# vibevoice-community/VibeVoice

Hardware: AMD Instinct MI355X
Metric: audio-sec/wall-sec (higher is better)
Workload: dtype bf16

## Files before the change

include/vvhip.h:

```cpp
#ifndef VVHIP_H
#define VVHIP_H
#include <stdint.h>
#ifdef __cplusplus
extern "C" {
#endif
typedef struct vv_ctx vv_ctx;

typedef struct vv_config {
    int lm_hidden, lm_layers, lm_heads, lm_kv_heads, lm_head_dim, lm_inter, lm_vocab;
    float lm_eps;
    int head_layers, head_ffn, latent_dim;
    float head_eps;
    int n_filters, n_ratios, ratios[8];
    int n_stages, enc_depths[8];
    int sem_dim;
    int has_acoustic_encoder;
    float codec_eps;
    int n_slots;
    int max_ctx;
    int max_rows;
    int xsplit;
    int attn_splits;
    int enc_frames;
    int use_graph;
    int tts_layers;
} vv_config;

#pragma GCC visibility push(default)
int vv_create(const vv_config* cfg, vv_ctx** out);
int vv_create_shared(const vv_config* cfg, vv_ctx* parent, vv_ctx** out);
void vv_destroy(vv_ctx* ctx);
const char* vv_last_error(vv_ctx* ctx);
const char* vv_build_id(void);
int vv_check(vv_ctx* ctx, void* stream);

int vv_num_weights(vv_ctx* ctx);
int vv_weight_info(vv_ctx* ctx, int idx, char* name, int name_cap, int64_t* nelem, int* loaded);
int vv_upload(vv_ctx* ctx, const char* name, const void* src, int src_dtype, int64_t nelem);
int vv_weight_read(vv_ctx* ctx, void* stream, const char* name, float* out_dev);
int vv_weight_shape(vv_ctx* ctx, const char* name, int* N, int* K);
int vv_lora_merge(vv_ctx* ctx, void* stream, const char* name, const float* a_dev, const float* b_dev, int r, float scale,
                  int delta_bf16);
int vv_lora_reset(vv_ctx* ctx, void* stream, const char* name);
int vv_set_speech_factors(vv_ctx* ctx, float scaling, float bias);
int vv_set_valid_tokens(vv_ctx* ctx, const int* ids, int n);
int vv_set_schedule(vv_ctx* ctx, int n_steps, const float* t, const float* coef, void* stream);
int vv_set_schedule_sde(vv_ctx* ctx, int n_steps, const float* t, const float* coef6, void* stream);

typedef struct vv_row { int cache; int pos; } vv_row;

int vv_lm_forward(vv_ctx* ctx, void* stream, int n_rows, const vv_row* rows,
                  const float* x_in_dev, float* hidden_out_dev);
int vv_lm_forward_range(vv_ctx* ctx, void* stream, int n_rows, const vv_row* rows, const float* x_in_dev,
                        float* hidden_out_dev, int layer_begin, int layer_end, int final_norm);
int vv_kv_import(vv_ctx* ctx, void* stream, int cache, int layer, int n_pos, const void* k_dev, const void* v_dev,
                 int src_dtype);
int vv_kv_import_at(vv_ctx* ctx, void* stream, int cache, int layer, int pos0, int n_pos, const void* k_dev,
                    const void* v_dev, int src_dtype);
int vv_kv_move(vv_ctx* ctx, void* stream, int cache, int src_pos, int dst_pos);
int vv_kv_export(vv_ctx* ctx, void* stream, int cache, int layer, int pos0, int n_pos, void* k_out_dev, void* v_out_dev,
                 int dst_dtype);
int64_t vv_kv_snapshot_bytes(vv_ctx* ctx, int n_pos);
int vv_kv_snapshot(vv_ctx* ctx, void* stream, int cache, int n_pos, void* k_out_dev, void* v_out_dev);
int vv_kv_restore(vv_ctx* ctx, void* stream, int cache, int n_pos, const void* k_dev, const void* v_dev);
int vv_add_type_embedding(vv_ctx* ctx, void* stream, int n, const float* x_dev, int type, float* out_dev);
int vv_eos_logit(vv_ctx* ctx, void* stream, int n, const float* hidden_dev, float* out_dev);
int vv_embed(vv_ctx* ctx, void* stream, int n, const int* ids, float* out_dev);
int vv_lm_logits(vv_ctx* ctx, void* stream, int n, const float* hidden_dev, float* logits_out_dev);
int vv_lm_logits_full(vv_ctx* ctx, void* stream, int n, const float* hidden_dev, float* logits_out_dev);
int vv_lm_warp_valid(vv_ctx* ctx, void* stream, int n, const float* logits_dev, const unsigned char* seen_dev,
                     float repetition_penalty, float temperature, int do_sample, int top_k, float top_p, float min_p,
                     float* out_dev, int* survivors_dev);
typedef struct vv_noise_key { uint32_t seed_lo, seed_hi, t0, aux; } vv_noise_key;
int vv_noise_rows(vv_ctx* ctx, void* stream, int n, const vv_noise_key* keys_host, uint32_t stream0, int n_streams,
                  int n_t, int width, float* out_dev);

int vv_diffusion_sample(vv_ctx* ctx, void* stream, int n, const float* cond_dev, const float* noise_dev,
                        float cfg_scale, float* latent_out_dev);
int vv_diffusion_sample_sde(vv_ctx* ctx, void* stream, int n, const float* cond_dev, const float* noise_dev,
                            const float* step_noise_dev, float cfg_scale, float* latent_out_dev);
int vv_diffusion_sample_rows(vv_ctx*, void* stream, int n, const float* cond_dev, const float* noise_dev,
                             const float* step_noise_dev, const float* cfg_rows_dev, float* latent_out_dev);
int vv_set_schedule_general(vv_ctx* ctx, int n_steps, const float* t, const float* coef8, int stochastic, void* stream);
int vv_diffusion_sample_general(vv_ctx* ctx, void* stream, int n, const float* cond_dev, const float* noise_dev,
                                const float* step_noise_dev, float cfg_scale, const float* cfg_rows_dev, float* latent_out_dev);
int vv_head_forward(vv_ctx* ctx, void* stream, int n, const float* noisy_dev, const float* t_host,
                    const float* cond_dev, float* out_dev);

int vv_codec_decode(vv_ctx* ctx, void* stream, int slot, int frames, const float* latent_dev,
                    float* audio_out_dev, int apply_speech_factors);
int vv_semantic_encode(vv_ctx* ctx, void* stream, int slot, int frames, const float* audio_dev,
                       float* sem_out_dev);
int vv_codec_chain_batch(vv_ctx* ctx, void* stream, int n, const int* slots, const float* latent_dev,
                         float* audio_out_dev, float* sem_out_dev, int apply_speech_factors);
int vv_acoustic_encode(vv_ctx* ctx, void* stream, int frames, const float* wav_dev, float* mean_out_dev);
int vv_acoustic_encode_ragged(vv_ctx* ctx, void* stream, int frames, long long valid_samples, const float* wav_dev, float* mean_out_dev);
int vv_set_enc_pass_frames(vv_ctx* ctx, int frames_per_pass);
int vv_audio_to_pcm16(vv_ctx* ctx, void* stream, int n, int samples, const float* audio_dev, int16_t* pcm_out_dev);
int vv_resampler_set(vv_ctx* ctx, int rs, int L, int M, int T, const float* coef_host, int n_streams, void* stream);
int vv_resampler_reset(vv_ctx* ctx, void* stream, int rs, int n, const int* stream_ids_host);
typedef struct vv_resample_row { int stream; int n_in; int flush; } vv_resample_row;
int vv_resample_rows(vv_ctx* ctx, void* stream, int rs, int n, const vv_resample_row* rows_host, const float* audio_dev, int ld_in,
                     void* out_dev, int ld_out, int out_fmt, int* n_out_host);
int vv_resample_once(vv_ctx* ctx, void* stream, int L, int M, int T, const float* coef_dev, int n, int n_in, const float* audio_dev,
                     int ld_in, float* out_dev, int ld_out);
int vv_tempo_set(vv_ctx* ctx, int tp, const float* window_host, int n_streams, void* stream);
int vv_tempo_reset(vv_ctx* ctx, void* stream, int tp, int n, const int* stream_ids_host);
#define VV_TEMPO_OVER_CAPACITY 3
typedef struct vv_tempo_row { int stream; int n_in; int flush; int P; int Q; } vv_tempo_row;
int vv_tempo_rows(vv_ctx* ctx, void* stream, int tp, int n, const vv_tempo_row* rows_host, const float* audio_dev, int ld_in,
                  void* out_dev, int ld_out, int out_fmt, int* n_out_host, int* offsets_dev, int ld_off);
int vv_tempo_once(vv_ctx* ctx, void* stream, const float* window_dev, int P, int Q, int n, int n_in, const float* audio_dev, int ld_in,
                  float* out_dev, int ld_out, int* offsets_dev, int ld_off);
int vv_codec_reset(vv_ctx* ctx, void* stream, int slot);
int vv_connect(vv_ctx* ctx, void* stream, int n, const float* latent_dev, const float* sem_dev,
               float* embeds_out_dev);

int64_t vv_packed_bytes(int N, int K);
int vv_pack_matrix(void* stream, const float* src_dev, void* dst_dev, int N, int K);
int vv_unpack_matrix(void* stream, const void* packed_dev, float* dst_dev, int N, int K);
int vv_lora_merge_raw(void* stream, const void* base_packed_dev, void* dst_packed_dev, int N, int K,
                      const float* a_dev, const float* b_dev, int r, float scale, int delta_bf16);
int vv_gemm_raw(void* stream, const void* w_packed_dev, const void* w2_packed_dev, const float* x_dev,
                float* y_dev, int T, int N, int K, int ldx, int ldy, int pro, int epi,
                const float* nw_dev, float eps, const float* bias_dev, const float* nscale_dev,
                int xsplit, int ksplit, int nontemporal);
#define VV_GEMV_REFUSED 1
typedef struct vv_gemv_case_args {
    const void* W; const void* W2; const float* X; float* Y;
    int T, N, K, ldx, ldy;
    int pro, epi;
    const float* nw; float eps; const float* bias; const float* nscale;
    const float* mod_scale; const float* mod_shift; int ld_mod;
    const float* addvec; int x_row_mod, add_rows_per_vec;
    const float* gate; int ld_gate;
    float* z; float* x0p; const float* coef; float cfg; int n_cfg; const float* sde_noise;
    int kgrid; float* yparts; const float* xa; int n_xa; const float* ya; int n_ya; int part_stride;
    int sl_n, sl_T, sl_x, sl_y; int sl_id[8];
    const float* dw_hist; const float* dw_w; const float* dw_b; const float* dw_gamma; const float* dw_nw;
    float* dw_xout; float* dw_hnew;
    const float* cfg_rows;
} vv_gemv_case_args;
int vv_gemv_case(void* stream, const vv_gemv_case_args* args, int xsplit, int* form_out);
int vv_gemm3_raw(vv_ctx* ctx, void* stream, const void* w_packed_dev, const void* w2_packed_dev, const float* x_dev, int T, int N, int K,
                 int epi, const float* nw_dev, float eps, const float* bias_dev, float* y_dev, void* xp_scratch, void* yp_scratch);
int vv_profile_begin(vv_ctx* ctx);
int vv_profile_end(vv_ctx* ctx, int64_t* launches, double* total_ms, double* bytes);
int vv_profile_replay(vv_ctx* ctx, void* stream, int reps, int64_t* launches, double* total_ms, double* bytes);
int vv_profile_replay_family(vv_ctx* ctx, void* stream, int family, int reps, int64_t* launches, double* total_ms, double* bytes);
int64_t vv_stat(vv_ctx* ctx, int what);

#pragma GCC visibility pop
#ifdef __cplusplus
}
#endif
#endif
```

vibevoice_amd/_lib.py:

```python
import ctypes as C
import os

HERE = os.path.dirname(os.path.abspath(__file__))
LIB_PATH = os.environ.get("VVHIP_LIB", os.path.join(HERE, "libvvhip.so"))


class VVConfig(C.Structure):
    _fields_ = [
        ("lm_hidden", C.c_int), ("lm_layers", C.c_int), ("lm_heads", C.c_int), ("lm_kv_heads", C.c_int),
        ("lm_head_dim", C.c_int), ("lm_inter", C.c_int), ("lm_vocab", C.c_int), ("lm_eps", C.c_float),
        ("head_layers", C.c_int), ("head_ffn", C.c_int), ("latent_dim", C.c_int), ("head_eps", C.c_float),
        ("n_filters", C.c_int), ("n_ratios", C.c_int), ("ratios", C.c_int * 8),
        ("n_stages", C.c_int), ("enc_depths", C.c_int * 8), ("sem_dim", C.c_int),
        ("has_acoustic_encoder", C.c_int), ("codec_eps", C.c_float),
        ("n_slots", C.c_int), ("max_ctx", C.c_int), ("max_rows", C.c_int), ("xsplit", C.c_int),
        ("attn_splits", C.c_int), ("enc_frames", C.c_int), ("use_graph", C.c_int), ("tts_layers", C.c_int),
    ]


class VVRow(C.Structure):
    _fields_ = [("cache", C.c_int), ("pos", C.c_int)]


_P = C.c_void_p


class VVGemvCase(C.Structure):
    _fields_ = [
        ("W", _P), ("W2", _P), ("X", _P), ("Y", _P),
        ("T", C.c_int), ("N", C.c_int), ("K", C.c_int), ("ldx", C.c_int), ("ldy", C.c_int),
        ("pro", C.c_int), ("epi", C.c_int),
        ("nw", _P), ("eps", C.c_float), ("bias", _P), ("nscale", _P),
        ("mod_scale", _P), ("mod_shift", _P), ("ld_mod", C.c_int),
        ("addvec", _P), ("x_row_mod", C.c_int), ("add_rows_per_vec", C.c_int),
        ("gate", _P), ("ld_gate", C.c_int),
        ("z", _P), ("x0p", _P), ("coef", _P), ("cfg", C.c_float), ("n_cfg", C.c_int), ("sde_noise", _P),
        ("kgrid", C.c_int), ("yparts", _P), ("xa", _P), ("n_xa", C.c_int), ("ya", _P), ("n_ya", C.c_int), ("part_stride", C.c_int),
        ("sl_n", C.c_int), ("sl_T", C.c_int), ("sl_x", C.c_int), ("sl_y", C.c_int), ("sl_id", C.c_int * 8),
        ("dw_hist", _P), ("dw_w", _P), ("dw_b", _P), ("dw_gamma", _P), ("dw_nw", _P), ("dw_xout", _P), ("dw_hnew", _P),
        ("cfg_rows", _P),
    ]


class VVNoiseKey(C.Structure):
    _fields_ = [("seed_lo", C.c_uint32), ("seed_hi", C.c_uint32), ("t0", C.c_uint32), ("aux", C.c_uint32)]


class VVResampleRow(C.Structure):
    _fields_ = [("stream", C.c_int), ("n_in", C.c_int), ("flush", C.c_int)]


class VVTempoRow(C.Structure):
    _fields_ = [("stream", C.c_int), ("n_in", C.c_int), ("flush", C.c_int), ("P", C.c_int), ("Q", C.c_int)]


GEMV_REFUSED = 1
TEMPO_OVER_CAPACITY = 3
_SIGS = {
    "vv_create": (C.c_int, [C.POINTER(VVConfig), C.POINTER(_P)]),
    "vv_create_shared": (C.c_int, [C.POINTER(VVConfig), _P, C.POINTER(_P)]),
    "vv_destroy": (None, [_P]),
    "vv_last_error": (C.c_char_p, [_P]),
    "vv_num_weights": (C.c_int, [_P]),
    "vv_weight_info": (C.c_int, [_P, C.c_int, C.c_char_p, C.c_int, C.POINTER(C.c_int64), C.POINTER(C.c_int)]),
    "vv_upload": (C.c_int, [_P, C.c_char_p, _P, C.c_int, C.c_int64]),
    "vv_set_speech_factors": (C.c_int, [_P, C.c_float, C.c_float]),
    "vv_set_valid_tokens": (C.c_int, [_P, C.POINTER(C.c_int), C.c_int]),
    "vv_set_schedule": (C.c_int, [_P, C.c_int, C.POINTER(C.c_float), C.POINTER(C.c_float), _P]),
    "vv_set_schedule_sde": (C.c_int, [_P, C.c_int, C.POINTER(C.c_float), C.POINTER(C.c_float), _P]),
    "vv_set_schedule_general": (C.c_int, [_P, C.c_int, C.POINTER(C.c_float), C.POINTER(C.c_float), C.c_int, _P]),
    "vv_lm_forward": (C.c_int, [_P, _P, C.c_int, C.POINTER(VVRow), _P, _P]),
    "vv_lm_forward_range": (C.c_int, [_P, _P, C.c_int, C.POINTER(VVRow), _P, _P, C.c_int, C.c_int, C.c_int]),
    "vv_kv_import": (C.c_int, [_P, _P, C.c_int, C.c_int, C.c_int, _P, _P, C.c_int]),
    "vv_kv_import_at": (C.c_int, [_P, _P, C.c_int, C.c_int, C.c_int, C.c_int, _P, _P, C.c_int]),
    "vv_add_type_embedding": (C.c_int, [_P, _P, C.c_int, _P, C.c_int, _P]),
    "vv_eos_logit": (C.c_int, [_P, _P, C.c_int, _P, _P]),
    "vv_embed": (C.c_int, [_P, _P, C.c_int, C.POINTER(C.c_int), _P]),
    "vv_lm_logits": (C.c_int, [_P, _P, C.c_int, _P, _P]),
    "vv_lm_logits_full": (C.c_int, [_P, _P, C.c_int, _P, _P]),
    "vv_lm_warp_valid": (C.c_int, [_P, _P, C.c_int, _P, _P, C.c_float, C.c_float, C.c_int, C.c_int, C.c_float, C.c_float, _P, _P]),
    "vv_noise_rows": (C.c_int, [_P, _P, C.c_int, C.POINTER(VVNoiseKey), C.c_uint32, C.c_int, C.c_int, C.c_int, _P]),
    "vv_diffusion_sample": (C.c_int, [_P, _P, C.c_int, _P, _P, C.c_float, _P]),
    "vv_diffusion_sample_sde": (C.c_int, [_P, _P, C.c_int, _P, _P, _P, C.c_float, _P]),
    "vv_diffusion_sample_rows": (C.c_int, [_P, _P, C.c_int, _P, _P, _P, _P, _P]),
    "vv_diffusion_sample_general": (C.c_int, [_P, _P, C.c_int, _P, _P, _P, C.c_float, _P, _P]),
    "vv_head_forward": (C.c_int, [_P, _P, C.c_int, _P, C.POINTER(C.c_float), _P, _P]),
    "vv_codec_decode": (C.c_int, [_P, _P, C.c_int, C.c_int, _P, _P, C.c_int]),
    "vv_semantic_encode": (C.c_int, [_P, _P, C.c_int, C.c_int, _P, _P]),
    "vv_codec_chain_batch": (C.c_int, [_P, _P, C.c_int, _P, _P, _P, _P, C.c_int]),
    "vv_acoustic_encode": (C.c_int, [_P, _P, C.c_int, _P, _P]),
    "vv_acoustic_encode_ragged": (C.c_int, [_P, _P, C.c_int, C.c_longlong, _P, _P]),
    "vv_kv_move": (C.c_int, [_P, _P, C.c_int, C.c_int, C.c_int]),
    "vv_kv_export": (C.c_int, [_P, _P, C.c_int, C.c_int, C.c_int, C.c_int, _P, _P, C.c_int]),
    "vv_kv_snapshot_bytes": (C.c_int64, [_P, C.c_int]),
    "vv_kv_snapshot": (C.c_int, [_P, _P, C.c_int, C.c_int, _P, _P]),
    "vv_kv_restore": (C.c_int, [_P, _P, C.c_int, C.c_int, _P, _P]),
    "vv_set_enc_pass_frames": (C.c_int, [_P, C.c_int]),
    "vv_audio_to_pcm16": (C.c_int, [_P, _P, C.c_int, C.c_int, _P, _P]),
    "vv_resampler_set": (C.c_int, [_P, C.c_int, C.c_int, C.c_int, C.c_int, _P, C.c_int, _P]),
    "vv_resampler_reset": (C.c_int, [_P, _P, C.c_int, C.c_int, C.POINTER(C.c_int)]),
    "vv_resample_rows": (C.c_int, [_P, _P, C.c_int, C.c_int, C.POINTER(VVResampleRow), _P, C.c_int, _P, C.c_int, C.c_int,
                                   C.POINTER(C.c_int)]),
    "vv_resample_once": (C.c_int, [_P, _P, C.c_int, C.c_int, C.c_int, _P, C.c_int, C.c_int, _P, C.c_int, _P, C.c_int]),
    "vv_tempo_set": (C.c_int, [_P, C.c_int, _P, C.c_int, _P]),
    "vv_tempo_reset": (C.c_int, [_P, _P, C.c_int, C.c_int, C.POINTER(C.c_int)]),
    "vv_tempo_rows": (C.c_int, [_P, _P, C.c_int, C.c_int, C.POINTER(VVTempoRow), _P, C.c_int, _P, C.c_int, C.c_int, C.POINTER(C.c_int), _P,
                                C.c_int]),
    "vv_tempo_once": (C.c_int, [_P, _P, _P, C.c_int, C.c_int, C.c_int, C.c_int, _P, C.c_int, _P, C.c_int, _P, C.c_int]),
    "vv_codec_reset": (C.c_int, [_P, _P, C.c_int]),
    "vv_connect": (C.c_int, [_P, _P, C.c_int, _P, _P, _P]),
    "vv_packed_bytes": (C.c_int64, [C.c_int, C.c_int]),
    "vv_pack_matrix": (C.c_int, [_P, _P, _P, C.c_int, C.c_int]),
    "vv_unpack_matrix": (C.c_int, [_P, _P, _P, C.c_int, C.c_int]),
    "vv_lora_merge_raw": (C.c_int, [_P, _P, _P, C.c_int, C.c_int, _P, _P, C.c_int, C.c_float, C.c_int]),
    "vv_weight_read": (C.c_int, [_P, _P, C.c_char_p, _P]),
    "vv_weight_shape": (C.c_int, [_P, C.c_char_p, C.POINTER(C.c_int), C.POINTER(C.c_int)]),
    "vv_lora_merge": (C.c_int, [_P, _P, C.c_char_p, _P, _P, C.c_int, C.c_float, C.c_int]),
    "vv_lora_reset": (C.c_int, [_P, _P, C.c_char_p]),
    "vv_gemm_raw": (C.c_int, [_P, _P, _P, _P, _P, C.c_int, C.c_int, C.c_int, C.c_int, C.c_int, C.c_int, C.c_int,
                              _P, C.c_float, _P, _P, C.c_int, C.c_int, C.c_int]),
    "vv_gemv_case": (C.c_int, [_P, C.POINTER(VVGemvCase), C.c_int, C.POINTER(C.c_int)]),
    "vv_gemm3_raw": (C.c_int, [_P, _P, _P, _P, _P, C.c_int, C.c_int, C.c_int, C.c_int, _P, C.c_float, _P, _P, _P, _P]),
    "vv_profile_begin": (C.c_int, [_P]),
    "vv_profile_end": (C.c_int, [_P, C.POINTER(C.c_int64), C.POINTER(C.c_double), C.POINTER(C.c_double)]),
    "vv_profile_replay": (C.c_int, [_P, _P, C.c_int, C.POINTER(C.c_int64), C.POINTER(C.c_double), C.POINTER(C.c_double)]),
    "vv_profile_replay_family": (C.c_int, [_P, _P, C.c_int, C.c_int, C.POINTER(C.c_int64), C.POINTER(C.c_double), C.POINTER(C.c_double)]),
    "vv_stat": (C.c_int64, [_P, C.c_int]),
    "vv_build_id": (C.c_char_p, []),
    "vv_check": (C.c_int, [_P, _P]),
}

EXPORTS = tuple(_SIGS)
_lib = None


def load():
    global _lib
    if _lib is not None:
        return _lib
    if not os.path.exists(LIB_PATH):
        raise RuntimeError(
            f"{LIB_PATH} is missing: the HIP engine has not been built "
            "(run `python -m vibevoice_amd.build`); there is no CPU/PyTorch fallback")
    from . import build as _build
    if _build.have_sources() and _build.binary_id(LIB_PATH) != _build.source_id():
        import sys
        print(f"[vibevoice_amd] {LIB_PATH} was built from other sources (binary id {_build.binary_id(LIB_PATH)}, sources "
              f"{_build.source_id()}): rebuilding with hipcc (about two minutes)", file=sys.stderr, flush=True)
        try:
            _build.build_locked()
        except Exception as ex:
            raise RuntimeError(
                f"{LIB_PATH} was built from different sources (binary id {_build.binary_id(LIB_PATH)}, sources "
                f"{_build.source_id()}) and could not be rebuilt ({ex}); run `python -m vibevoice_amd.build`") from ex
    lib = C.CDLL(LIB_PATH)
    for name, (res, args) in _SIGS.items():
        fn = getattr(lib, name)
        fn.restype = res
        fn.argtypes = args
    _lib = lib
    return lib
```

vibevoice_amd/build.py:

```python
import os
import shutil
import subprocess
import sys

HERE = os.path.dirname(os.path.abspath(__file__))
CSRC = os.path.join(HERE, "csrc")
LIB = os.path.join(HERE, "libvvhip.so")
SOURCES = ["gemm.hip", "gemv.hip", "gemv16p.hip", "headtail.hip", "solver.hip", "tile.hip", "prefill.hip", "attn.hip", "misc.hip", "warp.hip", "noise.hip", "kvspan.hip", "block1d.hip", "lora.hip", "resample.hip", "tempo.hip", "engine.hip",
           "engine_lm.hip", "engine_head.hip", "engine_codec.hip", "engine_prof.hip", "engine_lora.hip"]
HEADERS = [os.path.join(CSRC, "vv_common.h"), os.path.join(CSRC, "vv_device.h"), os.path.join(CSRC, "vv_launch.h"), os.path.join(CSRC, "gemv_plan.h"),
           os.path.join(CSRC, "prefill_plan.h"), os.path.join(CSRC, "pass_plan.h"), os.path.join(CSRC, "engine_ctx.h"),
           os.path.join(os.path.dirname(HERE), "include", "vvhip.h")]


def _hipcc():
    for c in ("/opt/rocm/bin/hipcc", shutil.which("hipcc") or ""):
        if c and os.path.exists(c):
            return c
    raise RuntimeError("hipcc not found: libvvhip.so cannot be built")


FLAGS = ["--offload-arch=gfx950", "-O3", "-std=c++17", "-fPIC", "-shared", "-fvisibility=hidden", "-fvisibility-inlines-hidden",
         "-Wno-unused-value", "-Wno-unused-result", "-mllvm", "-amdgpu-kernarg-preload-count=16"]


def _extra_flags():
    return os.environ.get("VVHIP_CFLAGS", "").split()


def source_id():
    import hashlib
    h = hashlib.sha256()
    for d in [os.path.join(CSRC, s) for s in SOURCES] + HEADERS:
        h.update(os.path.basename(d).encode() + b"\0")
        with open(d, "rb") as f:
            h.update(f.read())
    h.update(" ".join(FLAGS + _extra_flags()).encode())
    return h.hexdigest()[:16]


def binary_id(path=LIB):
    try:
        with open(path, "rb") as f:
            blob = f.read()
    except OSError:
        return None
    k = blob.find(b"VVHIP_BUILD_ID=")
    if k < 0:
        return None
    return blob[k + 15:k + 31].decode("ascii", "replace")


def have_sources():
    return all(os.path.exists(d) for d in [os.path.join(CSRC, s) for s in SOURCES] + HEADERS)


def stale():
    if not os.path.exists(LIB):
        return True
    return have_sources() and binary_id() != source_id()


def _object_key(src, flags, build_id):
    import hashlib
    h = hashlib.sha256()
    for d in [src] + HEADERS:
        with open(d, "rb") as f:
            h.update(f.read())
    h.update(" ".join(flags).encode())
    if os.path.basename(src) == "engine.hip":
        h.update(build_id.encode())
    return h.hexdigest()[:16]


def build(force=False, verbose=True, _locked=False):
    if not force and not stale():
        return LIB
    if not _locked:
        import fcntl
        with open(LIB + ".lock", "w") as lk:
            fcntl.flock(lk, fcntl.LOCK_EX)
            try:
                if not force and not stale():
                    return LIB
                return build(force=force, verbose=verbose, _locked=True)
            finally:
                fcntl.flock(lk, fcntl.LOCK_UN)
    from concurrent.futures import ThreadPoolExecutor
    hipcc = _hipcc()
    bid = source_id()
    cflags = [f for f in FLAGS if f != "-shared"] + _extra_flags()
    objdir = os.path.join(CSRC, ".obj")
    os.makedirs(objdir, exist_ok=True)
    jobs, objs = [], []
    for sname in SOURCES:
        src = os.path.join(CSRC, sname)
        obj = os.path.join(objdir, f"{os.path.splitext(sname)[0]}.{_object_key(src, cflags, bid)}.o")
        objs.append(obj)
        if not os.path.exists(obj):
            jobs.append((src, obj))

    def compile_one(job):
        src, obj = job
        tmp = f"{obj}.tmp{os.getpid()}"
        cmd = [hipcc] + cflags + [f'-DVV_BUILD_ID="{bid}"', "-c", src, "-o", tmp]
        if verbose:
            print("[vibevoice_amd] compiling", os.path.basename(src), file=sys.stderr)
        subprocess.run(cmd, check=True)
        os.replace(tmp, obj)
    with ThreadPoolExecutor(max_workers=min(8, max(1, len(jobs)))) as ex:
        list(ex.map(compile_one, jobs))
    keep = set(objs)
    for fn in os.listdir(objdir):
        full = os.path.join(objdir, fn)
        if fn.endswith(".o") and full not in keep:
            try:
                os.remove(full)
            except OSError:
                pass
    tmp = f"{LIB}.tmp{os.getpid()}"
    cmd = [hipcc, "--offload-arch=gfx950", "-shared", "-fPIC"] + _extra_flags() + objs + ["-o", tmp]
    if verbose:
        print("[vibevoice_amd] linking libvvhip.so", file=sys.stderr)
    subprocess.run(cmd, check=True)
    os.replace(tmp, LIB)
    return LIB


def build_locked():
    import fcntl
    with open(LIB + ".lock", "w") as lk:
        fcntl.flock(lk, fcntl.LOCK_EX)
        try:
            if stale():
                build(force=True, verbose=False, _locked=True)
        finally:
            fcntl.flock(lk, fcntl.LOCK_UN)
    return LIB


if __name__ == "__main__":
    build(force="--force" in sys.argv)
    print(LIB)
```

vibevoice_amd/csrc/block1d.hip:

```cpp
#include "vv_common.h"
#include "vv_device.h"
#include "vv_launch.h"

namespace {

struct VVBlock {
    const float* xin;
    float* xout;
    float* nst;
    const float *norm_w, *ffn_norm_w, *gamma, *ffn_gamma, *dw_w , *dw_b, *b1, *b2;
    const u32x4 *w1, *w2;
    int T;
    float eps;
    VVSlotIds sl;
    int64_t sx, snst;
};

template <int XS>
__device__ __forceinline__ void split_store(unsigned char* base, size_t part_stride, int byte_off, float v) {
    __bf16 h = (__bf16)v;
    *reinterpret_cast<__bf16*>(base + byte_off) = h;
    if constexpr (XS > 1) {
        float r = v - (float)h;
        __bf16 m = (__bf16)r;
        *reinterpret_cast<__bf16*>(base + part_stride + byte_off) = m;
        if constexpr (XS > 2) *reinterpret_cast<__bf16*>(base + 2 * part_stride + byte_off) = (__bf16)(r - (float)m);
    }
}

template <int C, int XS>
__global__ __launch_bounds__(256) void vv_block1d_kernel(const VVBlock a) {
    constexpr int TT = 16, HALO = 6, F = 4 * C;
    constexpr int KT1 = C / 32, NT1 = F / 16;
    constexpr int KT2 = F / 32, NT2 = C / 16;
    extern __shared__ __attribute__((aligned(16))) unsigned char smem[];
    float* nrm = reinterpret_cast<float*>(smem);
    float* xs = nrm + (TT + HALO) * C;
    float* rs2 = xs + TT * C;
    unsigned char* f1 = reinterpret_cast<unsigned char*>(rs2 + TT);
    unsigned char* f2 = f1 + (size_t)XS * KT1 * 1024;
    const int tid = threadIdx.x, lane = tid & 63;
    const int wave = __builtin_amdgcn_readfirstlane(tid >> 6);
    const int t0 = blockIdx.x * TT;
    const float* xin = a.xin; float* xout = a.xout; float* nst = a.nst;
    if (a.sl.n > 0) {
        const int64_t id = vv_slot_id(a.sl.id, blockIdx.y);
        xin += id * a.sx; xout += id * a.sx; nst += id * a.snst;
    }
    constexpr int M1 = (NT1 + 3) / 4, M2 = (NT2 + 3) / 4;
    u32x4 w1r[M1][KT1], w2r[M2][KT2];
#pragma unroll
    for (int i = 0; i < M1; ++i) {
        const int nt = wave + 4 * i;
#pragma unroll
        for (int kt = 0; kt < KT1; ++kt)
            w1r[i][kt] = (nt < NT1) ? a.w1[((int64_t)nt * KT1 + kt) * 64 + lane] : u32x4{0u, 0u, 0u, 0u};
    }
#pragma unroll
    for (int i = 0; i < M2; ++i) {
        const int nt = wave + 4 * i;
#pragma unroll
        for (int kt = 0; kt < KT2; ++kt)
            w2r[i][kt] = (nt < NT2) ? a.w2[((int64_t)nt * KT2 + kt) * 64 + lane] : u32x4{0u, 0u, 0u, 0u};
    }

    constexpr int CL = (C + 63) / 64;
    float nw_r[CL], fnw_r[CL];
#pragma unroll
    for (int i = 0; i < CL; ++i) {
        const int c = lane + i * 64;
        nw_r[i] = (c < C) ? a.norm_w[c] : 0.f;
        fnw_r[i] = (c < C) ? a.ffn_norm_w[c] : 0.f;
    }
    const int cc = tid % C;
    float dw_r[7];
#pragma unroll
    for (int j = 0; j < 7; ++j) dw_r[j] = a.dw_w[j * C + cc];
    const float dwb_r = a.dw_b[cc], gam_r = a.gamma[cc];
    const int frow = lane & 15, fq = lane >> 4;
    float4 b1_r[M1], b2_r[M2], fg_r[M2];
#pragma unroll
    for (int i = 0; i < M1; ++i) {
        const int nt = wave + 4 * i;
        b1_r[i] = (nt < NT1) ? *reinterpret_cast<const float4*>(a.b1 + nt * 16 + fq * 4) : float4{0.f, 0.f, 0.f, 0.f};
    }
#pragma unroll
    for (int i = 0; i < M2; ++i) {
        const int nt = wave + 4 * i;
        b2_r[i] = (nt < NT2) ? *reinterpret_cast<const float4*>(a.b2 + nt * 16 + fq * 4) : float4{0.f, 0.f, 0.f, 0.f};
        fg_r[i] = (nt < NT2) ? *reinterpret_cast<const float4*>(a.ffn_gamma + nt * 16 + fq * 4) : float4{0.f, 0.f, 0.f, 0.f};
    }

    constexpr int RW = (TT + HALO + 3) / 4;
    float xv[RW][CL];
#pragma unroll
    for (int i = 0; i < RW; ++i) {
        const int rr = wave + 4 * i;
        const int t = t0 - HALO + rr;
#pragma unroll
        for (int q = 0; q < CL; ++q) {
            const int c = lane + q * 64;
            float v = 0.f;
            if (rr < TT + HALO && c < C) {
                if (t < 0) v = nst[(HALO + t) * C + c];
                else if (t < a.T) v = xin[(int64_t)t * C + c];
            }
            xv[i][q] = v;
        }
    }
#pragma unroll
    for (int i = 0; i < RW; ++i) {
        const int rr = wave + 4 * i;
        if (rr >= TT + HALO) break;
        const int t = t0 - HALO + rr;
        if (t < 0) {
#pragma unroll
            for (int q = 0; q < CL; ++q) { const int c = lane + q * 64; if (c < C) nrm[rr * C + c] = xv[i][q]; }
        } else if (t < a.T) {
            float s = 0.f;
#pragma unroll
            for (int q = 0; q < CL; ++q) s += xv[i][q] * xv[i][q];
            const float r = rsqrtf(vv_wave_sum(s) / (float)C + a.eps);
#pragma unroll
            for (int q = 0; q < CL; ++q) {
                const int c = lane + q * 64;
                if (c < C) {
                    const float n = xv[i][q] * r * nw_r[q];
                    nrm[rr * C + c] = n;
                    if (rr >= HALO) xs[(rr - HALO) * C + c] = xv[i][q];
                    if (t >= a.T - HALO) nst[(HALO + t - (a.T - HALO)) * C + c] = n;
                }
            }
        } else {
#pragma unroll
            for (int q = 0; q < CL; ++q) {
                const int c = lane + q * 64;
                if (c < C) { nrm[rr * C + c] = 0.f; if (rr >= HALO) xs[(rr - HALO) * C + c] = 0.f; }
            }
        }
    }
    __syncthreads();
    for (int e = tid; e < TT * C; e += 256) {
        const int r = e / C;
        float acc = dwb_r;
#pragma unroll
        for (int j = 0; j < 7; ++j) acc += dw_r[j] * nrm[(r + j) * C + cc];
        xs[e] += gam_r * acc;
    }
    __syncthreads();
    for (int r = wave; r < TT; r += 4) {
        float s = 0.f;
        float xr[CL];
#pragma unroll
        for (int q = 0; q < CL; ++q) { const int c = lane + q * 64; xr[q] = (c < C) ? xs[r * C + c] : 0.f; s += xr[q] * xr[q]; }
        const float rr = rsqrtf(vv_wave_sum(s) / (float)C + a.eps);
#pragma unroll
        for (int q = 0; q < CL; ++q) {
            const int c = lane + q * 64;
            if (c < C) {
                const float n = xr[q] * rr * fnw_r[q];
                const int off = vv_packed_index(c >> 5, r, c) * 2;
                split_store<XS>(f1, (size_t)KT1 * 1024, off, n);
            }
        }
    }
    __syncthreads();
#pragma unroll
    for (int i1 = 0; i1 < M1; ++i1) {
        const int nt = wave + 4 * i1;
        if (nt >= NT1) break;
        f32x4 acc = {0.f, 0.f, 0.f, 0.f};
#pragma unroll
        for (int kt = 0; kt < KT1; ++kt) {
            const bf16x8 wf = __builtin_bit_cast(bf16x8, w1r[i1][kt]);
#pragma unroll
            for (int p = 0; p < XS; ++p) {
                const bf16x8 xb = __builtin_bit_cast(bf16x8, *reinterpret_cast<const u32x4*>(f1 + ((size_t)(p * KT1 + kt) * 64 + lane) * 16));
                acc = __builtin_amdgcn_mfma_f32_16x16x32_bf16(wf, xb, acc, 0, 0, 0);
            }
        }
        const int n0 = nt * 16 + fq * 4;
        float u[4];
        const float bb[4] = {b1_r[i1].x, b1_r[i1].y, b1_r[i1].z, b1_r[i1].w};
#pragma unroll
        for (int r = 0; r < 4; ++r) u[r] = vv_gelu_erf(acc[r] + bb[r]);
        const int off = vv_packed_index(n0 >> 5, frow, n0) * 2;
#pragma unroll
        for (int r = 0; r < 4; ++r) split_store<XS>(f2, (size_t)KT2 * 1024, off + r * 2, u[r]);
    }
    __syncthreads();
#pragma unroll
    for (int i2 = 0; i2 < M2; ++i2) {
        const int nt = wave + 4 * i2;
        if (nt >= NT2) break;
        f32x4 acc = {0.f, 0.f, 0.f, 0.f};
#pragma unroll
        for (int kt = 0; kt < KT2; ++kt) {
            const bf16x8 wf = __builtin_bit_cast(bf16x8, w2r[i2][kt]);
#pragma unroll
            for (int p = 0; p < XS; ++p) {
                const bf16x8 ub = __builtin_bit_cast(bf16x8, *reinterpret_cast<const u32x4*>(f2 + ((size_t)(p * KT2 + kt) * 64 + lane) * 16));
                acc = __builtin_amdgcn_mfma_f32_16x16x32_bf16(wf, ub, acc, 0, 0, 0);
            }
        }
        const int c0 = nt * 16 + fq * 4;
        const int t = t0 + frow;
        if (t < a.T) {
            float4 o;
            o.x = xs[frow * C + c0 + 0] + fg_r[i2].x * (acc[0] + b2_r[i2].x);
            o.y = xs[frow * C + c0 + 1] + fg_r[i2].y * (acc[1] + b2_r[i2].y);
            o.z = xs[frow * C + c0 + 2] + fg_r[i2].z * (acc[2] + b2_r[i2].z);
            o.w = xs[frow * C + c0 + 3] + fg_r[i2].w * (acc[3] + b2_r[i2].w);
            *reinterpret_cast<float4*>(xout + (int64_t)t * C + c0) = o;
        }
    }
}

template <int C, int XS>
static void go(const VVBlock& a, hipStream_t s) {
    constexpr int TT = 16, HALO = 6, F = 4 * C;
    const size_t smem = (size_t)((TT + HALO) * C + TT * C + TT) * 4 + (size_t)XS * (C / 32) * 1024 + (size_t)XS * (F / 32) * 1024;
    static const hipError_t lds = vv_raise_lds_limit(160 * 1024, &vv_block1d_kernel<C, XS>);
    (void)lds;
    hipLaunchKernelGGL((vv_block1d_kernel<C, XS>), dim3((a.T + TT - 1) / TT, a.sl.n > 0 ? a.sl.n : 1), dim3(256), smem, s, a);
}

}

extern "C" int vv_block1d_supported(int C) { return C == 32 || C == 64 || C == 128; }
extern "C" int vv_block1d_slots_launch(int C, int xs, const float* xin, float* xout, float* nst, const float* norm_w,
                                       const float* ffn_norm_w, const float* gamma, const float* ffn_gamma,
                                       const float* dw_w, const float* dw_b, const float* b1, const float* b2,
                                       const void* w1, const void* w2, int T, float eps, const int* ids, int n, int64_t sx,
                                       int64_t snst, hipStream_t s) {
    if (n < 0 || n > 8) return -1;
    VVBlock a{xin, xout, nst, norm_w, ffn_norm_w, gamma, ffn_gamma, dw_w, dw_b, b1, b2,
              (const u32x4*)w1, (const u32x4*)w2, T, eps};
    a.sl = vv_slot_ids(ids, n);
    a.sx = sx; a.snst = snst;
#define VV_B(C_)                                                     \
    do {                                                             \
        if (xs == 1) go<C_, 1>(a, s);                                \
        else if (xs == 2) go<C_, 2>(a, s);                           \
        else go<C_, 3>(a, s);                                        \
    } while (0)
    if (C == 32) VV_B(32);
    else if (C == 64) VV_B(64);
    else if (C == 128) VV_B(128);
    else return -1;
#undef VV_B
    return vv_launch_rc(0);
}
```

vibevoice_amd/csrc/engine_codec.hip:

```cpp
#include "engine_ctx.h"

static bool is_stem(const ConvG& g) { return g.K == 7 && g.ldx == 1; }
static bool is_conv1_head(const ConvG& g) { return g.N == 1 && g.K == 7 * g.ldx && (g.ldx & 3) == 0 && g.ldx <= 1024; }

int build_codec(vv_ctx* ctx, CodecNet& net, const std::string& pfx, bool decoder, int vae_dim, int Fmax, int n_slots) {
    const vv_config& c = ctx->c;
    const int ns = c.n_stages;
    const int nf = c.n_filters;
    net.decoder = decoder; net.Fmax = Fmax;
    std::vector<int> depths(ns), ratios(c.n_ratios);
    if (decoder) { for (int i = 0; i < ns; ++i) depths[i] = c.enc_depths[ns - 1 - i]; for (int i = 0; i < c.n_ratios; ++i) ratios[i] = c.ratios[i]; }
    else { for (int i = 0; i < ns; ++i) depths[i] = c.enc_depths[i]; for (int i = 0; i < c.n_ratios; ++i) ratios[i] = c.ratios[c.n_ratios - 1 - i]; }
    int hop = 1; for (int i = 0; i < c.n_ratios; ++i) hop *= c.ratios[i];
    ctx->hop = hop;
    std::vector<int> C(ns), Tpf(ns);
    for (int i = 0; i < ns; ++i) {
        if (decoder) { C[i] = nf << (ns - 1 - i); Tpf[i] = (i == 0) ? 1 : Tpf[i - 1] * ratios[i - 1]; }
        else { C[i] = nf << i; Tpf[i] = (i == 0) ? hop : Tpf[i - 1] / ratios[i - 1]; }
    }
    net.in_dim = decoder ? vae_dim : 1;
    net.out_dim = decoder ? 1 : vae_dim;
    net.in_Tpf = decoder ? 1 : hop;
    net.in_hist = 6;
    net.maxC = 1;
    size_t umax = 0;
    struct StageW { ConvG in; std::vector<Block> blocks; };
    std::vector<StageW> sw(ns);
    for (int i = 0; i < ns; ++i) {
        ConvG& g = sw[i].in;
        char nm[256];
        if (i == 0) {
            const int Cin = net.in_dim;
            g.K = 7 * Cin; g.N = C[0]; g.ldx = Cin; g.rows_per_frame = Tpf[0];
            g.w = alloc_packed(ctx, g.N, g.K);
            snprintf(nm, 256, "%s%s.0.0.conv.conv.", pfx.c_str(), decoder ? "upsample_layers" : "downsample_layers");
            add_mat(ctx, std::string(nm) + "weight", g.N, g.K, g.w, 0, 1, Cin, g.N, 7, 1);
            g.bias = add_vec(ctx, std::string(nm) + "bias", g.N);
        } else if (decoder) {
            const int s = ratios[i - 1], Cin = C[i - 1], Cout = C[i];
            g.K = 2 * Cin; g.N = s * Cout; g.ldx = Cin; g.rows_per_frame = Tpf[i - 1];
            g.w = alloc_packed(ctx, g.N, g.K);
            snprintf(nm, 256, "%supsample_layers.%d.0.convtr.convtr.", pfx.c_str(), i);
            add_mat(ctx, std::string(nm) + "weight", g.N, g.K, g.w, 0, 2, Cin, Cout, 2 * s, s, (int64_t)Cin * Cout * 2 * s);
            g.bias = add_vec(ctx, std::string(nm) + "bias", Cout, nullptr, W_BIAS_REP, s);
        } else {
            const int s = ratios[i - 1], Cin = C[i - 1], Cout = C[i];
            g.K = 2 * s * Cin; g.N = Cout; g.ldx = s * Cin; g.rows_per_frame = Tpf[i];
            g.w = alloc_packed(ctx, g.N, g.K);
            snprintf(nm, 256, "%sdownsample_layers.%d.0.conv.conv.", pfx.c_str(), i);
            add_mat(ctx, std::string(nm) + "weight", g.N, g.K, g.w, 0, 1, Cin, Cout, 2 * s, s);
            g.bias = add_vec(ctx, std::string(nm) + "bias", Cout);
        }
        if (C[i] > net.maxC) net.maxC = C[i];
        for (int j = 0; j < depths[i]; ++j) {
            Block b; b.C = C[i]; b.nb = nullptr;
            snprintf(nm, 256, "%sstages.%d.%d.", pfx.c_str(), i, j);
            std::string p(nm);
            b.gamma = add_vec(ctx, p + "gamma", C[i]);
            b.ffn_gamma = add_vec(ctx, p + "ffn_gamma", C[i]);
            b.norm_w = add_vec(ctx, p + "norm.weight", C[i]);
            b.ffn_norm_w = add_vec(ctx, p + "ffn_norm.weight", C[i]);
            b.dw_w = add_vec(ctx, p + "mixer.conv.conv.conv.weight", (int64_t)C[i] * 7, nullptr, W_DW);
            b.dw_b = add_vec(ctx, p + "mixer.conv.conv.conv.bias", C[i]);
            b.w1 = alloc_packed(ctx, 4 * C[i], C[i]);
            add_mat(ctx, p + "ffn.linear1.weight", 4 * C[i], C[i], b.w1, 0);
            b.b1 = add_vec(ctx, p + "ffn.linear1.bias", 4 * C[i]);
            b.w2 = alloc_packed(ctx, C[i], 4 * C[i]);
            add_mat(ctx, p + "ffn.linear2.weight", C[i], 4 * C[i], b.w2, 0);
            b.b2 = add_vec(ctx, p + "ffn.linear2.bias", C[i]);
            sw[i].blocks.push_back(b);
            size_t ub = (size_t)Tpf[i] * Fmax * 4 * C[i] * 4;
            if (ub > umax) umax = ub;
        }
    }
    {
        ConvG& g = net.head;
        const int Cin = C[ns - 1];
        g.K = 7 * Cin; g.N = net.out_dim; g.ldx = Cin; g.rows_per_frame = Tpf[ns - 1];
        g.w = alloc_packed(ctx, g.N, g.K);
        add_mat(ctx, pfx + "head.conv.conv.weight", g.N, g.K, g.w, 0, 1, Cin, g.N, 7, 1);
        g.bias = add_vec(ctx, pfx + "head.conv.conv.bias", g.N);
    }
    auto pad64 = [](size_t n) { return (n + 63) / 64 * 64; };
    net.u.resize(n_slots);
    net.u_stride = (int64_t)pad64(umax / 4 + 1);
    float* u_all = (float*)dalloc(ctx, (size_t)n_slots * net.u_stride * 4, false);
    net.in_buf.resize(n_slots); net.st.resize(n_slots);
    net.in_stride = (int64_t)pad64((size_t)(6 + net.in_Tpf * Fmax) * net.in_dim);
    float* in_all = (float*)dalloc(ctx, (size_t)n_slots * net.in_stride * 4);
    if (!u_all || !in_all) return -1;
    for (int sl = 0; sl < n_slots; ++sl) {
        net.u[sl] = u_all + (size_t)sl * net.u_stride;
        net.in_buf[sl] = in_all + (size_t)sl * net.in_stride;
        net.st[sl].resize(ns);
    }
    for (int i = 0; i < ns; ++i) {
        const int hist = (i == ns - 1) ? 6 : (decoder ? 1 : ratios[i]);
        const bool fused = vv_block1d_supported(C[i]) && Tpf[i] >= 8 && !sw[i].blocks.empty();
        const bool pp = !fused && !sw[i].blocks.empty() && (vv_normdw_sliced_ok(Tpf[i], C[i]) || vv_normdw_rows_ok(Tpf[i], C[i]));
        const int64_t xstride = (int64_t)pad64((size_t)(hist + (size_t)Tpf[i] * Fmax) * C[i]);
        float* xs_all = (float*)dalloc(ctx, (size_t)n_slots * xstride * 4);
        float* xs2_all = (fused || pp) ? (float*)dalloc(ctx, (size_t)n_slots * xstride * 4) : nullptr;
        if (!xs_all || ((fused || pp) && !xs2_all)) return -1;
        const int64_t nbstride = (int64_t)pad64(fused ? (size_t)12 * C[i] : (size_t)(6 + (size_t)Tpf[i] * Fmax) * C[i]);
        std::vector<float*> nb_all(sw[i].blocks.size());
        for (auto& p : nb_all) { p = (float*)dalloc(ctx, (size_t)n_slots * nbstride * 4); if (!p) return -1; }
        for (int sl = 0; sl < n_slots; ++sl) {
            Stage& s = net.st[sl][i];
            s.C = C[i]; s.Tpf = Tpf[i]; s.in = sw[i].in; s.hist = hist; s.fused = fused; s.pp = pp; s.sl_stride = xstride;
            s.xs = xs_all + (size_t)sl * xstride;
            s.xs2 = xs2_all ? xs2_all + (size_t)sl * xstride : nullptr;
            s.blocks = sw[i].blocks;
            s.xfinal = ((s.fused || s.pp) && (s.blocks.size() & 1)) ? s.xs2 : s.xs;
            for (size_t j = 0; j < s.blocks.size(); ++j) {
                Block& b = s.blocks[j];
                b.nb = nullptr; b.nst = nullptr; b.nb_stride = nbstride;
                if (s.fused) b.nst = nb_all[j] + (size_t)sl * nbstride;
                else b.nb = nb_all[j] + (size_t)sl * nbstride;
            }
        }
    }
    {
        const char* mode = getenv("VVHIP_BATCH_CODEC");
        const bool off = (mode && !strcmp(mode, "0")) || ctx->c.xsplit > 2 || n_slots < 2 || Fmax != 1;
        const bool heavy_only = mode && !strcmp(mode, "heavy");
        auto gemm_ok = [&](const ConvG& cg, int64_t sx, int64_t sy) {
            VVGemm g = mk_gemm(cg.w, net.in_buf[0], net.u[0], 2 * cg.rows_per_frame, cg.N, cg.K, cg.ldx, cg.N);
            g.epi = VV_EPI_BIAS; g.bias = cg.bias;
            g.sl_n = 2; g.sl_T = cg.rows_per_frame; g.sl_x = (int)sx; g.sl_y = (int)sy; g.sl_id[0] = 0; g.sl_id[1] = n_slots - 1;
            return vv_gemv_ok(&g) != 0;
        };
        auto ok = [&](int i) {
            const Stage& s = net.st[0][i];
            if (off || s.blocks.empty() || (s.C & 31)) return false;
            if (!is_stem(s.in) && !gemm_ok(s.in, i == 0 ? net.in_stride : net.st[0][i - 1].sl_stride, s.sl_stride)) return false;
            if (s.pp && vv_normdw_sliced_ok(s.Tpf, s.C)) return true;
            if (heavy_only) return false;
            return s.fused || (s.pp && vv_normdw_rows_ok(s.Tpf, s.C));
        };
        net.kd = 0; net.ke = ns;
        if (decoder) { while (net.kd < ns && ok(net.kd)) net.kd++; }
        else { while (net.ke > 0 && ok(net.ke - 1)) net.ke--; }
        const ConvG& h = net.head;
        const bool conv1 = is_conv1_head(h);
        net.head_batch = !off && !heavy_only && (conv1 || gemm_ok(h, net.st[0][ns - 1].sl_stride, 0));
        if (!decoder && net.ke < ns && !(conv1 || gemm_ok(h, net.st[0][ns - 1].sl_stride, 0))) net.ke = ns;
    }
    return 0;
}

struct SlotSet { const int* ids; int n; int sl; };
static SlotSet one_slot(int sl) { return {nullptr, 0, sl}; }

static void codec_table_entries(CodecNet& net, int sl, int F, std::vector<VVShiftH>& t) {
    t.push_back({net.in_buf[sl], net.in_Tpf * F, 6, net.in_dim});
    for (auto& s : net.st[sl]) {
        t.push_back({s.xfinal, s.Tpf * F, s.hist, s.C});
        for (auto& b : s.blocks) {
            if (s.fused) t.push_back({b.nst, 6, 6, s.C});
            else t.push_back({b.nb, s.Tpf * F, 6, s.C});
        }
    }
}
static int codec_tables(vv_ctx* ctx, CodecNet& net, SlotSet ss, int F, void** tab_out, int* n_out) {
    const int* ids = ss.n ? ss.ids : &ss.sl;
    const int n = ss.n ? ss.n : 1;
    uint64_t mask = 0;
    for (int j = 0; j < n; ++j) {
        if (ids[j] >= 64) return fail(ctx, "tokenizer slot %d: the history tables are keyed by a 64-bit slot mask", ids[j]);
        mask |= 1ull << ids[j];
    }
    auto it = net.shift_tab.find({mask, F});
    if (it == net.shift_tab.end()) {
        std::vector<VVShiftH> t;
        for (int j = 0; j < n; ++j) codec_table_entries(net, ids[j], F, t);
        void* d = dalloc(ctx, t.size() * sizeof(VVShiftH), false);
        if (!d) return -1;
        HIPCHK(ctx, hipMemcpy(d, t.data(), t.size() * sizeof(VVShiftH), hipMemcpyHostToDevice));
        it = net.shift_tab.emplace(std::make_pair(mask, F), std::make_pair(d, (int)t.size())).first;
    }
    *tab_out = it->second.first; *n_out = it->second.second;
    return 0;
}

static int run_codec(vv_ctx* ctx, CodecNet& net, SlotSet ss, int F, float* out, hipStream_t st, int i0 = 0, int i1 = -1,
                     bool head = true, bool shift = true, int tail_valid = -1) {
    const float eps = ctx->c.codec_eps;
    const bool batched = ss.n > 0;
    const bool stream_w = (F == 1);
    const int base = batched ? 0 : ss.sl;
    auto& stages = net.st[base];
    float* u = net.u[base];
    const int ns = (int)stages.size();
    if (i1 < 0) i1 = ns;
    auto stride = [&](int64_t s) { return batched ? s : (int64_t)0; };
    auto slots = [&](VVGemm& g, int rows, int64_t sx, int64_t sy) {
        if (!batched) return;
        g.sl_n = ss.n; g.sl_T = rows; g.sl_x = (int)sx; g.sl_y = (int)sy; g.T = ss.n * rows;
        for (int j = 0; j < 8; ++j) g.sl_id[j] = j < ss.n ? ss.ids[j] : 0;
    };
    auto nt = [&](int rows) { return batched ? 1 : (int)(stream_w && rows <= 16); };
    auto ffn1 = [&](const Stage& s, const Block& b, float* xo, int T, const float* dw_in) {
        VVGemm g1 = mk_gemm(b.w1, dw_in ? dw_in : xo, u, T, 4 * s.C, s.C, s.C, 4 * s.C);
        g1.pro = VV_PRO_RMS; g1.nw = b.ffn_norm_w; g1.eps = eps; g1.epi = VV_EPI_BIAS_GELU; g1.bias = b.b1; g1.nt = nt(T);
        if (dw_in) {
            g1.pro = VV_PRO_NORMDW;
            g1.dw_hist = b.nb; g1.dw_w = b.dw_w; g1.dw_b = b.dw_b; g1.dw_gamma = b.gamma; g1.dw_nw = b.norm_w;
            g1.dw_xout = xo; g1.dw_hnew = b.nb + 6 * (size_t)s.C;
        }
        slots(g1, T, s.sl_stride, 0);
        return g1;
    };
    auto ffn = [&](const Stage& s, const Block& b, const VVGemm& g1, float* xo, int T) -> int {
        GEMM(g1);
        VVGemm g2 = mk_gemm(b.w2, u, xo, T, s.C, 4 * s.C, 4 * s.C, s.C);
        g2.epi = VV_EPI_RESID; g2.bias = b.b2; g2.nscale = b.ffn_gamma; g2.nt = nt(T);
        slots(g2, T, 0, s.sl_stride);
        GEMM(g2);
        return 0;
    };
    for (int i = i0; i < i1; ++i) {
        Stage& s = stages[i];
        const int T = s.Tpf * F;
        float* x = s.xs + (size_t)s.hist * s.C;
        if (tail_valid >= 0 && i > 0) {
            Stage& pv = stages[i - 1];
            const int Tp = pv.Tpf * F;
            if (tail_valid < Tp)
                VVCHK(vv_zero_launch(pv.xfinal + ((size_t)pv.hist + tail_valid) * pv.C, (size_t)(Tp - tail_valid) * pv.C * 4, st));
            const int r = pv.Tpf / s.Tpf;
            tail_valid = (tail_valid + r - 1) / r;
        }
        {
            const ConvG& cg = s.in;
            const float* X = (i == 0) ? net.in_buf[base] : stages[i - 1].xfinal;
            const int64_t sx = (i == 0) ? net.in_stride : stages[i - 1].sl_stride;
            const int Trows = cg.rows_per_frame * F;
            if (is_stem(cg)) {
                ctx->launches++;
                VVCHK(vv_stem_conv_slots_launch(X, cg.w, cg.bias, x, Trows, cg.N, ss.ids, ss.n, stride(sx), stride(s.sl_stride), st));
            } else {
                VVGemm g = mk_gemm(cg.w, X, x, Trows, cg.N, cg.K, cg.ldx, cg.N);
                g.epi = VV_EPI_BIAS; g.bias = cg.bias; g.nt = nt(Trows);
                slots(g, Trows, sx, s.sl_stride);
                GEMM(g);
            }
        }
        float* xo = (s.fused || s.pp) ? s.xs2 + (size_t)s.hist * s.C : x;
        if (s.fused) {
            for (auto& b : s.blocks) {
                ctx->launches++;
                VVCHK(vv_block1d_slots_launch(s.C, ctx->c.xsplit, x, xo, b.nst, b.norm_w, b.ffn_norm_w, b.gamma, b.ffn_gamma, b.dw_w, b.dw_b,
                                              b.b1, b.b2, b.w1, b.w2, T, eps, ss.ids, ss.n, stride(s.sl_stride), stride(b.nb_stride), st));
                std::swap(x, xo);
            }
            continue;
        }
        for (auto& b : s.blocks) {
            const bool sliced = s.pp && vv_normdw_sliced_ok(T, s.C);
            if (sliced && T == 1 && !batched) {
                const VVGemm g1 = ffn1(s, b, xo, T, x);
                if (vv_gemv_ok(&g1)) {
                    VVTRY(ffn(s, b, g1, xo, T));
                    std::swap(x, xo);
                    continue;
                }
            }
            if (sliced) {
                ctx->launches += 1;
                VVCHK(vv_normdw_sliced_slots_launch(x, xo, b.nb, b.norm_w, b.dw_w, b.dw_b, b.gamma, T, s.C, eps, ss.ids, ss.n, stride(s.sl_stride),
                                                    stride(b.nb_stride), st));
            } else if (s.pp && vv_normdw_rows_ok(T, s.C)) {
                ctx->launches += 1;
                VVCHK(vv_normdw_rows_slots_launch(x, xo, b.nb, b.norm_w, b.dw_w, b.dw_b, b.gamma, T, s.C, eps, ss.ids, ss.n, stride(s.sl_stride),
                                                  stride(b.nb_stride), st));
            } else if (!s.pp && (size_t)T * s.C <= 8192 && (s.C & 3) == 0) {
                ctx->launches += 1;
                VVCHK(vv_normdw_launch(x, b.nb, b.norm_w, b.dw_w, b.dw_b, b.gamma, T, s.C, eps, st));
            } else {
                ctx->launches += 2;
                VVCHK(vv_rmsnorm_rows_launch(x, s.C, b.nb + 6 * (size_t)s.C, s.C, b.norm_w, T, s.C, eps, st));
                VVCHK(vv_dwconv_res_launch(b.nb, x, xo, b.dw_w, b.dw_b, b.gamma, T, s.C, st));
            }
            VVTRY(ffn(s, b, ffn1(s, b, xo, T, nullptr), xo, T));
            if (s.pp) std::swap(x, xo);
        }
    }
    if (head) {
        const ConvG& cg = net.head;
        Stage& s = stages[ns - 1];
        const int Trows = cg.rows_per_frame * F;
        if (is_conv1_head(cg)) {
            ctx->launches++;
            VVCHK(vv_head_conv1_slots_launch(s.xfinal, cg.w, cg.bias, out, Trows, cg.ldx, ss.ids, ss.n, stride(s.sl_stride), stride(Trows), st));
        } else {
            VVGemm g = mk_gemm(cg.w, s.xfinal, out, Trows, cg.N, cg.K, cg.ldx, cg.N);
            g.epi = VV_EPI_BIAS; g.bias = cg.bias;
            slots(g, Trows, s.sl_stride, 0);
            GEMM(g);
        }
    }
    if (!shift) return 0;
    void* tab; int n_tab;
    if (codec_tables(ctx, net, ss, F, &tab, &n_tab)) return -1;
    ctx->launches++;
    VVCHK(vv_shift_rows_launch(tab, n_tab, net.maxC, st));
    return 0;
}

static int zero_codec(vv_ctx* ctx, CodecNet& net, int sl, hipStream_t st) {
    void* tab; int nt;
    if (codec_tables(ctx, net, one_slot(sl), 1, &tab, &nt)) return -1;
    ctx->launches++;
    VVCHK(vv_zero_hist_launch(tab, nt, st));
    return 0;
}
extern "C" int vv_codec_decode(vv_ctx* ctx, void* stream, int slot, int frames, const float* latent_dev, float* audio_out_dev, int apply) {
    hipStream_t st = (hipStream_t)stream;
    if (slot < 0 || slot >= ctx->c.n_slots) return fail(ctx, "slot %d out of range", slot);
    if (frames != 1) return fail(ctx, "vv_codec_decode: streaming decode takes one frame per call");
    CodecNet& net = ctx->dec;
    ctx->launches = 0;
    char key[128]; snprintf(key, 128, "dec:%d:%d:%d:%p:%p", apply ? 1 : 0, slot, frames, (const void*)latent_dev, (void*)audio_out_dev);
    return graphed(ctx, key, st, [&]() {
        const int L = ctx->c.latent_dim;
        const float mul = apply ? 1.0f / ctx->scaling : 1.0f, add = apply ? -ctx->bias : 0.0f;
        ctx->launches++;
        VVCHK(vv_affine_launch(latent_dev, net.in_buf[slot] + 6 * L, mul, add, frames * L, st));
        return run_codec(ctx, net, one_slot(slot), frames, audio_out_dev, st);
    });
}

extern "C" int vv_semantic_encode(vv_ctx* ctx, void* stream, int slot, int frames, const float* audio_dev, float* sem_out_dev) {
    hipStream_t st = (hipStream_t)stream;
    if (ctx->c.sem_dim <= 0) return fail(ctx, "no semantic tokenizer configured");
    if (slot < 0 || slot >= ctx->c.n_slots) return fail(ctx, "slot %d out of range", slot);
    if (frames != 1) return fail(ctx, "vv_semantic_encode: streaming encode takes one frame per call");
    CodecNet& net = ctx->senc;
    ctx->launches = 0;
    char key[128]; snprintf(key, 128, "senc:%d:%d:%p:%p", slot, frames, (const void*)audio_dev, (void*)sem_out_dev);
    return graphed(ctx, key, st, [&]() {
        VVCHK(vv_copy_launch(net.in_buf[slot] + 6, audio_dev, (size_t)frames * ctx->hop * 4, st));
        return run_codec(ctx, net, one_slot(slot), frames, sem_out_dev, st);
    });
}

extern "C" int vv_codec_chain_batch(vv_ctx* ctx, void* stream, int n, const int* slots, const float* latent_dev,
                                    float* audio_out_dev, float* sem_out_dev, int apply) {
    hipStream_t st = (hipStream_t)stream;
    if (n < 1 || n > 8) return fail(ctx, "vv_codec_chain_batch: n = %d, must be 1..8", n);
    uint64_t mask = 0;
    for (int j = 0; j < n; ++j) {
        if (slots[j] < 0 || slots[j] >= ctx->c.n_slots || slots[j] >= 64) return fail(ctx, "slot %d out of range", slots[j]);
        if (mask & (1ull << slots[j])) return fail(ctx, "vv_codec_chain_batch: slot %d listed twice", slots[j]);
        mask |= 1ull << slots[j];
    }
    const bool sem = sem_out_dev != nullptr;
    if (sem && ctx->c.sem_dim <= 0) return fail(ctx, "no semantic tokenizer configured");
    if (!ctx->side_ready) {
        for (int j = 0; j < 8; ++j) {
            HIPCHK(ctx, hipStreamCreateWithFlags(&ctx->side[j], hipStreamNonBlocking));
            HIPCHK(ctx, hipEventCreateWithFlags(&ctx->ev_join[j], hipEventDisableTiming));
        }
        HIPCHK(ctx, hipEventCreateWithFlags(&ctx->ev_fork, hipEventDisableTiming));
        ctx->side_ready = true;
    }
    ctx->launches = 0;
    std::string key = apply ? "chain:1:" : "chain:0:";
    for (int j = 0; j < n; ++j) key += std::to_string(slots[j]) + ",";
    char kp[128]; snprintf(kp, 128, ":%p:%p:%p", (const void*)latent_dev, (void*)audio_out_dev, (void*)sem_out_dev);
    key += kp;
    std::vector<int> ids(slots, slots + n);
    return graphed(ctx, key, st, [&]() {
        CodecNet& dec = ctx->dec; CodecNet& senc = ctx->senc;
        const int L = ctx->c.latent_dim, S = ctx->c.sem_dim, hop = ctx->hop;
        const float mul = apply ? 1.0f / ctx->scaling : 1.0f, add = apply ? -ctx->bias : 0.0f;
        const int ns_d = (int)dec.st[0].size(), ns_e = sem ? (int)senc.st[0].size() : 0;
        const bool bd = n > 1 && dec.kd > 0, be = sem && n > 1 && senc.ke < ns_e;
        const bool dec_full = bd && dec.kd == ns_d && dec.head_batch;
        const bool enc_full = be && senc.ke == 0;
        const bool fork = n > 1 && !(dec_full && (!sem || enc_full));
        const SlotSet set = {ids.data(), n, 0};
        if (bd) {
            ctx->launches++;
            VVCHK(vv_affine_slots_launch(latent_dev, dec.in_buf[0] + 6 * L, mul, add, L, ids.data(), n, dec.in_stride, st));
            if (run_codec(ctx, dec, set, 1, audio_out_dev, st, 0, dec.kd, dec_full, dec_full)) return -1;
        }
        if (fork || n == 1) {
            if (fork) HIPCHK(ctx, hipEventRecord(ctx->ev_fork, st));
            for (int j = 0; j < n; ++j) {
                hipStream_t ss = fork ? ctx->side[j] : st;
                const int sl = ids[j];
                if (fork) HIPCHK(ctx, hipStreamWaitEvent(ss, ctx->ev_fork, 0));
                float* audio = audio_out_dev + (size_t)j * hop;
                if (!dec_full) {
                    if (!bd) {
                        ctx->launches++;
                        VVCHK(vv_affine_launch(latent_dev + (size_t)j * L, dec.in_buf[sl] + 6 * L, mul, add, L, ss));
                    }
                    if (run_codec(ctx, dec, one_slot(sl), 1, audio, ss, bd ? dec.kd : 0, ns_d, true, true)) return -1;
                }
                if (sem) {
                    VVCHK(vv_copy_launch(senc.in_buf[sl] + 6, audio, (size_t)hop * 4, ss));
                    if (run_codec(ctx, senc, one_slot(sl), 1, sem_out_dev + (size_t)j * S, ss, 0, be ? senc.ke : ns_e, !be, !be)) return -1;
                }
                if (fork) HIPCHK(ctx, hipEventRecord(ctx->ev_join[j], ss));
            }
            if (fork) for (int j = 0; j < n; ++j) HIPCHK(ctx, hipStreamWaitEvent(st, ctx->ev_join[j], 0));
        } else if (sem) {
            ctx->launches++;
            VVCHK(vv_affine_slots_launch(audio_out_dev, senc.in_buf[0] + 6, 1.0f, 0.0f, hop, ids.data(), n, senc.in_stride, st));
        }
        if (be && run_codec(ctx, senc, set, 1, sem_out_dev, st, senc.ke, ns_e, true, true)) return -1;
        return 0;
    });
}

extern "C" int vv_acoustic_encode_ragged(vv_ctx* ctx, void* stream, int frames, long long valid_samples, const float* wav_dev, float* mean_out_dev) {
    VV_SHARED;
    hipStream_t st = (hipStream_t)stream;
    if (!ctx->c.has_acoustic_encoder) return fail(ctx, "no acoustic encoder configured");
    if (valid_samples <= (int64_t)(frames - 1) * ctx->hop || valid_samples > (int64_t)frames * ctx->hop)
        return fail(ctx, "vv_acoustic_encode_ragged: %lld valid samples do not end in frame %d of %d", (long long)valid_samples, frames - 1, frames);
    CodecNet& net = ctx->aenc;
    if (zero_codec(ctx, net, 0, st)) return -1;
    const int L = ctx->c.latent_dim;
    const int pass = ctx->enc_pass > 0 ? std::min(ctx->enc_pass, net.Fmax) : net.Fmax;
    for (int f0 = 0; f0 < frames; f0 += pass) {
        const int F = std::min(pass, frames - f0);
        VVCHK(vv_copy_launch(net.in_buf[0] + 6, wav_dev + (size_t)f0 * ctx->hop, (size_t)F * ctx->hop * 4, st));
        const int64_t v = valid_samples - (int64_t)f0 * ctx->hop;
        const int tail = (f0 + F == frames && v < (int64_t)F * ctx->hop) ? (int)v : -1;
        if (run_codec(ctx, net, one_slot(0), F, mean_out_dev + (size_t)f0 * L, st, 0, -1, true, true, tail)) return -1;
    }
    return 0;
}

extern "C" int vv_acoustic_encode(vv_ctx* ctx, void* stream, int frames, const float* wav_dev, float* mean_out_dev) {
    return vv_acoustic_encode_ragged(ctx, stream, frames, (long long)frames * ctx->hop, wav_dev, mean_out_dev);
}

extern "C" int vv_set_enc_pass_frames(vv_ctx* ctx, int frames_per_pass) {
    if (!ctx->c.has_acoustic_encoder) return fail(ctx, "no acoustic encoder configured");
    if (frames_per_pass < 1 || frames_per_pass > ctx->aenc.Fmax) return fail(ctx, "frames_per_pass %d out of range [1,%d]", frames_per_pass, ctx->aenc.Fmax);
    ctx->enc_pass = frames_per_pass;
    return 0;
}

extern "C" int vv_codec_reset(vv_ctx* ctx, void* stream, int slot) {
    VV_SHARED;
    hipStream_t st = (hipStream_t)stream;
    if (slot < 0 || slot >= ctx->c.n_slots) return fail(ctx, "slot %d out of range", slot);
    if (zero_codec(ctx, ctx->dec, slot, st)) return -1;
    if (ctx->c.sem_dim > 0 && zero_codec(ctx, ctx->senc, slot, st)) return -1;
    return 0;
}

static int64_t rs_emitted(int64_t total, int L, int M, int T) {
    const int64_t a = total * L - (L * T - 2) / 2 - 1;
    return a < 0 ? 0 : a / M + 1;
}

extern "C" int vv_resampler_set(vv_ctx* ctx, int rs, int L, int M, int T, const float* coef_host, int n_streams, void* stream) {
    VV_SHARED;
    if (rs < 0 || rs >= vv_ctx::N_RESAMPLERS) return fail(ctx, "vv_resampler_set: configuration %d out of range [0,%d)", rs, vv_ctx::N_RESAMPLERS);
    if (L < 1 || L > 4096 || M < 1 || M > 4096) return fail(ctx, "vv_resampler_set: L = %d, M = %d must be in [1,4096]", L, M);
    if (T < 2 || (T & 1) || T > 4096) return fail(ctx, "vv_resampler_set: T = %d must be even and in [2,4096]", T);
    if (n_streams < 1 || n_streams > 65536) return fail(ctx, "vv_resampler_set: n_streams = %d must be in [1,65536]", n_streams);
    if (!coef_host) return fail(ctx, "vv_resampler_set: null coefficient table");
    if (vv_resample_lds_bytes(L, T, T) > 65536 - 64)
        return fail(ctx, "vv_resampler_set: the %d x %d coefficient table (%d bytes) does not fit the resampling kernel's 64 KiB of LDS; "
                         "this rate pair is not served", L, T, L * T * 4);
    vv_ctx::Resampler& r = ctx->rs[rs];
    HIPCHK(ctx, hipStreamSynchronize((hipStream_t)stream));
    dfree(ctx, r.coef); dfree(ctx, r.hist);
    r = vv_ctx::Resampler();
    float* coef = (float*)dalloc(ctx, (size_t)L * T * 4, false);
    float* hist = (float*)dalloc(ctx, (size_t)n_streams * T * 4, true);
    if (!coef || !hist) { dfree(ctx, coef); dfree(ctx, hist); return -1; }
    if (hipMemcpy(coef, coef_host, (size_t)L * T * 4, hipMemcpyHostToDevice) != hipSuccess) {
        dfree(ctx, coef); dfree(ctx, hist);
        return fail(ctx, "vv_resampler_set: the coefficient upload failed");
    }
    r.L = L; r.M = M; r.T = T; r.n_streams = n_streams; r.coef = coef; r.hist = hist;
    r.total.assign(n_streams, 0); r.flushed.assign(n_streams, 0);
    return 0;
}

extern "C" int vv_resampler_reset(vv_ctx* ctx, void* stream, int rs, int n, const int* stream_ids_host) {
    VV_SHARED;
    hipStream_t st = (hipStream_t)stream;
    if (rs < 0 || rs >= vv_ctx::N_RESAMPLERS || !ctx->rs[rs].coef) return fail(ctx, "vv_resampler_reset: configuration %d is not set", rs);
    vv_ctx::Resampler& r = ctx->rs[rs];
    std::vector<int> ids;
    if (!stream_ids_host) { for (int i = 0; i < r.n_streams; ++i) ids.push_back(i); }
    else {
        if (n < 1) return fail(ctx, "vv_resampler_reset: n = %d must be >= 1", n);
        ids.assign(stream_ids_host, stream_ids_host + n);
    }
    for (int id : ids)
        if (id < 0 || id >= r.n_streams) return fail(ctx, "vv_resampler_reset: stream id %d out of range [0,%d)", id, r.n_streams);
    for (size_t i0 = 0; i0 < ids.size(); i0 += 16)
        VVCHK(vv_resample_reset_launch(r.hist, r.T, r.n_streams, ids.data() + i0, (int)std::min<size_t>(16, ids.size() - i0), st));
    for (int id : ids) { r.total[id] = 0; r.flushed[id] = 0; }
    return 0;
}

extern "C" int vv_resample_rows(vv_ctx* ctx, void* stream, int rs, int n, const vv_resample_row* rows_host, const float* audio_dev, int ld_in,
                                void* out_dev, int ld_out, int out_fmt, int* n_out_host) {
    VV_SHARED;
    if (rs < 0 || rs >= vv_ctx::N_RESAMPLERS || !ctx->rs[rs].coef) return fail(ctx, "vv_resample_rows: configuration %d is not set", rs);
    vv_ctx::Resampler& r = ctx->rs[rs];
    if (n < 1 || n > 16) return fail(ctx, "vv_resample_rows: n = %d must be in [1,16]", n);
    if (!rows_host || !out_dev || !n_out_host) return fail(ctx, "vv_resample_rows: null rows / out / n_out pointer");
    if (out_fmt != 0 && out_fmt != 1) return fail(ctx, "vv_resample_rows: out_fmt = %d must be 0 (fp32) or 1 (int16)", out_fmt);
    VVRsRows kr;
    memset(&kr, 0, sizeof(kr));
    int max_in = 0;
    for (int i = 0; i < n; ++i) {
        const vv_resample_row& q = rows_host[i];
        if (q.stream < 0 || q.stream >= r.n_streams) return fail(ctx, "vv_resample_rows: row %d: stream id %d out of range [0,%d)", i, q.stream, r.n_streams);
        for (int j = 0; j < i; ++j)
            if (rows_host[j].stream == q.stream) return fail(ctx, "vv_resample_rows: stream %d is named twice (rows %d and %d)", q.stream, j, i);
        if (q.n_in < 0) return fail(ctx, "vv_resample_rows: row %d: n_in = %d must be >= 0", i, q.n_in);
        if (q.n_in > ld_in || (q.n_in > 0 && !audio_dev)) return fail(ctx, "vv_resample_rows: row %d: n_in = %d exceeds the input rows (ld_in = %d)", i, q.n_in, ld_in);
        if (r.flushed[q.stream]) return fail(ctx, "vv_resample_rows: stream %d has been flushed; reset it before its next push", q.stream);
        const int64_t before = r.total[q.stream], after = before + q.n_in;
        const int64_t m0 = rs_emitted(before, r.L, r.M, r.T);
        const int64_t m1 = q.flush ? (after * r.L + r.M - 1) / r.M : rs_emitted(after, r.L, r.M, r.T);
        const int64_t n_out = m1 - m0;
        if (n_out > ld_out) return fail(ctx, "vv_resample_rows: row %d emits %lld samples, the output rows hold %d", i, (long long)n_out, ld_out);
        if (n_out > VV_RS_MAX_OUT) return fail(ctx, "vv_resample_rows: row %d emits %lld samples, one push emits at most %d per row", i, (long long)n_out, VV_RS_MAX_OUT);
        const int64_t k0 = m0 * r.M + (r.L * r.T - 2) / 2;
        kr.r[i].stream = q.stream; kr.r[i].n_in = q.n_in; kr.r[i].n_out = (int)n_out;
        kr.r[i].p0 = (int)(k0 % r.L); kr.r[i].b0 = (int)(k0 / r.L - before + r.T);
        max_in = std::max(max_in, q.n_in);
    }
    if (vv_resample_lds_bytes(r.L, r.T, max_in) > 65536 - 64)
        return fail(ctx, "vv_resample_rows: a chunk of %d samples does not fit the kernel's LDS beside the %d x %d table; push at most %d at a time",
                    max_in, r.L, r.T, (65536 - 64) / 4 - r.L * (r.T + 1) - r.T - r.T / 2);
    for (int i = n; i < 16; ++i) kr.r[i] = kr.r[0];
    VVCHK(vv_resample_rows_launch(&kr, n, r.L, r.M, r.T, r.coef, r.hist, r.n_streams, audio_dev, ld_in, out_dev, ld_out, out_fmt, (hipStream_t)stream));
    for (int i = 0; i < n; ++i) {
        r.total[rows_host[i].stream] += rows_host[i].n_in;
        if (rows_host[i].flush) r.flushed[rows_host[i].stream] = 1;
        n_out_host[i] = kr.r[i].n_out;
    }
    return 0;
}

extern "C" int vv_resample_once(vv_ctx* ctx, void* stream, int L, int M, int T, const float* coef_dev, int n, int n_in, const float* audio_dev,
                                int ld_in, float* out_dev, int ld_out) {
    VV_SHARED;
    if (L < 1 || L > 4096 || M < 1 || M > 4096 || T < 2 || (T & 1) || T > 4096) return fail(ctx, "vv_resample_once: L = %d, M = %d in [1,4096], T = %d even in [2,4096]", L, M, T);
    if (n < 1 || n > 65535 || n_in < 1 || n_in > ld_in) return fail(ctx, "vv_resample_once: n = %d in [1,65535], n_in = %d in [1, ld_in = %d]", n, n_in, ld_in);
    const int64_t n_out = ((int64_t)n_in * L + M - 1) / M;
    if (n_out > ld_out || n_out >= ((int64_t)1 << 31) - 256) return fail(ctx, "vv_resample_once: %lld output samples per row, the output rows hold %d", (long long)n_out, ld_out);
    if (!coef_dev || !audio_dev || !out_dev) return fail(ctx, "vv_resample_once: null coef / audio / out pointer");
    VVCHK(vv_resample_once_launch(L, M, T, coef_dev, n, n_in, audio_dev, ld_in, out_dev, ld_out, (hipStream_t)stream));
    return 0;
}

static int64_t tp_a(int64_t k, int P, int Q) { return k < 0 ? -(int64_t)VV_TP_HS : (k * VV_TP_HS * P) / Q; }

static int64_t tp_emitted(int64_t total, int P, int Q) {
    const int64_t room = total - VV_TP_DELTA - VV_TP_N;
    if (room < 0) return 0;
    int64_t k = ((room + 1) * Q) / ((int64_t)VV_TP_HS * P) + 1;
    while (k > 0 && std::max(tp_a(k - 1, P, Q), tp_a(k - 2, P, Q) + VV_TP_HS) > room) --k;
    return k;
}

static bool tp_speed_ok(int P, int Q) { return P >= 1 && Q >= 1 && Q <= 100 && P <= 2 * Q && Q <= 2 * P; }

extern "C" int vv_tempo_set(vv_ctx* ctx, int tp, const float* window_host, int n_streams, void* stream) {
    VV_SHARED;
    if (tp < 0 || tp >= vv_ctx::N_TEMPOS) return fail(ctx, "vv_tempo_set: configuration %d out of range [0,%d)", tp, vv_ctx::N_TEMPOS);
    if (n_streams < 1 || n_streams > 65536) return fail(ctx, "vv_tempo_set: n_streams = %d must be in [1,65536]", n_streams);
    if (!window_host) return fail(ctx, "vv_tempo_set: null window table");
// ... 100 lines not shown
```

vibevoice_amd/csrc/engine_prof.hip:

```cpp
#include "engine_ctx.h"

static __global__ void vv_nan_probe_kernel(const float* __restrict__ p, int n, unsigned* __restrict__ rec) {
    unsigned cnt = 0, first = 0xffffffffu, mx = 0;
    for (int i = blockIdx.x * blockDim.x + threadIdx.x; i < n; i += gridDim.x * blockDim.x) {
        const float v = p[i];
        if (!(fabsf(v) <= 3.0e38f)) { cnt++; first = min(first, (unsigned)i); }
        else mx = max(mx, __float_as_uint(fabsf(v)));
    }
    if (cnt) { atomicAdd(rec, cnt); atomicMax(rec + 1, 0xffffffffu - first); }
    atomicMax(rec + 2, mx);
}
void nan_probe(vv_ctx* ctx, hipStream_t st, const char* name, const void* p, size_t n) {
    if (!ctx->probe_on || !p || n == 0) return;
    const int id = (int)ctx->probe_names.size();
    if (id >= PROBE_MAX) return;
    ctx->probe_names.push_back(name);
    if (id == 0) (void)vv_zero_launch(ctx->probe_rec, PROBE_MAX * 16, st);
    hipLaunchKernelGGL(vv_nan_probe_kernel, dim3(64), dim3(256), 0, st, (const float*)p, (int)n, ctx->probe_rec + 4 * id);
}
void nan_probe_report(vv_ctx* ctx, hipStream_t st, const char* what) {
    if (!ctx->probe_on) return;
    std::vector<unsigned> h(PROBE_MAX * 4);
    const hipError_t e1 = hipStreamSynchronize(st);
    const hipError_t e2 = hipMemcpy(h.data(), ctx->probe_rec, PROBE_MAX * 16, hipMemcpyDeviceToHost);
    const int call = ctx->probe_calls++;
    if (e1 != hipSuccess || e2 != hipSuccess) { fprintf(stderr, "[nan_probe] %s call %d: sync %d copy %d\n", what, call, (int)e1, (int)e2); (void)hipGetLastError(); return; }
    { const size_t ns = ctx->probe_names.size(); bool tail_dirty = false;
      for (size_t i = 4 * ns; i < (size_t)PROBE_MAX * 4; ++i) if (h[i]) { tail_dirty = true; break; }
      if (tail_dirty) fprintf(stderr, "[nan_probe] %s call %d (prof %d): record buffer %p holds words nobody wrote: %08x %08x %08x %08x | %08x %08x %08x %08x (last 4 words)\n",
                              what, call, (int)ctx->prof_on, (void*)ctx->probe_rec, h[0], h[1], h[2], h[3], h[4092], h[4093], h[4094], h[4095]); }
    int bad = 0;
    for (size_t i = 0; i < ctx->probe_names.size(); ++i) if (h[4 * i]) bad++;
    if (!bad) { if (call < 6) fprintf(stderr, "[nan_probe] %s call %d: %zu stages clean\n", what, call, ctx->probe_names.size()); return; }
    fprintf(stderr, "[nan_probe] %s call %d: %d of %zu stages hold non-finite values\n", what, call, bad, ctx->probe_names.size());
    int shown = 0;
    for (size_t i = 0; i < ctx->probe_names.size() && shown < 12; ++i) {
        float mx; memcpy(&mx, &h[4 * i + 2], 4);
        if (h[4 * i] || (i + 1 < ctx->probe_names.size() && h[4 * (i + 1)] && !shown)) {
            fprintf(stderr, "[nan_probe]   stage %3zu %-28s non-finite %u (first at %u), finite absmax %.4e\n", i, ctx->probe_names[i].c_str(), h[4 * i],
                    h[4 * i] ? 0xffffffffu - h[4 * i + 1] : 0u, mx);
            if (h[4 * i]) shown++;
        }
    }
}
static double gemm_bytes(const VVGemm& g) {
    double w = (double)vv_packed_elems(g.N, g.K) * 2.0 * (g.W2 ? 2.0 : 1.0);
    double x = (double)g.T * g.K * 4.0;
    double y = (double)g.T * g.N * 4.0 * ((g.epi == VV_EPI_RESID || g.epi == VV_EPI_GATED_RESID) ? 2.0 : 1.0);
    return w + x + y;
}
int gemm_prof(vv_ctx* ctx, const VVGemm& g, hipStream_t st) {
    if ((size_t)(2 * ctx->prof_n + 2) > ctx->prof_ev.size()) {
        size_t old = ctx->prof_ev.size();
        ctx->prof_ev.resize(old + 2048);
        for (size_t i = old; i < ctx->prof_ev.size(); ++i) hipEventCreate(&ctx->prof_ev[i]);
    }
    ctx->prof_stream = st;
    hipEventRecord(ctx->prof_ev[2 * ctx->prof_n], st);
    int r = vv_gemm_launch(g, ctx->c.xsplit, st);
    hipEventRecord(ctx->prof_ev[2 * ctx->prof_n + 1], st);
    ctx->prof_n++;
    ctx->prof_bytes += gemm_bytes(g);
    const bool is_gemv = vv_gemm_route(&g, ctx->c.xsplit) == VV_ROUTE_GEMV;
    ctx->prof_rec.push_back({g.T, g.N, g.K, g.pro, g.epi, g.W2 ? 1 : 0, gemm_bytes(g), is_gemv});
    if (is_gemv) { ctx->prof_gemv.push_back(g); ctx->prof_gemv_bytes += gemm_bytes(g); }
    return r;
}
#ifdef VV_GEMM_TIMING
constexpr int TL_MAX = 4096, TL_STRIDE = 16 + 2 * 3200;
int gemm_tl(vv_ctx* ctx, VVGemm g, hipStream_t st) {
    if (!ctx->tl_base && getenv("VVHIP_TIMELINE")) {
        if (hipMalloc(&ctx->tl_base, (size_t)TL_MAX * TL_STRIDE * 8) != hipSuccess) return -9;
        hipMemset(ctx->tl_base, 0, (size_t)TL_MAX * TL_STRIDE * 8);
    }
    const bool gv = vv_gemm_route(&g, ctx->c.xsplit) == VV_ROUTE_GEMV;
    const bool want = gv ? ((g.T <= 4 || g.T != 16 || g.N > 16384) && (g.N + 15) / 16 <= 3200) : (g.T > 16);
    if (ctx->tl_base && ctx->tl_idx < TL_MAX && want) {
        g.dbg = ctx->tl_base + (size_t)ctx->tl_idx * TL_STRIDE;
        ctx->tl_rec.push_back({g.T, g.N, g.K, g.pro, gv ? g.epi : g.epi + 100});
        ctx->tl_idx++;
    }
    return vv_gemm_launch(g, ctx->c.xsplit, st);
}
extern "C" int vv_timeline_dump(vv_ctx* ctx, unsigned long long* out_host, int* meta_host, int max_launches) {
    VV_SHARED;
    hipDeviceSynchronize();
    const int n = std::min(max_launches, ctx->tl_idx);
    if (n > 0) hipMemcpy(out_host, ctx->tl_base, (size_t)n * TL_STRIDE * 8, hipMemcpyDeviceToHost);
    for (int i = 0; i < n; ++i) { const auto& r = ctx->tl_rec[i]; int* m = meta_host + 5 * i; m[0] = r.T; m[1] = r.N; m[2] = r.K; m[3] = r.pro; m[4] = r.epi; }
    return n;
}
#endif

extern "C" int vv_gemm_raw(void* stream, const void* w, const void* w2, const float* x, float* y, int T, int N, int K,
                           int ldx, int ldy, int pro, int epi, const float* nw, float eps, const float* bias,
                           const float* nscale, int xsplit, int ksplit, int nontemporal) {
    VVGemm g = mk_gemm(w, x, y, T, N, K, ldx, ldy);
    g.W2 = (const u32x4*)w2; g.pro = pro; g.epi = epi; g.nw = nw; g.eps = eps; g.bias = bias; g.nscale = nscale;
    g.ksplit = ksplit & 0xff; g.nt = 1;
    g.dbg = (unsigned long long*)(uintptr_t)0;
    if (nontemporal > 1) g.dbg = reinterpret_cast<unsigned long long*>(const_cast<float*>(nscale));
    if (g.dbg) g.nscale = nullptr;
    return vv_gemm_launch(g, xsplit, (hipStream_t)stream);
}
extern "C" int vv_gemv_case(void* stream, const vv_gemv_case_args* c, int xsplit, int* form_out) {
    if (!c || xsplit < 1 || xsplit > 3) return -1;
    VVGemm g = mk_gemm(c->W, c->X, c->Y, c->T, c->N, c->K, c->ldx, c->ldy);
    g.W2 = (const u32x4*)c->W2; g.pro = c->pro; g.epi = c->epi; g.nw = c->nw; g.eps = c->eps; g.bias = c->bias; g.nscale = c->nscale;
    g.mod_scale = c->mod_scale; g.mod_shift = c->mod_shift; g.ld_mod = c->ld_mod;
    g.addvec = c->addvec; g.x_row_mod = c->x_row_mod; g.add_rows_per_vec = c->add_rows_per_vec;
    g.gate = c->gate; g.ld_gate = c->ld_gate;
    g.z = c->z; g.x0p = c->x0p; g.coef = c->coef; g.cfg = c->cfg; g.n_cfg = c->n_cfg; g.sde_noise = c->sde_noise;
    g.cfg_rows = c->cfg_rows;
    g.kgrid = c->kgrid; g.yparts = c->yparts; g.xa = c->xa; g.n_xa = c->n_xa; g.ya = c->ya; g.n_ya = c->n_ya; g.part_stride = c->part_stride;
    g.sl_n = c->sl_n; g.sl_T = c->sl_T; g.sl_x = c->sl_x; g.sl_y = c->sl_y;
    for (int j = 0; j < 8; ++j) g.sl_id[j] = c->sl_id[j];
    g.dw_hist = c->dw_hist; g.dw_w = c->dw_w; g.dw_b = c->dw_b; g.dw_gamma = c->dw_gamma; g.dw_nw = c->dw_nw;
    g.dw_xout = c->dw_xout; g.dw_hnew = c->dw_hnew;
    g.nt = 1;
    if (!vv_gemv_ok(&g)) return VV_GEMV_REFUSED;
    int form[5] = {0, 0, 0, 0, 0};
    const int r = vv_gemv_launch(g, xsplit, (hipStream_t)stream, form);
    if (r == VV_RC_NO_FORM) return VV_GEMV_REFUSED;
    if (r == 0 && form_out) for (int j = 0; j < 5; ++j) form_out[j] = form[j];
    return r;
}
extern "C" int vv_gemm3_raw(vv_ctx* ctx, void* stream, const void* w, const void* w2, const float* x_dev, int T, int N, int K, int epi,
                            const float* nw_dev, float eps, const float* bias_dev, float* y_dev, void* xp_scratch, void* yp_scratch) {
    hipStream_t st = (hipStream_t)stream;
    if (ctx && ksplit_check(ctx, st)) return -1;
    int r = vv_pack_rows_launch(x_dev, K, nw_dev, eps, xp_scratch, T, K, st);
    if (r) return r;
    r = vv_gemm3_launch(w, w2, xp_scratch, y_dev, yp_scratch, bias_dev, T, N, K, N, epi, ctx ? &ctx->gws : nullptr, st);
    if (r) return r;
    if (epi == VV_EPI_SWIGLU) r = vv_unpack_rows_launch(yp_scratch, y_dev, T, N, st);
    return r;
}
extern "C" int vv_profile_begin(vv_ctx* ctx) {
    { VV_SHARED; HIPCHK(ctx, hipDeviceSynchronize()); }
    ctx->prof_on = true; ctx->prof_n = 0; ctx->prof_bytes = 0.0; ctx->prof_rec.clear();
    ctx->prof_gemv.clear(); ctx->prof_gemv_bytes = 0.0; ctx->prof_other.clear();
    return 0;
}
extern "C" int vv_profile_end(vv_ctx* ctx, int64_t* launches, double* total_ms, double* bytes) {
    { VV_SHARED; HIPCHK(ctx, hipDeviceSynchronize()); }
    double ms = 0.0, raw_ms = 0.0;
    int64_t n_other = 0; double ms_other = 0.0, by_other = 0.0;
    double ev_over = 0.0;
    {
        const int reps = 64;
        std::vector<hipEvent_t> ev(2 * reps);
        for (auto& e : ev) hipEventCreate(&e);
        hipStream_t ps = ctx->prof_stream;
        if (ctx->tmp1) vv_silu_launch(ctx->tmp1, 64, ps);
        for (int i = 0; i < reps; ++i) { hipEventRecord(ev[2 * i], ps); hipEventRecord(ev[2 * i + 1], ps); }
        hipStreamSynchronize(ps);
        std::vector<float> d(reps);
        for (int i = 0; i < reps; ++i) { d[i] = 0.f; hipEventElapsedTime(&d[i], ev[2 * i], ev[2 * i + 1]); }
        std::sort(d.begin(), d.end());
        ev_over = d[reps / 2];
        for (auto& e : ev) hipEventDestroy(e);
    }
    const char* csv = getenv("VVHIP_PROF_CSV");
    FILE* f = csv ? fopen(csv, "w") : nullptr;
    if (f) fprintf(f, "idx,T,N,K,pro,epi,dual,bytes,us\n");
    for (int i = 0; i < ctx->prof_n; ++i) {
        float e = 0.f;
        HIPCHK(ctx, hipEventElapsedTime(&e, ctx->prof_ev[2 * i], ctx->prof_ev[2 * i + 1]));
        if (ctx->prof_rec[i].gemv) raw_ms += e;
        e = (float)std::max(0.0, (double)e - ev_over);
        if (ctx->prof_rec[i].gemv) ms += e;
        else { n_other++; ms_other += e; by_other += ctx->prof_rec[i].bytes; }
        if (f) { const auto& r = ctx->prof_rec[i]; fprintf(f, "%d,%d,%d,%d,%d,%d,%d,%.0f,%.3f\n", i, r.T, r.N, r.K, r.pro, r.epi, r.dual, r.bytes, e * 1e3); }
    }
    if (f) fclose(f);
    if (launches) { launches[0] = ctx->prof_n - n_other; launches[1] = n_other; }
    if (total_ms) { total_ms[0] = ms; total_ms[1] = ms_other; }
    if (bytes) { bytes[0] = ctx->prof_bytes - by_other; bytes[1] = by_other; }
    ctx->prof_raw_ns = (int64_t)(raw_ms * 1e6); ctx->prof_ev_over_ns = (int64_t)(ev_over * 1e6);
    ctx->prof_on = false;
    return 0;
}
extern "C" int vv_profile_replay_family(vv_ctx* ctx, void* stream, int family, int reps, int64_t* launches, double* total_ms, double* bytes) {
    hipStream_t st = (hipStream_t)stream;
    if (ctx->prof_on) return fail(ctx, "vv_profile_replay: call vv_profile_end first");
    int64_t n = 0; double by = 0.0;
    if (family == 0) { n = (int64_t)ctx->prof_gemv.size(); by = ctx->prof_gemv_bytes; }
    else for (const auto& l : ctx->prof_other) if (l.family == family) { ++n; by += l.bytes; }
    if (launches) *launches = 0;
    if (total_ms) *total_ms = 0.0;
    if (bytes) *bytes = 0.0;
    if (n == 0) return family == 0 ? fail(ctx, "vv_profile_replay: the last profile window recorded no GEMV launches") : 0;
    if (reps < 1) reps = 1;
    HIPCHK(ctx, hipStreamSynchronize(st));
    hipGraph_t graph; hipGraphExec_t exec;
    HIPCHK(ctx, hipStreamBeginCapture(st, hipStreamCaptureModeRelaxed));
    int rr = 0;
    if (family == 0) { for (const VVGemm& g : ctx->prof_gemv) { rr = vv_gemm_launch(g, ctx->c.xsplit, st); if (rr) break; } }
    else for (const auto& l : ctx->prof_other) if (l.family == family) { rr = l.fn(st); if (rr) break; }
    hipError_t e = hipStreamEndCapture(st, &graph);
    if (rr) return fail(ctx, "vv_profile_replay: launch failed (%d)", rr);
    HIPCHK(ctx, e);
    HIPCHK(ctx, hipGraphInstantiate(&exec, graph, nullptr, nullptr, 0));
    hipGraphDestroy(graph);
    hipEvent_t e0, e1;
    hipEventCreate(&e0); hipEventCreate(&e1);
    HIPCHK(ctx, hipGraphLaunch(exec, st));
    HIPCHK(ctx, hipEventRecord(e0, st));
    for (int i = 0; i < reps; ++i) HIPCHK(ctx, hipGraphLaunch(exec, st));
    HIPCHK(ctx, hipEventRecord(e1, st));
    HIPCHK(ctx, hipStreamSynchronize(st));
    float ms = 0.f;
    HIPCHK(ctx, hipEventElapsedTime(&ms, e0, e1));
    hipEventDestroy(e0); hipEventDestroy(e1);
    hipGraphExecDestroy(exec);
    if (launches) *launches = n * reps;
    if (total_ms) *total_ms = ms;
    if (bytes) *bytes = by * reps;
    return 0;
}
extern "C" int vv_profile_replay(vv_ctx* ctx, void* stream, int reps, int64_t* launches, double* total_ms, double* bytes) {
    return vv_profile_replay_family(ctx, stream, 0, reps, launches, total_ms, bytes);
}
```

vibevoice_amd/csrc/misc.hip:

```cpp
#include "vv_common.h"
#include "vv_device.h"
#include "vv_launch.h"

namespace {

__global__ void vv_embed_kernel(const __bf16* __restrict__ table, const int* __restrict__ ids,
                                float* __restrict__ out, int H) {
    const int i = blockIdx.x;
    const __bf16* src = table + (int64_t)ids[i] * H;
    for (int k = threadIdx.x; k < H; k += blockDim.x) out[(int64_t)i * H + k] = (float)src[k];
}

template <int RPB>
__global__ __launch_bounds__(256) void vv_rmsnorm_rows_kernel(const float* __restrict__ x, int ldx, float* __restrict__ y, int ldy,
                                                              const float* __restrict__ w, int T, int C, float eps) {
    constexpr int NTH = 256 / RPB;
    constexpr int MAXV = (RPB == 1) ? 4 : 8;
    __shared__ float part[4];
    const int sub = threadIdx.x / NTH, tl = threadIdx.x % NTH;
    const int t = blockIdx.x * RPB + sub;
    const bool live = t < T;
    const float* xr = x + (int64_t)(live ? t : 0) * ldx;
    const bool vec = ((C & 3) == 0) && ((ldx & 3) == 0) && ((ldy & 3) == 0) && C <= NTH * 4 * MAXV;
    float4 v[MAXV];
// ... 170 lines not shown
    float4 wj[7];
#pragma unroll
    for (int j = 0; j < 7; ++j) wj[j] = *reinterpret_cast<const float4*>(w + (size_t)j * C + c4);
    const float4 bb = *reinterpret_cast<const float4*>(b + c4), gg = *reinterpret_cast<const float4*>(gamma + c4);
#pragma unroll
    for (int i = 0; i < RPW; ++i) {
        const int rr = wave * RPW + i, t = t0 - 6 + rr;
        if (rr >= RB + 6) break;
        float rs = 1.0f;
        const bool cur = (t >= 0 && t < T);
        if (cur) {
            float s = 0.f;
#pragma unroll
            for (int q = 0; q < NCH; ++q) s += v[i][q].x * v[i][q].x + v[i][q].y * v[i][q].y + v[i][q].z * v[i][q].z + v[i][q].w * v[i][q].w;
            rs = rsqrtf(vv_wave_sum(s) / (float)C + eps);
        }
        const bool keep = cur && (rr >= 6) && (t >= T - 6);
#pragma unroll
        for (int q = 0; q < NCH; ++q) {
            const int c = (q * 64 + lane) * 4;
            float4 o = v[i][q];
            if (cur) o = float4{o.x * rs * nwv[q].x, o.y * rs * nwv[q].y, o.z * rs * nwv[q].z, o.w * rs * nwv[q].w};
            *reinterpret_cast<float4*>(nrm_sh + (size_t)rr * C + c) = o;
            if (rr >= 6) *reinterpret_cast<float4*>(raw_sh + (size_t)(rr - 6) * C + c) = v[i][q];
            if (keep) *reinterpret_cast<float4*>(nb + (int64_t)(6 + t) * C + c) = o;
        }
    }
    __syncthreads();
    for (int e = tid; e < RB * C4; e += 256) {
        const int r = e / C4;
        const int t = t0 + r;
        if (t >= T) break;
        float4 acc = bb;
#pragma unroll
        for (int j = 0; j < 7; ++j) {
            const float4 nj = *reinterpret_cast<const float4*>(nrm_sh + (size_t)(r + j) * C + c4);
            acc.x += wj[j].x * nj.x; acc.y += wj[j].y * nj.y; acc.z += wj[j].z * nj.z; acc.w += wj[j].w * nj.w;
        }
        const float4 xv = *reinterpret_cast<const float4*>(raw_sh + (size_t)r * C + c4);
        *reinterpret_cast<float4*>(xout + (int64_t)t * C + c4) = float4{xv.x + gg.x * acc.x, xv.y + gg.y * acc.y, xv.z + gg.z * acc.z, xv.w + gg.w * acc.w};
    }
}

__device__ __forceinline__ float packed_w(const __bf16* __restrict__ wp, int KT, int n, int k) {
    return (float)wp[vv_packed_index((int64_t)(n >> 4) * KT + (k >> 5), n & 15, k)];
}

__global__ void vv_stem_conv_kernel(const float* __restrict__ in, const __bf16* __restrict__ wp, const float* __restrict__ bias,
                                    float* __restrict__ out, int T, int N, const VVSlotIds sl, int64_t s_in, int64_t s_out) {
    const int e = blockIdx.x * blockDim.x + threadIdx.x;
    if (e >= T * N) return;
    if (sl.n > 0) { const int64_t id = vv_slot_id(sl.id, blockIdx.y); in += id * s_in; out += id * s_out; }
    const int t = e / N, n = e - t * N;
    float acc = bias[n];
#pragma unroll
    for (int j = 0; j < 7; ++j) acc += packed_w(wp, 1, n, j) * in[t + j];
    out[e] = acc;
}

__global__ __launch_bounds__(256) void vv_head_conv1_kernel(const float* __restrict__ x, const __bf16* __restrict__ wp,
                                                            const float* __restrict__ bias, float* __restrict__ out, int T, int Cin,
                                                            const VVSlotIds sl, int64_t s_in, int64_t s_out) {
    extern __shared__ float wsh[];
    if (sl.n > 0) { x += (int64_t)vv_slot_id(sl.id, blockIdx.y) * s_in; out += (int64_t)blockIdx.y * s_out; }
    const int K = 7 * Cin, KT = (K + 31) >> 5;
    for (int k = threadIdx.x; k < K; k += 256) wsh[k] = packed_w(wp, KT, 0, k);
    __syncthreads();
    const int g = blockIdx.x * 64 + (threadIdx.x >> 2), part = threadIdx.x & 3;
    float acc = 0.f;
    if (g < T) {
        const float* xr = x + (int64_t)g * Cin;
        for (int k = part * 4; k < K; k += 16) {
            const float4 v = *reinterpret_cast<const float4*>(xr + k);
            acc += v.x * wsh[k] + v.y * wsh[k + 1] + v.z * wsh[k + 2] + v.w * wsh[k + 3];
        }
    }
    acc += __shfl_xor(acc, 1);
    acc += __shfl_xor(acc, 2);
    if (g < T && part == 0) out[g] = acc + bias[0];
}

struct VVShift { float* buf; int T, hist, C; };
__global__ void vv_shift_rows_kernel(const VVShift* __restrict__ tab) {
    const VVShift e = tab[blockIdx.x];
    for (int c = blockIdx.y * blockDim.x + threadIdx.x; c < e.C; c += gridDim.y * blockDim.x)
        for (int r = 0; r < e.hist; ++r) e.buf[(int64_t)r * e.C + c] = e.buf[(int64_t)(r + e.T) * e.C + c];
}

__global__ void vv_zero_hist_kernel(const VVShift* __restrict__ tab) {
    const VVShift e = tab[blockIdx.x];
    const int64_t n = (int64_t)e.hist * e.C;
    for (int64_t i = blockIdx.y * blockDim.x + threadIdx.x; i < n; i += (int64_t)gridDim.y * blockDim.x) e.buf[i] = 0.f;
}

__global__ void vv_affine_kernel(const float* __restrict__ x, float* __restrict__ y, float mul, float add, int n) {
    const int i = blockIdx.x * blockDim.x + threadIdx.x;
    if (i < n) y[i] = x[i] * mul + add;
}

__global__ void vv_copy_words_kernel(const unsigned* __restrict__ src, unsigned* __restrict__ dst, size_t n) {
    for (size_t i = (size_t)blockIdx.x * blockDim.x + threadIdx.x; i < n; i += (size_t)gridDim.x * blockDim.x) dst[i] = src[i];
}
__global__ void vv_copy_quads_kernel(const uint4* __restrict__ src, uint4* __restrict__ dst, size_t n) {
    for (size_t i = (size_t)blockIdx.x * blockDim.x + threadIdx.x; i < n; i += (size_t)gridDim.x * blockDim.x) dst[i] = src[i];
}
__global__ void vv_zero_words_kernel(unsigned* __restrict__ dst, size_t n) {
    for (size_t i = (size_t)blockIdx.x * blockDim.x + threadIdx.x; i < n; i += (size_t)gridDim.x * blockDim.x) dst[i] = 0u;
}
__global__ void vv_sampler_init_kernel(const float* __restrict__ noise, float* __restrict__ z, float* __restrict__ x0p, int nL) {
    const int i = blockIdx.x * blockDim.x + threadIdx.x;
    if (i < nL) { const float v = noise[i]; z[i] = v; z[nL + i] = v; x0p[i] = 0.f; }
}

__global__ void vv_tfreq_kernel(const float* __restrict__ t, float* __restrict__ out, int n) {
    const int i = blockIdx.x, k = threadIdx.x;
    const float f = expf(-logf(10000.f) * (float)k / 128.f);
    const float arg = t[i] * f;
    out[i * 256 + k] = cosf(arg);
    out[i * 256 + 128 + k] = sinf(arg);
}

__global__ void vv_add_rows_kernel(const float* __restrict__ x, const float* __restrict__ v, float* __restrict__ y, int n, int C) {
    const int i = blockIdx.x * blockDim.x + threadIdx.x;
    if (i < n * C) y[i] = x[i] + v[i % C];
}
__global__ void vv_relu_kernel(float* __restrict__ x, int n) {
    const int i = blockIdx.x * blockDim.x + threadIdx.x;
    if (i < n) x[i] = fmaxf(x[i], 0.f);
}
template <typename ST>
__global__ void vv_kv_import_kernel(const ST* __restrict__ k, const ST* __restrict__ v, __bf16* __restrict__ kc,
                                    __bf16* __restrict__ vc, int L, int D, int64_t head_stride, int pos0) {
    const int h = blockIdx.y, d = threadIdx.x;
    const int64_t si = ((int64_t)h * L + blockIdx.x) * D + d;
    const int pos = pos0 + (int)blockIdx.x;
    __bf16* kb = kc + (int64_t)h * head_stride;
    __bf16* vb = vc + (int64_t)h * head_stride;
    {
        const int64_t tile = (int64_t)(pos >> 4) * (D / 32) + (d >> 5);
        const int ln = (pos & 15) + 16 * ((d & 31) >> 3);
        kb[(tile * 64 + ln) * 8 + (d & 7)] = (__bf16)(float)k[si];
    }
    {
        const int p = pos & 31, half = p >> 4, pp = p & 15, q4 = pp >> 2, rr = pp & 3;
        const int64_t tile = (int64_t)(pos >> 5) * (D / 16) + (d >> 4);
        const int ln = (d & 15) + 16 * q4;
        vb[(tile * 64 + ln) * 8 + half * 4 + rr] = (__bf16)(float)v[si];
    }
}

__global__ void vv_kv_move_kernel(__bf16* __restrict__ kc, __bf16* __restrict__ vc, int D, int64_t layer_stride, int64_t head_stride,
                                  int src, int dst) {
    const int d = threadIdx.x;
    __bf16* kb = kc + (int64_t)blockIdx.x * layer_stride + (int64_t)blockIdx.y * head_stride;
    __bf16* vb = vc + (int64_t)blockIdx.x * layer_stride + (int64_t)blockIdx.y * head_stride;
    auto kidx = [&](int pos) {
        const int64_t tile = (int64_t)(pos >> 4) * (D / 32) + (d >> 5);
        return vv_packed_index(tile, pos & 15, d);
    };
    auto vidx = [&](int pos) {
        const int p = pos & 31, half = p >> 4, pp = p & 15, q4 = pp >> 2, rr = pp & 3;
        const int64_t tile = (int64_t)(pos >> 5) * (D / 16) + (d >> 4);
        return (tile * 64 + (d & 15) + 16 * q4) * 8 + half * 4 + rr;
    };
    kb[kidx(dst)] = kb[kidx(src)];
    vb[vidx(dst)] = vb[vidx(src)];
}

__global__ void vv_kv_zero_v_tail_kernel(__bf16* __restrict__ vc, const VVRow* __restrict__ rows, int R, int D, int64_t cache_stride,
                                         int64_t layer_stride, int64_t head_stride, int max_ctx) {
    const int d = threadIdx.x;
    const VVRow last = rows[R - 1];
    const int p0 = last.pos + 1;
    const int p1 = min(max_ctx, (p0 + 63) & ~63);
    __bf16* vb = vc + (int64_t)last.cache * cache_stride + (int64_t)blockIdx.x * layer_stride + (int64_t)blockIdx.y * head_stride;
    for (int pos = p0; pos < p1; ++pos) {
        const int p = pos & 31, half = p >> 4, pp = p & 15, q4 = pp >> 2, rr = pp & 3;
        const int64_t tile = (int64_t)(pos >> 5) * (D / 16) + (d >> 4);
        vb[(tile * 64 + (d & 15) + 16 * q4) * 8 + half * 4 + rr] = (__bf16)0.0f;
    }
}

__global__ __launch_bounds__(256) void vv_pcm16_kernel(const float* __restrict__ x, short* __restrict__ out, int samples) {
    const float* xr = x + (size_t)blockIdx.x * samples;
    short* orow = out + (size_t)blockIdx.x * samples;
    float mx = 0.f;
    for (int i = threadIdx.x; i < samples; i += 256) mx = fmaxf(mx, fabsf(xr[i]));
#pragma unroll
    for (int o = 32; o >= 1; o >>= 1) mx = fmaxf(mx, __shfl_xor(mx, o));
    __shared__ float wmx[4];
    if ((threadIdx.x & 63) == 0) wmx[threadIdx.x >> 6] = mx;
    __syncthreads();
    const float peak = fmaxf(fmaxf(wmx[0], wmx[1]), fmaxf(wmx[2], wmx[3]));
    for (int i = threadIdx.x; i < samples; i += 256) {
        float v = xr[i];
        if (peak > 1.0f) v = __fdiv_rn(v, peak);
        orow[i] = (short)(int)__fmul_rn(v, 32767.0f);
    }
}

__global__ void vv_ada_in_kernel(const float* __restrict__ cproj, const float* __restrict__ temb, float* __restrict__ out,
                                 int rows, int n_steps, int H) {
    const int q = blockIdx.x * blockDim.x + threadIdx.x;
    const int H4 = H >> 2;
    if (q >= rows * n_steps * H4) return;
    const int t = q / H4, k4 = q - t * H4;
    const int i = t / rows, r = t - i * rows;
    const float4 c = reinterpret_cast<const float4*>(cproj)[r * H4 + k4];
    const float4 e = reinterpret_cast<const float4*>(temb)[i * H4 + k4];
    float4 o;
    float u;
    u = c.x + e.x; o.x = vv_silu(u);
    u = c.y + e.y; o.y = vv_silu(u);
    u = c.z + e.z; o.z = vv_silu(u);
    u = c.w + e.w; o.w = vv_silu(u);
    reinterpret_cast<float4*>(out)[q] = o;
}

__global__ void vv_silu_kernel(float* __restrict__ x, int n) {
    const int i = blockIdx.x * blockDim.x + threadIdx.x;
    if (i < n) x[i] = vv_silu(x[i]);
}

__global__ void vv_cvt_bf16_to_f32_kernel(const __bf16* __restrict__ s, float* __restrict__ d, int64_t n) {
    for (int64_t i = (int64_t)blockIdx.x * blockDim.x + threadIdx.x; i < n; i += (int64_t)gridDim.x * blockDim.x) d[i] = (float)s[i];
}
__global__ void vv_cvt_f32_to_bf16_kernel(const float* __restrict__ s, __bf16* __restrict__ d, int64_t n) {
    for (int64_t i = (int64_t)blockIdx.x * blockDim.x + threadIdx.x; i < n; i += (int64_t)gridDim.x * blockDim.x) d[i] = (__bf16)s[i];
}
__global__ void vv_dw_transpose_kernel(const float* __restrict__ s, float* __restrict__ d, int C) {
    const int i = blockIdx.x * blockDim.x + threadIdx.x;
    if (i < C * 7) { const int c = i / 7, j = i - c * 7; d[j * C + c] = s[i]; }
}

__global__ __launch_bounds__(256) void vv_logits_full_kernel(const __bf16* __restrict__ table, const float* __restrict__ hidden,
                                                             float* __restrict__ out, int n, int V, int H) {
    const int lane = threadIdx.x & 63;
    const int v = blockIdx.x * 4 + (threadIdx.x >> 6);
    if (v >= V) return;
    const __bf16* wrow = table + (int64_t)v * H;
    float acc[16];
#pragma unroll
    for (int r = 0; r < 16; ++r) acc[r] = 0.f;
    for (int k = lane * 8; k < H; k += 512) {
        const u32x4 wv = *reinterpret_cast<const u32x4*>(wrow + k);
        const bf16x8 w8 = __builtin_bit_cast(bf16x8, wv);
        float wf[8];
#pragma unroll
        for (int j = 0; j < 8; ++j) wf[j] = (float)w8[j];
#pragma unroll
        for (int r = 0; r < 16; ++r) {
            if (r < n) {
                const float4 a = *reinterpret_cast<const float4*>(hidden + (int64_t)r * H + k);
                const float4 b = *reinterpret_cast<const float4*>(hidden + (int64_t)r * H + k + 4);
                acc[r] += a.x * wf[0] + a.y * wf[1] + a.z * wf[2] + a.w * wf[3] + b.x * wf[4] + b.y * wf[5] + b.z * wf[6] + b.w * wf[7];
            }
        }
    }
#pragma unroll
    for (int r = 0; r < 16; ++r) {
        if (r < n) {
            float t = acc[r];
#pragma unroll
            for (int o = 32; o > 0; o >>= 1) t += __shfl_xor(t, o);
            if (lane == 0) out[(int64_t)r * V + v] = t;
        }
    }
}

}

static inline int okk() { return vv_launch_rc(0); }

extern "C" {

int vv_logits_full_launch(const void* table, const float* hidden, float* out, int n, int V, int H, hipStream_t s) {
    if (n < 1 || n > 16 || V < 1 || (H & 7)) return -1;
    hipLaunchKernelGGL(vv_logits_full_kernel, dim3((V + 3) / 4), dim3(256), 0, s, (const __bf16*)table, hidden, out, n, V, H);
    return okk();
}
int vv_embed_launch(const void* table, const int* ids, float* out, int n, int H, hipStream_t s) {
    hipLaunchKernelGGL(vv_embed_kernel, dim3(n), dim3(256), 0, s, (const __bf16*)table, ids, out, H);
    return okk();
}
int vv_rmsnorm_rows_launch(const float* x, int ldx, float* y, int ldy, const float* w, int T, int C, float eps, hipStream_t s) {
    if (C > 1024 || T < 64)
        hipLaunchKernelGGL((vv_rmsnorm_rows_kernel<1>), dim3(T), dim3(256), 0, s, x, ldx, y, ldy, w, T, C, eps);
    else
        hipLaunchKernelGGL((vv_rmsnorm_rows_kernel<4>), dim3((T + 3) / 4), dim3(256), 0, s, x, ldx, y, ldy, w, T, C, eps);
    return okk();
}
int vv_dwconv_res_launch(const float* nb, const float* x, float* xo, const float* w, const float* b, const float* gamma, int T, int C, hipStream_t s) {
    int64_t total = (int64_t)T * C;
    int blocks = (int)((total + 255) / 256);
    if (blocks > 4096) blocks = 4096;
    hipLaunchKernelGGL(vv_dwconv_res_kernel, dim3(blocks), dim3(256), 0, s, nb, x, xo, w, b, gamma, T, C);
    return okk();
}
int vv_normdw_launch(float* x, float* nb, const float* nw, const float* w, const float* b, const float* gamma,
                     int T, int C, float eps, hipStream_t s) {
    hipLaunchKernelGGL(vv_normdw_kernel, dim3(1), dim3(1024), 0, s, x, nb, nw, w, b, gamma, T, C, eps);
    return okk();
}
int vv_normdw_sliced_ok(int T, int C) { return T >= 1 && T <= 8 && (C == 1024 || C == 2048); }
int vv_normdw_sliced_slots_launch(const float* xin, float* xout, float* nb, const float* nw, const float* w, const float* b,
                                  const float* gamma, int T, int C, float eps, const int* ids, int n, int64_t sx, int64_t snb,
                                  hipStream_t s) {
    if (!vv_normdw_sliced_ok(T, C) || xin == xout || n < 0 || n > 8) return -1;
    const VVSlotIds sl = vv_slot_ids(ids, n);
    const dim3 grid(C / 256, sl.n > 0 ? sl.n : 1);
    if (C == 1024) hipLaunchKernelGGL((vv_normdw_sliced_kernel<1>), grid, dim3(256), 0, s, xin, xout, nb, nw, w, b, gamma, T, C, eps, sl, sx, snb);
    else hipLaunchKernelGGL((vv_normdw_sliced_kernel<2>), grid, dim3(256), 0, s, xin, xout, nb, nw, w, b, gamma, T, C, eps, sl, sx, snb);
    return okk();
}
static __global__ void vv_affine_slots_kernel(const float* __restrict__ x, float* __restrict__ y, float mul, float add, int L,
                                       const VVSlotIds sl, int64_t stride) {
    const int j = blockIdx.y, c = blockIdx.x * blockDim.x + threadIdx.x;
    if (c < L) y[(int64_t)vv_slot_id(sl.id, j) * stride + c] = x[(int64_t)j * L + c] * mul + add;
}
int vv_affine_slots_launch(const float* x, float* y, float mul, float add, int L, const int* ids, int n, int64_t stride, hipStream_t s) {
    if (n < 1 || n > 8) return -1;
    const VVSlotIds sl = vv_slot_ids(ids, n);
    hipLaunchKernelGGL(vv_affine_slots_kernel, dim3((L + 255) / 256, n), dim3(256), 0, s, x, y, mul, add, L, sl, stride);
    return okk();
}
int vv_normdw_rows_ok(int T, int C) { return T >= 1 && (C == 256 || C == 512 || C == 1024); }
int vv_normdw_rows_slots_launch(const float* xin, float* xout, float* nb, const float* nw, const float* w, const float* b,
                                const float* gamma, int T, int C, float eps, const int* ids, int n, int64_t sx, int64_t snb,
                                hipStream_t s) {
    if (!vv_normdw_rows_ok(T, C) || xin == xout || n < 0 || n > 8) return -1;
    constexpr int RB = 8;
    const size_t smem = (size_t)(2 * RB + 6) * C * 4;
    const VVSlotIds sl = vv_slot_ids(ids, n);
    const dim3 grid((T + RB - 1) / RB, sl.n > 0 ? sl.n : 1);
    static const hipError_t lds = vv_raise_lds_limit(160 * 1024, &vv_normdw_rows_kernel<RB, 4>);
    (void)lds;
    if (C == 256) hipLaunchKernelGGL((vv_normdw_rows_kernel<RB, 1>), grid, dim3(256), smem, s, xin, xout, nb, nw, w, b, gamma, T, C, eps, sl, sx, snb);
    else if (C == 512) hipLaunchKernelGGL((vv_normdw_rows_kernel<RB, 2>), grid, dim3(256), smem, s, xin, xout, nb, nw, w, b, gamma, T, C, eps, sl, sx, snb);
    else hipLaunchKernelGGL((vv_normdw_rows_kernel<RB, 4>), grid, dim3(256), smem, s, xin, xout, nb, nw, w, b, gamma, T, C, eps, sl, sx, snb);
    return okk();
}
int vv_stem_conv_slots_launch(const float* in, const void* wp, const float* bias, float* out, int T, int N, const int* ids, int n,
                              int64_t s_in, int64_t s_out, hipStream_t s) {
    if (n < 0 || n > 8) return -1;
    const VVSlotIds sl = vv_slot_ids(ids, n);
    hipLaunchKernelGGL(vv_stem_conv_kernel, dim3((T * N + 255) / 256, sl.n > 0 ? sl.n : 1), dim3(256), 0, s, in, (const __bf16*)wp, bias, out, T, N, sl, s_in, s_out);
    return okk();
}
int vv_head_conv1_slots_launch(const float* x, const void* wp, const float* bias, float* out, int T, int Cin, const int* ids, int n,
                               int64_t s_in, int64_t s_out, hipStream_t s) {
    if ((Cin & 3) || (((uintptr_t)x) & 15) || 7 * Cin * 4 > 48 * 1024 || n < 0 || n > 8 || (s_in & 3)) return -1;
    const VVSlotIds sl = vv_slot_ids(ids, n);
    hipLaunchKernelGGL(vv_head_conv1_kernel, dim3((T + 63) / 64, sl.n > 0 ? sl.n : 1), dim3(256), (size_t)7 * Cin * 4, s, x, (const __bf16*)wp, bias, out, T, Cin, sl, s_in, s_out);
    return okk();
}
int vv_shift_rows_launch(const void* tab, int n_entries, int maxC, hipStream_t s) {
    int cy = (maxC + 255) / 256; if (cy < 1) cy = 1; if (cy > 16) cy = 16;
    hipLaunchKernelGGL(vv_shift_rows_kernel, dim3(n_entries, cy), dim3(256), 0, s, (const VVShift*)tab);
    return okk();
}
int vv_zero_hist_launch(const void* tab, int n_entries, hipStream_t s) {
    hipLaunchKernelGGL(vv_zero_hist_kernel, dim3(n_entries, 8), dim3(256), 0, s, (const VVShift*)tab);
    return okk();
}
int vv_affine_launch(const float* x, float* y, float mul, float add, int n, hipStream_t s) {
    hipLaunchKernelGGL(vv_affine_kernel, dim3((n + 255) / 256), dim3(256), 0, s, x, y, mul, add, n);
    return okk();
}
int vv_copy_launch(void* dst, const void* src, size_t bytes, hipStream_t s) {
    if (bytes == 0) return 0;
    if ((bytes & 3) || ((uintptr_t)dst & 3) || ((uintptr_t)src & 3)) { g_vv_launch_err = (int)hipErrorInvalidValue; return -1; }
    if (!(bytes & 15) && !((uintptr_t)dst & 15) && !((uintptr_t)src & 15)) {
        const size_t n = bytes >> 4;
        hipLaunchKernelGGL(vv_copy_quads_kernel, dim3((unsigned)std::min<size_t>((n + 255) / 256, 4096)), dim3(256), 0, s, (const uint4*)src, (uint4*)dst, n);
    } else {
        const size_t n = bytes >> 2;
        hipLaunchKernelGGL(vv_copy_words_kernel, dim3((unsigned)std::min<size_t>((n + 255) / 256, 4096)), dim3(256), 0, s, (const unsigned*)src, (unsigned*)dst, n);
    }
    return okk();
}
int vv_zero_launch(void* dst, size_t bytes, hipStream_t s) {
    if (bytes == 0) return 0;
    if ((bytes & 3) || ((uintptr_t)dst & 3)) { g_vv_launch_err = (int)hipErrorInvalidValue; return -1; }
    const size_t n = bytes >> 2;
    hipLaunchKernelGGL(vv_zero_words_kernel, dim3((unsigned)std::min<size_t>((n + 255) / 256, 4096)), dim3(256), 0, s, (unsigned*)dst, n);
    return okk();
}
int vv_sampler_init_launch(const float* noise, float* z, float* x0p, int nL, hipStream_t s) {
    hipLaunchKernelGGL(vv_sampler_init_kernel, dim3((nL + 255) / 256), dim3(256), 0, s, noise, z, x0p, nL);
    return okk();
}
int vv_tfreq_launch(const float* t, float* out, int n, hipStream_t s) {
    hipLaunchKernelGGL(vv_tfreq_kernel, dim3(n), dim3(128), 0, s, t, out, n);
    return okk();
}
int vv_add_rows_launch(const float* x, const float* v, float* y, int n, int C, hipStream_t s) {
    hipLaunchKernelGGL(vv_add_rows_kernel, dim3((n * C + 255) / 256), dim3(256), 0, s, x, v, y, n, C);
    return okk();
}
int vv_relu_launch(float* x, int n, hipStream_t s) {
    hipLaunchKernelGGL(vv_relu_kernel, dim3((n + 255) / 256), dim3(256), 0, s, x, n);
    return okk();
}
int vv_kv_import_launch(const void* k, const void* v, int src_bf16, void* kc, void* vc, int L, int Hkv, int D,
                        int64_t head_stride, int pos0, hipStream_t s) {
    if (src_bf16) hipLaunchKernelGGL((vv_kv_import_kernel<__bf16>), dim3(L, Hkv), dim3(D), 0, s, (const __bf16*)k, (const __bf16*)v, (__bf16*)kc, (__bf16*)vc, L, D, head_stride, pos0);
    else hipLaunchKernelGGL((vv_kv_import_kernel<float>), dim3(L, Hkv), dim3(D), 0, s, (const float*)k, (const float*)v, (__bf16*)kc, (__bf16*)vc, L, D, head_stride, pos0);
    return okk();
}
int vv_kv_move_launch(void* kc, void* vc, int layers, int Hkv, int D, int64_t layer_stride, int64_t head_stride, int src, int dst, hipStream_t s) {
    hipLaunchKernelGGL(vv_kv_move_kernel, dim3(layers, Hkv), dim3(D), 0, s, (__bf16*)kc, (__bf16*)vc, D, layer_stride, head_stride, src, dst);
    return okk();
}
int vv_kv_zero_v_tail_launch(void* vc, const VVRow* rows, int R, int layers, int Hkv, int D, int64_t cache_stride, int64_t layer_stride,
                             int64_t head_stride, int max_ctx, hipStream_t s) {
    hipLaunchKernelGGL(vv_kv_zero_v_tail_kernel, dim3(layers, Hkv), dim3(D), 0, s, (__bf16*)vc, rows, R, D, cache_stride, layer_stride, head_stride, max_ctx);
    return okk();
}
int vv_pcm16_launch(const float* x, short* out, int n, int samples, hipStream_t s) {
    hipLaunchKernelGGL(vv_pcm16_kernel, dim3(n), dim3(256), 0, s, x, out, samples);
    return okk();
}
int vv_ada_in_launch(const float* cproj, const float* temb, float* out, int rows, int n_steps, int H, hipStream_t s) {
    if (H & 3) return -1;
    const int n4 = rows * n_steps * (H >> 2);
    hipLaunchKernelGGL(vv_ada_in_kernel, dim3((n4 + 255) / 256), dim3(256), 0, s, cproj, temb, out, rows, n_steps, H);
    return vv_launch_rc(0);
}
int vv_silu_launch(float* x, int n, hipStream_t s) {
    hipLaunchKernelGGL(vv_silu_kernel, dim3((n + 255) / 256), dim3(256), 0, s, x, n);
    return okk();
}
int vv_cvt_launch(const void* src, void* dst, int64_t n, int to_bf16, hipStream_t s) {
    int blocks = (int)((n + 255) / 256); if (blocks > 8192) blocks = 8192; if (blocks < 1) blocks = 1;
    if (to_bf16) hipLaunchKernelGGL(vv_cvt_f32_to_bf16_kernel, dim3(blocks), dim3(256), 0, s, (const float*)src, (__bf16*)dst, n);
    else hipLaunchKernelGGL(vv_cvt_bf16_to_f32_kernel, dim3(blocks), dim3(256), 0, s, (const __bf16*)src, (float*)dst, n);
    return okk();
}
int vv_dw_transpose_launch(const float* src, float* dst, int C, hipStream_t s) {
    hipLaunchKernelGGL(vv_dw_transpose_kernel, dim3((C * 7 + 255) / 256), dim3(256), 0, s, src, dst, C);
    return okk();
}

}
```

vibevoice_amd/csrc/vv_launch.h:

```cpp
#pragma once
#include "vv_common.h"
#include "gemv_plan.h"

struct VVSolverStep {
    const float* eps;
    const float* z_in; const float* m1_in; const float* m2_in;
    float* z_out; float* m1_out; float* m2_out;
    const float* coef;
    float cfg; const float* cfg_rows;
    const float* noise;
    int n, L;
    const u32x4* Win;
    float* Xout;
    int H, xs;
};
extern "C" {
int vv_gemm_launch(VVGemm a, int xs, hipStream_t s);
int vv_pack_launch(const void* src, int src_is_bf16, void* dst, int N, int K, int kind, int Cin, int Cout, int ksz, int stride, hipStream_t s);
int vv_rope_append_launch(int D, const float* qkv, const VVRow* rows, const float* inv_freq, float* q_out, void* kc, void* vc, int R, int Hq, int Hkv,
                          int64_t cache_stride, int64_t head_stride, hipStream_t s);
int vv_rope_table_launch(const float* inv_freq, void* tab, int n_pos, int half, hipStream_t s);
int vv_attn_fused_launch(int D, int xs, const float* qkv, const VVRow* rows, const void* rope_tab, void* kc, void* vc, int R, int Hq, int Hkv,
                         int64_t cache_stride, int64_t head_stride, int S, float* pm, float* pl, float* po, float* out, void* out_packed,
                         hipStream_t s);
int vv_attn_launch(int D, int xs, const float* q, const VVRow* rows, const void* kc, const void* vc, int R, int Hq, int Hkv, int64_t cache_stride,
                   int64_t head_stride, int S, float* pm, float* pl, float* po, float* out, hipStream_t s);
int vv_embed_launch(const void* table, const int* ids, float* out, int n, int H, hipStream_t s);
int vv_logits_full_launch(const void* table, const float* hidden, float* out, int n, int V, int H, hipStream_t s);
int vv_warp_valid_launch(const float* logits, const unsigned char* seen, float* out, int* survivors, int n, int V, const int* ids, int n_valid,
                         float pen, float temp, int do_sample, int top_k, float top_p, float min_p, hipStream_t s);
int vv_noise_rows_launch(float* out, int n, const uint32_t* keys, uint32_t stream0, int n_streams, int n_t, int width, hipStream_t s);
int vv_rmsnorm_rows_launch(const float* x, int ldx, float* y, int ldy, const float* w, int T, int C, float eps, hipStream_t s);
int vv_dwconv_res_launch(const float* nb, const float* x, float* xo, const float* w, const float* b, const float* gamma, int T, int C, hipStream_t s);
int vv_normdw_sliced_ok(int T, int C);
int vv_normdw_sliced_slots_launch(const float* xin, float* xout, float* nb, const float* nw, const float* w, const float* b, const float* gamma,
                                  int T, int C, float eps, const int* ids, int n, int64_t sx, int64_t snb, hipStream_t s);
int vv_normdw_rows_slots_launch(const float* xin, float* xout, float* nb, const float* nw, const float* w, const float* b, const float* gamma, int T,
                                int C, float eps, const int* ids, int n, int64_t sx, int64_t snb, hipStream_t s);
int vv_stem_conv_slots_launch(const float* in, const void* wp, const float* bias, float* out, int T, int N, const int* ids, int n, int64_t s_in,
                              int64_t s_out, hipStream_t s);
int vv_head_conv1_slots_launch(const float* x, const void* wp, const float* bias, float* out, int T, int Cin, const int* ids, int n, int64_t s_in,
                               int64_t s_out, hipStream_t s);
int vv_block1d_slots_launch(int C, int xs, const float* xin, float* xout, float* nst, const float* norm_w, const float* ffn_norm_w,
                            const float* gamma, const float* ffn_gamma, const float* dw_w, const float* dw_b, const float* b1, const float* b2,
                            const void* w1, const void* w2, int T, float eps, const int* ids, int n, int64_t sx, int64_t snst, hipStream_t s);
int vv_affine_slots_launch(const float* x, float* y, float mul, float add, int L, const int* ids, int n, int64_t stride, hipStream_t s);
int vv_normdw_launch(float* x, float* nb, const float* nw, const float* w, const float* b, const float* gamma, int T, int C, float eps,
                     hipStream_t s);
int vv_normdw_rows_ok(int T, int C);
int vv_shift_rows_launch(const void* tab, int n_entries, int maxC, hipStream_t s);
int vv_zero_hist_launch(const void* tab, int n_entries, hipStream_t s);
int vv_affine_launch(const float* x, float* y, float mul, float add, int n, hipStream_t s);
int vv_copy_launch(void* dst, const void* src, size_t bytes, hipStream_t s);
int vv_zero_launch(void* dst, size_t bytes, hipStream_t s);
int vv_sampler_init_launch(const float* noise, float* z, float* x0p, int nL, hipStream_t s);
int vv_tfreq_launch(const float* t, float* out, int n, hipStream_t s);
int vv_silu_launch(float* x, int n, hipStream_t s);
int vv_ada_in_launch(const float* cproj, const float* temb, float* out, int rows, int n_steps, int H, hipStream_t s);
int vv_add_rows_launch(const float* x, const float* v, float* y, int n, int C, hipStream_t s);
int vv_relu_launch(float* x, int n, hipStream_t s);
int vv_kv_import_launch(const void* k, const void* v, int src_bf16, void* kc, void* vc, int L, int Hkv, int D, int64_t head_stride, int pos0,
                        hipStream_t s);
int vv_kv_move_launch(void* kc, void* vc, int layers, int Hkv, int D, int64_t layer_stride, int64_t head_stride, int src, int dst, hipStream_t s);
int vv_kv_zero_v_tail_launch(void* vc, const VVRow* rows, int R, int layers, int Hkv, int D, int64_t cache_stride, int64_t layer_stride,
                             int64_t head_stride, int max_ctx, hipStream_t s);
int vv_kv_span_copy_launch(void* kc, void* vc, void* ks, void* vs, int to_cache, int layers, int Hkv, int D, int64_t layer_stride,
                           int64_t head_stride, int n_pos, hipStream_t s);
int vv_kv_export_launch(const void* kc, const void* vc, void* k, void* v, int dst_bf16, int L, int Hkv, int D, int64_t head_stride, int pos0,
                        hipStream_t s);
int vv_pcm16_launch(const float* x, short* out, int n, int samples, hipStream_t s);
int vv_cvt_launch(const void* src, void* dst, int64_t n, int to_bf16, hipStream_t s);
int vv_dw_transpose_launch(const float* src, float* dst, int C, hipStream_t s);
int vv_pack_rows_launch(const float* x, int ldx, const float* nw, float eps, void* xp, int T, int K, hipStream_t s);
int vv_unpack_rows_launch(const void* xp, float* x, int T, int K, hipStream_t s);
int vv_pack16_launch(const float* x, int ldx, int mode, const float* nw, float eps, const float* sc, const float* sh, int ld_mod, void* xp, int T,
                     int K, hipStream_t s);
int vv_gemv16p_launch(const void* W, const void* W2, const void* Xp, float* Y, void* Yp, const float* bias, const float* gate, int T, int N, int K,
                      int ldy, int ld_gate, int epi, hipStream_t s);
int vv_gemv16p_launch2(const VVGemv16p* a, int epi, int flags, hipStream_t s);
int vv_head_tail_ok(const VVTail* a);
int vv_head_tail_init();
int vv_head_tail_launch(const VVTail* a, hipStream_t s);
int vv_solver_step_ok(const VVSolverStep* a);
int vv_solver_step_fused_ok(const VVSolverStep* a);
int vv_solver_step_launch(const VVSolverStep* a, hipStream_t s);
int vv_pack16_tiles_launch(const float* x, int ldx, int64_t stride_outer, int n_inner, int64_t stride_inner, void* xp, int64_t tile_bytes, int T,
                           int K, int n_tiles, hipStream_t s);
int vv_ada_pack_launch(const float* cproj, const float* temb, void* xp, int rows, int n_steps, int H, hipStream_t s);
int vv_gemm3_launch(const void* W, const void* W2, const void* Xp, float* Y, void* Yp, const float* bias, int T, int N, int K, int ldy, int epi,
                    const VVGemmWs* ws, hipStream_t s);
int vv_gemm_qkv_rope_launch(const void* W, const void* Xp, const float* bias, int T, int K, int D, int Hq, int Hkv, const VVRow* rows_dev,
                            const void* rope_tab, float* q_out, void* kc, void* vc, int64_t cache_stride, int64_t head_stride, const VVGemmWs* ws,
                            hipStream_t s);
int vv_attn_prefill4_launch(int D, const float* q, const VVRow* rows, const void* kc, const void* vc, int R, int Hq, int Hkv, int64_t cache_stride,
                            int64_t head_stride, float* out, void* out_packed, hipStream_t s);
int vv_block1d_supported(int C);
int vv_gemv_ok(const VVGemm* a);
int vv_gemv_launch(VVGemm a, int xs, hipStream_t s, int* form);
int vv_tile_ok(const VVGemm* a, int xs);
int vv_tile_launch(VVGemm a, int xs, hipStream_t s);
int vv_lora_merge_launch(const void* base, void* dst, int N, int K, const float* a, const float* b, int r, float scale, int delta_bf16,
                         hipStream_t s);
int vv_unpack_launch(const void* packed, float* dst, int N, int K, hipStream_t s);
int vv_resample_lds_bytes(int L, int T, int n_in);
int vv_resample_rows_launch(const VVRsRows* rows, int n, int L, int M, int T, const float* coef, float* hist, int n_streams, const float* x,
                            int ld_in, void* out, int ld_out, int pcm16, hipStream_t s);
int vv_resample_once_launch(int L, int M, int T, const float* coef, int n, int n_in, const float* x, int ld_in, float* out, int ld_out, hipStream_t s);
int vv_resample_reset_launch(float* hist, int T, int n_streams, const int* ids, int n, hipStream_t s);
int vv_tempo_rows_launch(const VVTpRows* rows, int n, const float* window, float* hist, int* dstate, int n_streams, const float* x, int ld_in,
                         void* out, int ld_out, int pcm16, int* offsets, int ld_off, hipStream_t s);
int vv_tempo_once_launch(const float* window, int P, int Q, int n, int n_in, const float* x, int ld_in, float* out, int ld_out, int* offsets,
                         int ld_off, hipStream_t s);
int vv_tempo_reset_launch(float* hist, int* dstate, int n_streams, const int* ids, int n, hipStream_t s);
}
```

vibevoice_amd/engine.py:

```python
import ctypes as C
from dataclasses import dataclass, field
from typing import Dict, List, Optional, Sequence

import numpy as np
import torch

from . import _lib
from . import schedule as _schedule


@dataclass
class EngineConfig:
    lm_hidden: int
    lm_layers: int
    lm_heads: int
    lm_kv_heads: int
    lm_inter: int
    lm_vocab: int
    lm_head_dim: Optional[int] = None
    lm_eps: float = 1e-6
    rope_theta: float = 1e6
    head_layers: int = 4
    head_ffn_ratio: float = 3.0
    latent_dim: int = 64
# ... 483 lines not shown
        from . import tempo as _tp
        w = self.__dict__.get("_tp_window")
        if w is None:
            w = self.__dict__["_tp_window"] = torch.from_numpy(np.array(_tp.window())).to(self.device)
        return w

    def time_stretch(self, audio: torch.Tensor, speed: float, stream=None, return_offsets: bool = False):
        from . import tempo as _tp
        P, Q = _tp.ratio(speed)
        x = audio.detach().to(device=self.device, dtype=torch.float32)
        if x.dim() not in (1, 2):
            raise ValueError(f"Engine.time_stretch: audio is [samples] or [n, samples], got {tuple(audio.shape)}")
        x2 = x.reshape(-1, x.shape[-1]).contiguous()
        n, n_in = x2.shape
        n_out = _tp.total_out(n_in, P, Q)
        nblk = -(-n_out // _tp.HS)
        out = torch.empty((n, n_out), dtype=torch.float32, device=self.device)
        offs = torch.zeros((n, max(nblk, 1)), dtype=torch.int32, device=self.device) if return_offsets else None
        if n and n_in:
            w = self._tempo_window()
            st = stream if stream is not None else torch.cuda.current_stream(self.device)
            for i0 in range(0, n, 65535):
                nn = min(65535, n - i0)
                self._chk(self.lib.vv_tempo_once(self._ctx, self._sp(st), self._p(w), P, Q, nn, n_in, self._p(x2[i0:]), n_in, self._p(out[i0:]),
                                                 n_out, self._p(offs[i0:]) if offs is not None else None, max(nblk, 1)), "vv_tempo_once")
        out = out.reshape(x.shape[:-1] + (n_out,))
        return (out, offs[:, :nblk].reshape(x.shape[:-1] + (nblk,))) if return_offsets else out

    def codec_reset(self, slot: int):
        self._chk(self.lib.vv_codec_reset(self._ctx, self._s, slot), "vv_codec_reset")

    def connect(self, n: int, latent: torch.Tensor, sem: Optional[torch.Tensor], out: torch.Tensor):
        self._chk(self.lib.vv_connect(self._ctx, self._s, n, self._p(latent), self._p(sem), self._p(out)), "vv_connect")

    def profile_begin(self):
        self._chk(self.lib.vv_profile_begin(self._ctx), "vv_profile_begin")

    def profile_end(self):
        n, ms, by = (C.c_int64 * 2)(), (C.c_double * 2)(), (C.c_double * 2)()
        self._chk(self.lib.vv_profile_end(self._ctx, n, ms, by), "vv_profile_end")
        return (n[0], ms[0], by[0]), (n[1], ms[1], by[1])

    def profile_replay(self, reps=3, family=0):
        n, ms, by = C.c_int64(), C.c_double(), C.c_double()
        self._chk(self.lib.vv_profile_replay_family(self._ctx, self._s, int(family), int(reps), C.byref(n), C.byref(ms), C.byref(by)),
                  "vv_profile_replay_family")
        return n.value, ms.value, by.value

    def stat(self, what=0):
        return int(self.lib.vv_stat(self._ctx, what))

    def pack_matrix(self, w: torch.Tensor) -> torch.Tensor:
        N, K = w.shape
        out = torch.empty(int(self.lib.vv_packed_bytes(N, K)), dtype=torch.uint8, device=self.device)
        w = w.to(self.device, torch.float32).contiguous()
        with torch.cuda.stream(self.stream):
            rc = self.lib.vv_pack_matrix(self._s, self._p(w), self._p(out), N, K)
        if rc != 0:
            raise EngineError("vv_pack_matrix failed")
        self.sync()
        return out

    MERGE_DTYPES = ("float32", "bfloat16")

    def _dev_tensor(self, what, name, t, numel, dtype=torch.float32, unaligned_ok=False):
        if not isinstance(t, torch.Tensor) or t.device != self.device:
            raise ValueError(f"{what}: {name} is not a tensor on {self.device}")
        if t.dtype != dtype:
            raise ValueError(f"{what}: {name} is {t.dtype}, expected {dtype}")
        if not t.is_contiguous():
            raise ValueError(f"{what}: {name} is not contiguous")
        if t.data_ptr() % 16 and not unaligned_ok:
            raise ValueError(f"{what}: {name} is not 16-byte aligned")
        if t.numel() < numel:
            raise ValueError(f"{what}: {name} holds {t.numel()} elements, the launch addresses {numel}")

    @staticmethod
    def _shape_ints(what, **ints):
        for k, v in ints.items():
            if not isinstance(v, (int, np.integer)) or isinstance(v, bool) or v < 1 or v >= (1 << 30):
                raise ValueError(f"{what}: {k} = {v!r} is not an int in [1, 2^30)")

    def _delta_flag(self, what, merge_dtype):
        if merge_dtype not in self.MERGE_DTYPES:
            raise ValueError(f"{what}: merge_dtype must be one of {self.MERGE_DTYPES}, got {merge_dtype!r}")
        return 1 if merge_dtype == "bfloat16" else 0

    def _raw_err(self):
        s = self.lib.vv_last_error(None)
        return s.decode() if s else "?"

    def _mat_shape(self, name):
        tab = self.__dict__.setdefault("_mat_shapes", {})
        if name not in tab:
            n, k = C.c_int(), C.c_int()
            tab[name] = (n.value, k.value) if self.lib.vv_weight_shape(self._ctx, name.encode(), C.byref(n), C.byref(k)) == 0 else None
        return tab[name]

    def _after_producer(self):
        self.stream.wait_stream(torch.cuda.current_stream(self.device))

    def unpack_matrix(self, packed: torch.Tensor, N: int, K: int, out: Optional[torch.Tensor] = None) -> torch.Tensor:
        self._shape_ints("unpack_matrix", N=N, K=K)
        self._dev_tensor("unpack_matrix", "packed", packed, int(self.lib.vv_packed_bytes(N, K)), torch.uint8)
        if out is None:
            with torch.cuda.stream(self.stream):
                out = torch.empty(N, K, dtype=torch.float32, device=self.device)
        self._dev_tensor("unpack_matrix", "out", out, N * K)
        self._after_producer()
        if self.lib.vv_unpack_matrix(self._s, self._p(packed), self._p(out), int(N), int(K)) != 0:
            raise EngineError("vv_unpack_matrix failed: " + self._raw_err())
        return out

    def lora_merge_raw(self, base_packed: torch.Tensor, dst_packed: torch.Tensor, N: int, K: int, a: torch.Tensor, b: torch.Tensor,
                       scale: float, merge_dtype: str = "float32", unaligned_ok=()):
        what = "lora_merge_raw"
        self._shape_ints(what, N=N, K=K)
        flag = self._delta_flag(what, merge_dtype)
        if not isinstance(a, torch.Tensor) or not isinstance(b, torch.Tensor) or a.dim() != 2 or b.dim() != 2:
            raise ValueError(f"{what}: a and b are 2-D tensors")
        r = int(a.shape[0])
        if tuple(a.shape) != (r, K) or tuple(b.shape) != (N, r):
            raise ValueError(f"{what}: a {tuple(a.shape)} / b {tuple(b.shape)} do not factor an [{N}, {K}] matrix")
        nb = int(self.lib.vv_packed_bytes(N, K))
        self._dev_tensor(what, "base_packed", base_packed, nb, torch.uint8, "base_packed" in unaligned_ok)
        self._dev_tensor(what, "dst_packed", dst_packed, nb, torch.uint8, "dst_packed" in unaligned_ok)
        self._dev_tensor(what, "a", a, r * K, unaligned_ok="a" in unaligned_ok)
        self._dev_tensor(what, "b", b, N * r, unaligned_ok="b" in unaligned_ok)
        self._after_producer()
        if self.lib.vv_lora_merge_raw(self._s, self._p(base_packed), self._p(dst_packed), int(N), int(K), self._p(a), self._p(b), r,
                                      float(scale), flag) != 0:
            raise EngineError("vv_lora_merge_raw failed: " + self._raw_err())

    def weight_read(self, name: str, shape: Sequence[int]) -> torch.Tensor:
        nk = self._mat_shape(name)
        if nk is not None and tuple(int(v) for v in shape) != nk:
            raise ValueError(f"weight_read({name}): shape {tuple(shape)}, the parameter is {nk}")
        with torch.cuda.stream(self.stream):
            out = torch.empty(*[int(v) for v in shape], dtype=torch.float32, device=self.device)
        self._chk(self.lib.vv_weight_read(self._ctx, self._s, name.encode(), self._p(out)), f"vv_weight_read({name})")
        return out

    def lora_merge(self, name: str, a: torch.Tensor, b: torch.Tensor, scale: float, merge_dtype: str = "float32", unaligned_ok=()):
        what = f"lora_merge({name})"
        flag = self._delta_flag(what, merge_dtype)
        if not isinstance(a, torch.Tensor) or not isinstance(b, torch.Tensor) or a.dim() != 2 or b.dim() != 2 or a.shape[0] != b.shape[1]:
            raise ValueError(f"{what}: a [r, K] and b [N, r] are 2-D tensors with one r")
        r, K, N = int(a.shape[0]), int(a.shape[1]), int(b.shape[0])
        nk = self._mat_shape(name)
        if nk is not None and (N, K) != nk:
            raise ValueError(f"{what}: b @ a is [{N}, {K}], the parameter is {list(nk)}")
        self._dev_tensor(what, "a", a, r * K, unaligned_ok="a" in unaligned_ok)
        self._dev_tensor(what, "b", b, N * r, unaligned_ok="b" in unaligned_ok)
        self._after_producer()
        self._chk(self.lib.vv_lora_merge(self._ctx, self._s, name.encode(), self._p(a), self._p(b), r, float(scale), flag),
                  f"vv_lora_merge({name})")
        if name.startswith("head."):
            self._n_steps = None

    def lora_reset(self, name: Optional[str] = None):
        self._chk(self.lib.vv_lora_reset(self._ctx, self._s, name.encode() if name is not None else None), f"vv_lora_reset({name})")
        if name is None or name.startswith("head."):
            self._n_steps = None

    def gemm3_raw(self, wp, x, y, N, K, epi=0, w2p=None, nw=None, eps=1e-6, bias=None, ksplit=True):
        T = x.shape[0]
        xp = torch.zeros(int(self.lib.vv_packed_bytes(T, K)), dtype=torch.uint8, device=self.device)
        yp = torch.zeros(int(self.lib.vv_packed_bytes(T, N)), dtype=torch.uint8, device=self.device)
        torch.cuda.synchronize(self.device)
        rc = self.lib.vv_gemm3_raw(self._ctx if ksplit else None, self._s, self._p(wp), self._p(w2p), self._p(x), T, N, K, epi, self._p(nw), float(eps),
                                   self._p(bias), self._p(y), self._p(xp), self._p(yp))
        if rc != 0:
            raise EngineError(f"vv_gemm3_raw failed ({rc})")
        self.sync()

    def gemm_raw(self, wp, x, y, N, K, T=None, ldx=None, ldy=None, pro=0, epi=0, w2p=None, nw=None, eps=1e-6,
                 bias=None, nscale=None, xsplit=None, ksplit=0, nontemporal=0):
        T = x.shape[0] if T is None else T
        rc = self.lib.vv_gemm_raw(self._s, self._p(wp), self._p(w2p), self._p(x), self._p(y), T, N, K,
                                  ldx or K, ldy or N, pro, epi, self._p(nw), float(eps), self._p(bias),
                                  self._p(nscale), xsplit or self.cfg.xsplit, ksplit, nontemporal)
        if rc != 0:
            raise EngineError(f"vv_gemm_raw failed ({rc})")

    PRO_NONE, PRO_RMS, PRO_RMS_MOD, PRO_ADD_SILU, PRO_NORMDW = 0, 1, 2, 3, 4
    EPI_STORE, EPI_BIAS, EPI_BIAS_GELU, EPI_SWIGLU, EPI_RESID, EPI_GATED_RESID, EPI_CFG_DPM = 0, 1, 2, 3, 4, 5, 6

    def gemv_case(self, wp, x, y, T, N, K, *, ldx=None, ldy=None, pro=0, epi=0, w2p=None, nw=None, eps=1e-6, bias=None, nscale=None,
                  mod_scale=None, mod_shift=None, ld_mod=0, addvec=None, x_row_mod=0, add_rows_per_vec=0, gate=None, ld_gate=0,
                  z=None, x0p=None, coef=None, cfg=0.0, n_cfg=0, sde_noise=None, cfg_rows=None,
                  kgrid=0, yparts=None, xa=None, n_xa=0, ya=None, n_ya=0, part_stride=0,
                  sl_n=0, sl_T=0, sl_x=0, sl_y=0, sl_id=(),
                  dw_hist=None, dw_w=None, dw_b=None, dw_gamma=None, dw_nw=None, dw_xout=None, dw_hnew=None,
                  xsplit=None, unaligned_ok=()):
        ldx = K if ldx is None else ldx
        ldy = N if ldy is None else ldy
        xs = self.cfg.xsplit if xsplit is None else xsplit
        ints = dict(T=T, N=N, K=K, ldx=ldx, ldy=ldy, pro=pro, epi=epi, ld_mod=ld_mod, x_row_mod=x_row_mod, add_rows_per_vec=add_rows_per_vec,
                    ld_gate=ld_gate, n_cfg=n_cfg, kgrid=kgrid, n_xa=n_xa, n_ya=n_ya, part_stride=part_stride, sl_n=sl_n, sl_T=sl_T,
                    sl_x=sl_x, sl_y=sl_y, xsplit=xs)
        for k, v in ints.items():
            if not isinstance(v, (int, np.integer)) or isinstance(v, bool) or v < 0 or v >= (1 << 30):
                raise ValueError(f"gemv_case: {k} = {v!r} is not an int in [0, 2^30)")
        if T < 1 or N < 1 or K < 1:
            raise ValueError(f"gemv_case: T, N, K = {T}, {N}, {K} must be positive")
        if xs not in (1, 2, 3):
            raise ValueError(f"gemv_case: xsplit = {xs}")
        if not 0 <= pro <= 4 or not 0 <= epi <= 6:
            raise ValueError(f"gemv_case: pro = {pro}, epi = {epi}")
        if ldx < K or ldy < N:
            raise ValueError(f"gemv_case: ldx = {ldx} < K = {K} or ldy = {ldy} < N = {N}")
        sl_id = [int(v) for v in sl_id]
        if sl_n > 8 or len(sl_id) < sl_n or len(sl_id) > 8 or any(v < 0 or v >= (1 << 20) for v in sl_id):
            raise ValueError(f"gemv_case: sl_n = {sl_n}, sl_id = {sl_id}")
        if sl_n > 0 and (sl_T < 1 or T != sl_n * sl_T):
            raise ValueError(f"gemv_case: T = {T} is not sl_n * sl_T = {sl_n} * {sl_T}")
        if sl_n == 0 and (sl_T or sl_x or sl_y or sl_id):
            raise ValueError("gemv_case: slot fields without sl_n")

        def need(name, t, numel, dtype=torch.float32, required=True):
            if t is None:
                if required:
                    raise ValueError(f"gemv_case: {name} is required here")
                return
            if not isinstance(t, torch.Tensor) or t.device != self.device:
                raise ValueError(f"gemv_case: {name} is not a tensor on {self.device}")
            if t.dtype != dtype:
                raise ValueError(f"gemv_case: {name} is {t.dtype}, expected {dtype}")
            if not t.is_contiguous():
                raise ValueError(f"gemv_case: {name} is not contiguous")
            if t.data_ptr() % 16 and name not in unaligned_ok:
                raise ValueError(f"gemv_case: {name} is not 16-byte aligned")
            if t.numel() < numel:
                raise ValueError(f"gemv_case: {name} holds {t.numel()} elements, the launch addresses {numel}")

        def extent(rows, ld, width, slot_stride):
            if sl_n > 0 and slot_stride > 0:
                return max(sl_id[:sl_n]) * slot_stride + (sl_T - 1) * ld + width
            return (rows - 1) * ld + width
        x_rows = x_row_mod if x_row_mod > 0 else T
        x_need = extent(x_rows, ldx, K, sl_x)
        y_need = extent(T, ldy, N, sl_y)
        wbytes = int(self.lib.vv_packed_bytes(N, K))
        need("wp", wp, wbytes, torch.uint8)
        need("w2p", w2p, wbytes, torch.uint8, required=epi == self.EPI_SWIGLU)
        need("x", x, x_need)
        need("y", y, y_need, required=epi != self.EPI_CFG_DPM)
        need("nw", nw, K, required=False)
        need("bias", bias, N, required=False)
        need("nscale", nscale, N, required=False)
        is_mod = pro == self.PRO_RMS_MOD
        if is_mod and ld_mod < K:
            raise ValueError(f"gemv_case: ld_mod = {ld_mod} < K = {K}")
        need("mod_scale", mod_scale, (T - 1) * ld_mod + K, required=is_mod)
        need("mod_shift", mod_shift, (T - 1) * ld_mod + K, required=is_mod)
        n_vec = (T - 1) // add_rows_per_vec + 1 if add_rows_per_vec > 0 else 1
        need("addvec", addvec, n_vec * K, required=pro == self.PRO_ADD_SILU)
        is_gated = epi == self.EPI_GATED_RESID
        if is_gated and ld_gate < N:
            raise ValueError(f"gemv_case: ld_gate = {ld_gate} < N = {N}")
        need("gate", gate, (T - 1) * ld_gate + N, required=is_gated)
        is_cfg = epi == self.EPI_CFG_DPM
        if is_cfg and n_cfg < 1:
            raise ValueError("gemv_case: the CFG epilogue needs n_cfg >= 1")
        need("z", z, 2 * n_cfg * N, required=is_cfg)
        need("x0p", x0p, n_cfg * N, required=is_cfg)
        need("coef", coef, 6, required=is_cfg)
        need("sde_noise", sde_noise, n_cfg * N, required=False)
        need("cfg_rows", cfg_rows, n_cfg, required=False)
        if (kgrid > 1 or n_xa or n_ya) and part_stride < max(x_need if n_xa else 0, y_need if (kgrid > 1 or n_ya) else 0):
            raise ValueError(f"gemv_case: part_stride = {part_stride} is smaller than one part tensor")
        need("yparts", yparts, (kgrid - 2) * part_stride + y_need if kgrid > 1 else 0, required=kgrid > 1)
        need("xa", xa, (max(n_xa, 2) - 1) * part_stride + x_need, required=n_xa > 0)
        need("ya", ya, (max(n_ya, 2) - 1) * part_stride + y_need, required=n_ya > 0)
        is_dw = pro == self.PRO_NORMDW
        for name, t, rows in (("dw_hist", dw_hist, 6), ("dw_w", dw_w, 7), ("dw_b", dw_b, 1), ("dw_gamma", dw_gamma, 1), ("dw_nw", dw_nw, 1),
                              ("dw_xout", dw_xout, 1), ("dw_hnew", dw_hnew, 1)):
            need(name, t, rows * K, required=is_dw)

        a = _lib.VVGemvCase()
        p = lambda t: t.data_ptr() if t is not None else None
        a.W, a.W2, a.X, a.Y = p(wp), p(w2p), p(x), p(y)
        a.T, a.N, a.K, a.ldx, a.ldy, a.pro, a.epi = T, N, K, ldx, ldy, pro, epi
        a.nw, a.eps, a.bias, a.nscale = p(nw), float(eps), p(bias), p(nscale)
        a.mod_scale, a.mod_shift, a.ld_mod = p(mod_scale), p(mod_shift), ld_mod
        a.addvec, a.x_row_mod, a.add_rows_per_vec = p(addvec), x_row_mod, add_rows_per_vec
        a.gate, a.ld_gate = p(gate), ld_gate
        a.z, a.x0p, a.coef, a.cfg, a.n_cfg, a.sde_noise = p(z), p(x0p), p(coef), float(cfg), n_cfg, p(sde_noise)
        a.kgrid, a.yparts, a.xa, a.n_xa, a.ya, a.n_ya, a.part_stride = kgrid, p(yparts), p(xa), n_xa, p(ya), n_ya, part_stride
        a.sl_n, a.sl_T, a.sl_x, a.sl_y = sl_n, sl_T, sl_x, sl_y
        for j, v in enumerate(sl_id):
            a.sl_id[j] = v
        a.dw_hist, a.dw_w, a.dw_b, a.dw_gamma, a.dw_nw = p(dw_hist), p(dw_w), p(dw_b), p(dw_gamma), p(dw_nw)
        a.dw_xout, a.dw_hnew = p(dw_xout), p(dw_hnew)
        a.cfg_rows = p(cfg_rows)
        form = (C.c_int * 5)()
        rc = self.lib.vv_gemv_case(self._s, C.byref(a), xs, form)
        if rc == _lib.GEMV_REFUSED:
            return None
        if rc != 0:
            raise EngineError(f"vv_gemv_case failed ({rc})")
        return tuple(form)


class TempoCapacityError(EngineError):
    """A Tempo.push row that brings more input, or emits more output, than one launch takes per row; nothing ran, no state changed:
    push it in pieces."""


class Tempo:

    def __init__(self, engine: Engine, slot: int, n_streams: int):
        from . import tempo as _tp
        self.engine, self.slot, self.n_streams = engine, slot, int(n_streams)
        self.delay_samples, self.max_in = _tp.delay_samples(), 7680
        self.total = [0] * self.n_streams
        self.ratio = [None] * self.n_streams
        w = np.ascontiguousarray(_tp.window())
        engine._chk(engine.lib.vv_tempo_set(engine._ctx, slot, C.c_void_p(w.ctypes.data), self.n_streams, engine._s), "vv_tempo_set")

    def counts(self, stream_id: int, n_in: int, speed=None, flush: bool = False) -> int:
        from . import tempo as _tp
        P, Q = self.ratio[stream_id] or _tp.ratio(speed)
        return _tp.counts(P, Q, self.total[stream_id], n_in, flush)[1]

    def max_out(self, n_in: int) -> int:
        return 2 * (int(n_in) + 880) + 1

    def push(self, audio: Optional[torch.Tensor], stream_ids: Sequence[int], speeds, flush=False, out: Optional[torch.Tensor] = None,
             n_in=None, stream=None, pcm16: bool = False, return_offsets: bool = False):
        from . import tempo as _tp
        e = self.engine
        ids = [int(i) for i in stream_ids]
        n = len(ids)
        samples = 0 if audio is None else int(audio.shape[-1])
        if audio is not None:
            if audio.dim() != 2 or audio.dtype != torch.float32 or not audio.is_contiguous() or audio.device != e.device or audio.shape[0] < n:
                raise ValueError(f"Tempo.push: audio is a contiguous fp32 [n >= {n}, samples] tensor on {e.device}")
        nin = [samples] * n if n_in is None else [int(v) for v in n_in]
        fl = [bool(flush)] * n if isinstance(flush, (bool, int)) else [bool(v) for v in flush]
        sp = [speeds] * n if not hasattr(speeds, "__len__") else list(speeds)
        if len(nin) != n or len(fl) != n or len(sp) != n:
            raise ValueError("Tempo.push: n_in, flush and speeds name one value per row")
        pq = [_tp.ratio(v) for v in sp]
        dt = torch.int16 if pcm16 else torch.float32
        if out is None:
            out = torch.empty((max(n, 1), self.max_out(max(nin, default=0))), dtype=dt, device=e.device)
        elif out.dim() != 2 or out.dtype != dt or not out.is_contiguous() or out.device != e.device or out.shape[0] < n:
            raise ValueError(f"Tempo.push: out is a contiguous {dt} [n >= {n}, capacity] tensor on {e.device}")
        cap = int(out.shape[1])
        ld_off = -(-cap // _tp.HS)
        offs = torch.zeros((max(n, 1), ld_off), dtype=torch.int32, device=e.device) if return_offsets else None
        st = stream if stream is not None else torch.cuda.current_stream(e.device)
        cnts = (C.c_int * max(n, 1))()
        rows = (_lib.VVTempoRow * max(n, 1))()
        for i in range(n):
            rows[i].stream, rows[i].n_in, rows[i].flush, rows[i].P, rows[i].Q = ids[i], nin[i], int(fl[i]), pq[i][0], pq[i][1]
        for i0 in range(0, n, 16):
            nn = min(16, n - i0)
            a = C.c_void_p(audio.data_ptr() + i0 * samples * 4) if audio is not None else C.c_void_p()
            o = C.c_void_p(out.data_ptr() + i0 * cap * out.element_size())
            f = C.c_void_p(offs.data_ptr() + i0 * ld_off * 4) if offs is not None else C.c_void_p()
            rc = e.lib.vv_tempo_rows(e._ctx, e._sp(st), self.slot, nn, C.cast(C.byref(rows, i0 * C.sizeof(_lib.VVTempoRow)), C.POINTER(_lib.VVTempoRow)),
                                     a, samples, o, cap, int(pcm16), C.cast(C.byref(cnts, i0 * 4), C.POINTER(C.c_int)), f, ld_off)
            if rc == _lib.TEMPO_OVER_CAPACITY:
                raise TempoCapacityError(f"Tempo.push: {e._err()}")
            e._chk(rc, "vv_tempo_rows")
            for i in range(i0, i0 + nn):
                self.total[ids[i]] += nin[i]
                self.ratio[ids[i]] = pq[i]
        res = [int(cnts[i]) for i in range(n)]
        return (out, res, offs) if return_offsets else (out, res)

    def reset(self, ids: Optional[Sequence[int]] = None, stream=None):
        e = self.engine
        st = stream if stream is not None else torch.cuda.current_stream(e.device)
        if ids is None:
            e._chk(e.lib.vv_tempo_reset(e._ctx, e._sp(st), self.slot, 0, None), "vv_tempo_reset")
            self.total, self.ratio = [0] * self.n_streams, [None] * self.n_streams
            return
        arr = (C.c_int * max(1, len(ids)))(*[int(i) for i in ids])
        e._chk(e.lib.vv_tempo_reset(e._ctx, e._sp(st), self.slot, len(ids), arr), "vv_tempo_reset")
        for i in ids:
            self.total[int(i)], self.ratio[int(i)] = 0, None

    def close(self):
        used = getattr(self.engine, "_tp_used", None)
        if used is not None and used[self.slot] is self:
            used[self.slot] = None


class Resampler:

    def __init__(self, engine: Engine, slot: int, src_rate: int, dst_rate: int, n_streams: int):
        from . import resample as _rs
        self.engine, self.slot = engine, slot
        self.src_rate, self.dst_rate, self.n_streams = int(src_rate), int(dst_rate), int(n_streams)
        self.L, self.M, self.T, coef = _rs.design(src_rate, dst_rate)
        self.taps, self.delay_samples = self.T, _rs.delay_samples(self.T)
        self.total = [0] * self.n_streams
        c = np.ascontiguousarray(coef)
        engine._chk(engine.lib.vv_resampler_set(engine._ctx, slot, self.L, self.M, self.T, C.c_void_p(c.ctypes.data), self.n_streams,
                                                engine._s), "vv_resampler_set")

    def counts(self, stream_id: int, n_in: int, flush: bool = False) -> int:
        from . import resample as _rs
        return _rs.counts(self.L, self.M, self.T, self.total[stream_id], n_in, flush)[1]

    def max_out(self, n_in: int) -> int:
        return -((-(int(n_in) + self.delay_samples + 1) * self.L) // self.M) + 1

    def push(self, audio: Optional[torch.Tensor], stream_ids: Sequence[int], flush=False, out: Optional[torch.Tensor] = None,
             pcm16: bool = False, n_in=None, stream=None):
        e = self.engine
        ids = [int(i) for i in stream_ids]
        n = len(ids)
        samples = 0 if audio is None else int(audio.shape[-1])
        if audio is not None:
            if audio.dim() != 2 or audio.dtype != torch.float32 or not audio.is_contiguous() or audio.device != e.device or audio.shape[0] < n:
                raise ValueError(f"Resampler.push: audio is a contiguous fp32 [n >= {n}, samples] tensor on {e.device}")
        nin = [samples] * n if n_in is None else [int(v) for v in n_in]
        fl = [bool(flush)] * n if isinstance(flush, (bool, int)) else [bool(v) for v in flush]
        if len(nin) != n or len(fl) != n:
            raise ValueError("Resampler.push: n_in and flush name one value per row")
        dt = torch.int16 if pcm16 else torch.float32
        if out is None:
            out = torch.empty((max(n, 1), self.max_out(max(nin, default=0))), dtype=dt, device=e.device)
        elif out.dim() != 2 or out.dtype != dt or not out.is_contiguous() or out.device != e.device or out.shape[0] < n:
            raise ValueError(f"Resampler.push: out is a contiguous {dt} [n >= {n}, capacity] tensor on {e.device}")
        st = stream if stream is not None else torch.cuda.current_stream(e.device)
        cnts = (C.c_int * max(n, 1))()
        rows = (_lib.VVResampleRow * max(n, 1))()
        for i in range(n):
            rows[i].stream, rows[i].n_in, rows[i].flush = ids[i], nin[i], int(fl[i])
        cap = int(out.shape[1])
        for i0 in range(0, max(n, 1), 16):
            nn = min(16, n - i0)
            a = C.c_void_p(audio.data_ptr() + i0 * samples * 4) if audio is not None else C.c_void_p()
            o = C.c_void_p(out.data_ptr() + i0 * cap * out.element_size())
            e._chk(e.lib.vv_resample_rows(e._ctx, e._sp(st), self.slot, nn, C.cast(C.byref(rows, i0 * C.sizeof(_lib.VVResampleRow)), C.POINTER(_lib.VVResampleRow)),
                                          a, samples, o, cap, int(pcm16), C.cast(C.byref(cnts, i0 * 4), C.POINTER(C.c_int))), "vv_resample_rows")
            for i in range(i0, i0 + nn):
                self.total[ids[i]] += nin[i]
        return out, [int(cnts[i]) for i in range(n)]

    def reset(self, ids: Optional[Sequence[int]] = None, stream=None):
        e = self.engine
        st = stream if stream is not None else torch.cuda.current_stream(e.device)
        if ids is None:
            e._chk(e.lib.vv_resampler_reset(e._ctx, e._sp(st), self.slot, 0, None), "vv_resampler_reset")
            self.total = [0] * self.n_streams
            return
        arr = (C.c_int * max(1, len(ids)))(*[int(i) for i in ids])
        e._chk(e.lib.vv_resampler_reset(e._ctx, e._sp(st), self.slot, len(ids), arr), "vv_resampler_reset")
        for i in ids:
            self.total[int(i)] = 0

    def close(self):
        used = getattr(self.engine, "_rs_used", None)
        if used is not None and used[self.slot] is self:
            used[self.slot] = None
```

Baseline: 16.49.

## Fuse all ConvNeXt 1D blocks of a codec stage into one kernel

Adds a stage-level block1d kernel that runs several consecutive depthwise-conv/FFN blocks of a codec stage in one launch. Each block recomputes a shrinking row window with halos and keeps intermediates in LDS instead of writing them to global memory between blocks. It also moves the per-stage kernel choice into a shared codec plan (route enum). This cuts launches and global round trips in the codec, at the cost of extra halo recompute, more LDS and more code.

```diff
diff --git a/include/vvhip.h b/include/vvhip.h
--- a/include/vvhip.h
+++ b/include/vvhip.h
@@ -142,6 +142,8 @@
     const float* cfg_rows;
 } vv_gemv_case_args;
 int vv_gemv_case(void* stream, const vv_gemv_case_args* args, int xsplit, int* form_out);
+int vv_block1d_case(void* stream, int stage, int C, int xsplit, int nb, const float* xin_dev, float* xout_dev, float* nst_dev,
+                    const float* prm_dev, const void* const* w1_packed, const void* const* w2_packed, int T, float eps);
 int vv_gemm3_raw(vv_ctx* ctx, void* stream, const void* w_packed_dev, const void* w2_packed_dev, const float* x_dev, int T, int N, int K,
                  int epi, const float* nw_dev, float eps, const float* bias_dev, float* y_dev, void* xp_scratch, void* yp_scratch);
 int vv_profile_begin(vv_ctx* ctx);
diff --git a/vibevoice_amd/_lib.py b/vibevoice_amd/_lib.py
--- a/vibevoice_amd/_lib.py
+++ b/vibevoice_amd/_lib.py
@@ -120,6 +120,7 @@
     "vv_gemm_raw": (C.c_int, [_P, _P, _P, _P, _P, C.c_int, C.c_int, C.c_int, C.c_int, C.c_int, C.c_int, C.c_int,
                               _P, C.c_float, _P, _P, C.c_int, C.c_int, C.c_int]),
     "vv_gemv_case": (C.c_int, [_P, C.POINTER(VVGemvCase), C.c_int, C.POINTER(C.c_int)]),
+    "vv_block1d_case": (C.c_int, [_P, C.c_int, C.c_int, C.c_int, C.c_int, _P, _P, _P, _P, C.POINTER(_P), C.POINTER(_P), C.c_int, C.c_float]),
     "vv_gemm3_raw": (C.c_int, [_P, _P, _P, _P, _P, C.c_int, C.c_int, C.c_int, C.c_int, _P, C.c_float, _P, _P, _P, _P]),
     "vv_profile_begin": (C.c_int, [_P]),
     "vv_profile_end": (C.c_int, [_P, C.POINTER(C.c_int64), C.POINTER(C.c_double), C.POINTER(C.c_double)]),
diff --git a/vibevoice_amd/build.py b/vibevoice_amd/build.py
--- a/vibevoice_amd/build.py
+++ b/vibevoice_amd/build.py
@@ -9,7 +9,7 @@
 SOURCES = ["gemm.hip", "gemv.hip", "gemv16p.hip", "headtail.hip", "solver.hip", "tile.hip", "prefill.hip", "attn.hip", "misc.hip", "warp.hip", "noise.hip", "kvspan.hip", "block1d.hip", "lora.hip", "resample.hip", "tempo.hip", "engine.hip",
            "engine_lm.hip", "engine_head.hip", "engine_codec.hip", "engine_prof.hip", "engine_lora.hip"]
 HEADERS = [os.path.join(CSRC, "vv_common.h"), os.path.join(CSRC, "vv_device.h"), os.path.join(CSRC, "vv_launch.h"), os.path.join(CSRC, "gemv_plan.h"),
-           os.path.join(CSRC, "prefill_plan.h"), os.path.join(CSRC, "pass_plan.h"), os.path.join(CSRC, "engine_ctx.h"),
+           os.path.join(CSRC, "prefill_plan.h"), os.path.join(CSRC, "pass_plan.h"), os.path.join(CSRC, "codec_plan.h"), os.path.join(CSRC, "engine_ctx.h"),
            os.path.join(os.path.dirname(HERE), "include", "vvhip.h")]
 
 
diff --git a/vibevoice_amd/csrc/block1d.hip b/vibevoice_amd/csrc/block1d.hip
--- a/vibevoice_amd/csrc/block1d.hip
+++ b/vibevoice_amd/csrc/block1d.hip
@@ -16,6 +16,18 @@
     int64_t sx, snst;
 };
 
+constexpr int B1D_TT = 16, B1D_HALO = 6;
+constexpr int B1D_STAGE_MAX = VV_BLOCK1D_STAGE_MAX;
+#define B1D_STAGE_WAVES(RT) ((RT) == 2 ? 8 : 4)
+
+struct VVStageArgs {
+    const float* xin;
+    float* xout;
+    int T, nb;
+    float eps;
+    VVBlock1dW b[B1D_STAGE_MAX];
+};
+
 template <int XS>
 __device__ __forceinline__ void split_store(unsigned char* base, size_t part_stride, int byte_off, float v) {
     __bf16 h = (__bf16)v;
@@ -28,206 +40,352 @@
     }
 }
 
+template <int C, int NW = 4>
+struct B1dShape {
+    static constexpr int F = 4 * C;
+    static constexpr int KT1 = C / 32, NT1 = F / 16;
+    static constexpr int KT2 = F / 32, NT2 = C / 16;
+    static constexpr int M1 = (NT1 + NW - 1) / NW, M2 = (NT2 + NW - 1) / NW;
+    static constexpr int CL = (C + 63) / 64;
+    static constexpr int PRM = 17 * C;
+};
+
+template <int C, int NW>
+struct B1dPrm {
+    using S = B1dShape<C, NW>;
+    float nw[S::CL], fnw[S::CL], dw[7], dwb, gam;
+    float4 b1[S::M1], b2[S::M2], fg[S::M2];
+};
+
+template <int C, int NW>
+__device__ __forceinline__ void b1d_load_prm(B1dPrm<C, NW>& p, const float* norm_w, const float* ffn_norm_w, const float* gamma, const float* ffn_gamma,
+                                             const float* dw_w, const float* dw_b, const float* b1, const float* b2, int tid, int wave, int lane) {
+    using S = B1dShape<C, NW>;
+#pragma unroll
+    for (int i = 0; i < S::CL; ++i) {
+        const int c = lane + i * 64;
+        p.nw[i] = (c < C) ? norm_w[c] : 0.f;
+        p.fnw[i] = (c < C) ? ffn_norm_w[c] : 0.f;
+    }
+    const int cc = tid % C;
+#pragma unroll
+    for (int j = 0; j < 7; ++j) p.dw[j] = dw_w[j * C + cc];
+    p.dwb = dw_b[cc]; p.gam = gamma[cc];
+    const int fq = lane >> 4;
+#pragma unroll
+    for (int i = 0; i < S::M1; ++i) {
+        const int nt = wave + NW * i;
+        p.b1[i] = (nt < S::NT1) ? *reinterpret_cast<const float4*>(b1 + nt * 16 + fq * 4) : float4{0.f, 0.f, 0.f, 0.f};
+    }
+#pragma unroll
+    for (int i = 0; i < S::M2; ++i) {
+        const int nt = wave + NW * i;
+        p.b2[i] = (nt < S::NT2) ? *reinterpret_cast<const float4*>(b2 + nt * 16 + fq * 4) : float4{0.f, 0.f, 0.f, 0.f};
+        p.fg[i] = (nt < S::NT2) ? *reinterpret_cast<const float4*>(ffn_gamma + nt * 16 + fq * 4) : float4{0.f, 0.f, 0.f, 0.f};
+    }
+}
+
+template <int C, int NW, class W>
+__device__ __forceinline__ void b1d_load_w1(W& w1r, const u32x4* w1, int wave, int lane) {
+    using S = B1dShape<C, NW>;
+#pragma unroll
+    for (int i = 0; i < S::M1; ++i) {
+        const int nt = wave + NW * i;
+#pragma unroll
+        for (int kt = 0; kt < S::KT1; ++kt)
+            w1r[i][kt] = (nt < S::NT1) ? w1[((int64_t)nt * S::KT1 + kt) * 64 + lane] : u32x4{0u, 0u, 0u, 0u};
+    }
+}
+template <int C, int NW, class W>
+__device__ __forceinline__ void b1d_load_w2(W& w2r, const u32x4* w2, int wave, int lane) {
+    using S = B1dShape<C, NW>;
+#pragma unroll
+    for (int i = 0; i < S::M2; ++i) {
+        const int nt = wave + NW * i;
+#pragma unroll
+        for (int kt = 0; kt < S::KT2; ++kt)
+            w2r[i][kt] = (nt < S::NT2) ? w2[((int64_t)nt * S::KT2 + kt) * 64 + lane] : u32x4{0u, 0u, 0u, 0u};
+    }
+}
+
+template <int C, int XS, int RT>
+struct B1dLds {
+    using S = B1dShape<C>;
+    static constexpr int ROWS = RT * B1D_TT;
+    static constexpr size_t NRM = 0;
+    static constexpr size_t XS_ = NRM + (size_t)(ROWS + B1D_HALO) * C * 4;
+    static constexpr size_t F1 = XS_ + (size_t)ROWS * C * 4;
+    static constexpr size_t F2 = F1 + (size_t)RT * XS * S::KT1 * 1024;
+    static constexpr size_t END = F2 + (size_t)RT * XS * S::KT2 * 1024;
+};
+
+template <int C, int XS, int RT, int NW, bool FROM_GLOBAL, bool TO_GLOBAL, class W1, class W2>
+__device__ __forceinline__ void b1d_body(unsigned char* smem, const B1dPrm<C, NW>& p, W1& w1r, W2& w2r, const float* xin, float* xout, float* nst,
+                                         int tb, int rt0, int jin, int T, float eps, bool hist) {
+    using S = B1dShape<C, NW>;
+    using L = B1dLds<C, XS, RT>;
+    constexpr int TT = B1D_TT, HALO = B1D_HALO, KT1 = S::KT1, NT1 = S::NT1, KT2 = S::KT2, NT2 = S::NT2, M1 = S::M1, M2 = S::M2, CL = S::CL;
+    float* nrm = reinterpret_cast<float*>(smem + L::NRM);
+    float* xs = reinterpret_cast<float*>(smem + L::XS_);
+    unsigned char* f1 = smem + L::F1;
+    unsigned char* f2 = smem + L::F2;
+    const int tid = threadIdx.x, lane = tid & 63;
+    const int wave = __builtin_amdgcn_readfirstlane(tid >> 6);
+    const int cc = tid % C;
+    const int frow = lane & 15, fq = lane >> 4;
+    const int jlo = rt0 * TT;
+    const int nrows = (RT - rt0) * TT + HALO;
+
+    constexpr int RW = (RT * TT + HALO + NW - 1) / NW;
+    float xv[RW][CL];
+#pragma unroll
+    for (int i = 0; i < RW; ++i) {
+        const int rr = wave + NW * i;
+        const int j = jlo - HALO + rr;
+        const int t = tb + j;
+#pragma unroll
+        for (int q = 0; q < CL; ++q) {
+            const int c = lane + q * 64;
+            float v = 0.f;
+            if (rr < nrows && c < C) {
+                if (t < 0) { if (t >= -HALO) v = nst[(HALO + t) * C + c]; }
+                else if (t < T) {
+                    if constexpr (FROM_GLOBAL) v = xin[(int64_t)t * C + c];
+                    else if (j >= jin) v = xs[j * C + c];
+                }
+            }
+            xv[i][q] = v;
+        }
+    }
+#pragma unroll
+    for (int i = 0; i < RW; ++i) {
+        const int rr = wave + NW * i;
+        if (rr >= nrows) break;
+        const int j = jlo - HALO + rr;
+        const int t = tb + j;
+        if (t < 0) {
+#pragma unroll
+            for (int q = 0; q < CL; ++q) { const int c = lane + q * 64; if (c < C) nrm[(j + HALO) * C + c] = xv[i][q]; }
+        } else if (t < T && (FROM_GLOBAL || j >= jin)) {
+            float s = 0.f;
+#pragma unroll
+            for (int q = 0; q < CL; ++q) s += xv[i][q] * xv[i][q];
+            const float r = rsqrtf(vv_wave_sum(s) / (float)C + eps);
+#pragma unroll
+            for (int q = 0; q < CL; ++q) {
+                const int c = lane + q * 64;
+                if (c < C) {
+                    const float n = xv[i][q] * r * p.nw[q];
+                    nrm[(j + HALO) * C + c] = n;
+                    if constexpr (FROM_GLOBAL) { if (j >= jlo) xs[j * C + c] = xv[i][q]; }
+                    if (hist && t >= T - HALO) nst[(HALO + t - (T - HALO)) * C + c] = n;
+                }
+            }
+        } else {
+#pragma unroll
+            for (int q = 0; q < CL; ++q) {
+                const int c = lane + q * 64;
+                if (c < C) { nrm[(j + HALO) * C + c] = 0.f; if (j >= jlo) xs[j * C + c] = 0.f; }
+            }
+        }
+    }
+    __syncthreads();
+    for (int e = jlo * C + tid; e < RT * TT * C; e += NW * 64) {
+        const int r = e / C;
+        float acc = p.dwb;
+#pragma unroll
+        for (int j = 0; j < 7; ++j) acc += p.dw[j] * nrm[(r + j) * C + cc];
+        xs[e] += p.gam * acc;
+    }
+    __syncthreads();
+    for (int r = jlo + wave; r < RT * TT; r += NW) {
+        float s = 0.f;
+        float xr[CL];
+#pragma unroll
+        for (int q = 0; q < CL; ++q) { const int c = lane + q * 64; xr[q] = (c < C) ? xs[r * C + c] : 0.f; s += xr[q] * xr[q]; }
+        const float rr = rsqrtf(vv_wave_sum(s) / (float)C + eps);
+        unsigned char* f1t = f1 + (size_t)(r >> 4) * XS * KT1 * 1024;
+#pragma unroll
+        for (int q = 0; q < CL; ++q) {
+            const int c = lane + q * 64;
+            if (c < C) {
+                const float n = xr[q] * rr * p.fnw[q];
+                const int off = vv_packed_index(c >> 5, r & 15, c) * 2;
+                split_store<XS>(f1t, (size_t)KT1 * 1024, off, n);
+            }
+        }
+    }
+    __syncthreads();
+#pragma unroll
+    for (int i1 = 0; i1 < M1; ++i1) {
+        const int nt = wave + NW * i1;
+        if (nt >= NT1) break;
+        for (int rt = rt0; rt < RT; ++rt) {
+            const unsigned char* f1t = f1 + (size_t)rt * XS * KT1 * 1024;
+            unsigned char* f2t = f2 + (size_t)rt * XS * KT2 * 1024;
+            f32x4 acc = {0.f, 0.f, 0.f, 0.f};
+#pragma unroll
+            for (int kt = 0; kt < KT1; ++kt) {
+                const bf16x8 wf = __builtin_bit_cast(bf16x8, w1r[i1][kt]);
+#pragma unroll
+                for (int pp = 0; pp < XS; ++pp) {
+                    const bf16x8 xb = __builtin_bit_cast(bf16x8, *reinterpret_cast<const u32x4*>(f1t + ((size_t)(pp * KT1 + kt) * 64 + lane) * 16));
+                    acc = __builtin_amdgcn_mfma_f32_16x16x32_bf16(wf, xb, acc, 0, 0, 0);
+                }
+            }
+            const int n0 = nt * 16 + fq * 4;
+            float u[4];
+            const float bb[4] = {p.b1[i1].x, p.b1[i1].y, p.b1[i1].z, p.b1[i1].w};
+#pragma unroll
+            for (int r = 0; r < 4; ++r) u[r] = vv_gelu_erf(acc[r] + bb[r]);
+            const int off = vv_packed_index(n0 >> 5, frow, n0) * 2;
+#pragma unroll
+            for (int r = 0; r < 4; ++r) split_store<XS>(f2t, (size_t)KT2 * 1024, off + r * 2, u[r]);
+        }
+    }
+    __syncthreads();
+#pragma unroll
+    for (int i2 = 0; i2 < M2; ++i2) {
+        const int nt = wave + NW * i2;
+        if (nt >= NT2) break;
+        for (int rt = rt0; rt < RT; ++rt) {
+            const unsigned char* f2t = f2 + (size_t)rt * XS * KT2 * 1024;
+            f32x4 acc = {0.f, 0.f, 0.f, 0.f};
+#pragma unroll
+            for (int kt = 0; kt < KT2; ++kt) {
+                const bf16x8 wf = __builtin_bit_cast(bf16x8, w2r[i2][kt]);
+#pragma unroll
+                for (int pp = 0; pp < XS; ++pp) {
+                    const bf16x8 ub = __builtin_bit_cast(bf16x8, *reinterpret_cast<const u32x4*>(f2t + ((size_t)(pp * KT2 + kt) * 64 + lane) * 16));
+                    acc = __builtin_amdgcn_mfma_f32_16x16x32_bf16(wf, ub, acc, 0, 0, 0);
+                }
+            }
+            const int c0 = nt * 16 + fq * 4;
+            const int j = rt * TT + frow;
+            const int t = tb + j;
+            float4 o;
+            o.x = xs[j * C + c0 + 0] + p.fg[i2].x * (acc[0] + p.b2[i2].x);
+            o.y = xs[j * C + c0 + 1] + p.fg[i2].y * (acc[1] + p.b2[i2].y);
+            o.z = xs[j * C + c0 + 2] + p.fg[i2].z * (acc[2] + p.b2[i2].z);
+            o.w = xs[j * C + c0 + 3] + p.fg[i2].w * (acc[3] + p.b2[i2].w);
+            if constexpr (TO_GLOBAL) {
+                if (rt == RT - 1 && t < T) *reinterpret_cast<float4*>(xout + (int64_t)t * C + c0) = o;
+            } else {
+                *reinterpret_cast<float4*>(xs + j * C + c0) = o;
+            }
+        }
+    }
+}
+
 template <int C, int XS>
 __global__ __launch_bounds__(256) void vv_block1d_kernel(const VVBlock a) {
-    constexpr int TT = 16, HALO = 6, F = 4 * C;
-    constexpr int KT1 = C / 32, NT1 = F / 16;
-    constexpr int KT2 = F / 32, NT2 = C / 16;
+    using S = B1dShape<C, 4>;
     extern __shared__ __attribute__((aligned(16))) unsigned char smem[];
-    float* nrm = reinterpret_cast<float*>(smem);
-    float* xs = nrm + (TT + HALO) * C;
-    float* rs2 = xs + TT * C;
-    unsigned char* f1 = reinterpret_cast<unsigned char*>(rs2 + TT);
-    unsigned char* f2 = f1 + (size_t)XS * KT1 * 1024;
     const int tid = threadIdx.x, lane = tid & 63;
     const int wave = __builtin_amdgcn_readfirstlane(tid >> 6);
-    const int t0 = blockIdx.x * TT;
     const float* xin = a.xin; float* xout = a.xout; float* nst = a.nst;
     if (a.sl.n > 0) {
         const int64_t id = vv_slot_id(a.sl.id, blockIdx.y);
         xin += id * a.sx; xout += id * a.sx; nst += id * a.snst;
     }
-    constexpr int M1 = (NT1 + 3) / 4, M2 = (NT2 + 3) / 4;
-    u32x4 w1r[M1][KT1], w2r[M2][KT2];
-#pragma unroll
-    for (int i = 0; i < M1; ++i) {
-        const int nt = wave + 4 * i;
-#pragma unroll
-        for (int kt = 0; kt < KT1; ++kt)
-            w1r[i][kt] = (nt < NT1) ? a.w1[((int64_t)nt * KT1 + kt) * 64 + lane] : u32x4{0u, 0u, 0u, 0u};
-    }
-#pragma unroll
-    for (int i = 0; i < M2; ++i) {
-        const int nt = wave + 4 * i;
-#pragma unroll
-        for (int kt = 0; kt < KT2; ++kt)
-            w2r[i][kt] = (nt < NT2) ? a.w2[((int64_t)nt * KT2 + kt) * 64 + lane] : u32x4{0u, 0u, 0u, 0u};
-    }
-
-    constexpr int CL = (C + 63) / 64;
-    float nw_r[CL], fnw_r[CL];
-#pragma unroll
-    for (int i = 0; i < CL; ++i) {
-        const int c = lane + i * 64;
-        nw_r[i] = (c < C) ? a.norm_w[c] : 0.f;
-        fnw_r[i] = (c < C) ? a.ffn_norm_w[c] : 0.f;
-    }
-    const int cc = tid % C;
-    float dw_r[7];
-#pragma unroll
-    for (int j = 0; j < 7; ++j) dw_r[j] = a.dw_w[j * C + cc];
-    const float dwb_r = a.dw_b[cc], gam_r = a.gamma[cc];
-    const int frow = lane & 15, fq = lane >> 4;
-    float4 b1_r[M1], b2_r[M2], fg_r[M2];
-#pragma unroll
-    for (int i = 0; i < M1; ++i) {
-        const int nt = wave + 4 * i;
-        b1_r[i] = (nt < NT1) ? *reinterpret_cast<const float4*>(a.b1 + nt * 16 + fq * 4) : float4{0.f, 0.f, 0.f, 0.f};
-    }
-#pragma unroll
-    for (int i = 0; i < M2; ++i) {
-        const int nt = wave + 4 * i;
-        b2_r[i] = (nt < NT2) ? *reinterpret_cast<const float4*>(a.b2 + nt * 16 + fq * 4) : float4{0.f, 0.f, 0.f, 0.f};
-        fg_r[i] = (nt < NT2) ? *reinterpret_cast<const float4*>(a.ffn_gamma + nt * 16 + fq * 4) : float4{0.f, 0.f, 0.f, 0.f};
-    }
-
-    constexpr int RW = (TT + HALO + 3) / 4;
-    float xv[RW][CL];
-#pragma unroll
-    for (int i = 0; i < RW; ++i) {
-        const int rr = wave + 4 * i;
-        const int t = t0 - HALO + rr;
-#pragma unroll
-        for (int q = 0; q < CL; ++q) {
-            const int c = lane + q * 64;
-            float v = 0.f;
-            if (rr < TT + HALO && c < C) {
-                if (t < 0) v = nst[(HALO + t) * C + c];
-                else if (t < a.T) v = xin[(int64_t)t * C + c];
-            }
-            xv[i][q] = v;
-        }
-    }
-#pragma unroll
-    for (int i = 0; i < RW; ++i) {
-        const int rr = wave + 4 * i;
-        if (rr >= TT + HALO) break;
-        const int t = t0 - HALO + rr;
-        if (t < 0) {
-#pragma unroll
-            for (int q = 0; q < CL; ++q) { const int c = lane + q * 64; if (c < C) nrm[rr * C + c] = xv[i][q]; }
-        } else if (t < a.T) {
-            float s = 0.f;
-#pragma unroll
-            for (int q = 0; q < CL; ++q) s += xv[i][q] * xv[i][q];
-            const float r = rsqrtf(vv_wave_sum(s) / (float)C + a.eps);
-#pragma unroll
-            for (int q = 0; q < CL; ++q) {
-                const int c = lane + q * 64;
-                if (c < C) {
-                    const float n = xv[i][q] * r * nw_r[q];
-                    nrm[rr * C + c] = n;
-                    if (rr >= HALO) xs[(rr - HALO) * C + c] = xv[i][q];
-                    if (t >= a.T - HALO) nst[(HALO + t - (a.T - HALO)) * C + c] = n;
-                }
-            }
+    u32x4 w1r[S::M1][S::KT1], w2r[S::M2][S::KT2];
+    b1d_load_w1<C, 4>(w1r, a.w1, wave, lane);
+    b1d_load_w2<C, 4>(w2r, a.w2, wave, lane);
+    B1dPrm<C, 4> p;
+    b1d_load_prm<C, 4>(p, a.norm_w, a.ffn_norm_w, a.gamma, a.ffn_gamma, a.dw_w, a.dw_b, a.b1, a.b2, tid, wave, lane);
+    b1d_body<C, XS, 1, 4, true, true>(smem, p, w1r, w2r, xin, xout, nst, blockIdx.x * B1D_TT, 0, 0, a.T, a.eps, true);
+}
+
+template <int C, int NTHR>
+__device__ __forceinline__ void b1d_stage_params(float* dst, const VVBlock1dW& b, int tid) {
+    for (int c = tid; c < C; c += NTHR) {
+        dst[c] = b.norm_w[c]; dst[C + c] = b.ffn_norm_w[c]; dst[2 * C + c] = b.gamma[c]; dst[3 * C + c] = b.ffn_gamma[c];
+        dst[11 * C + c] = b.dw_b[c]; dst[16 * C + c] = b.b2[c];
+    }
+    for (int e = tid; e < 7 * C; e += NTHR) dst[4 * C + e] = b.dw_w[e];
+    for (int e = tid; e < 4 * C; e += NTHR) dst[12 * C + e] = b.b1[e];
+}
+
+template <int C, int NTHR>
+__device__ __forceinline__ unsigned b1d_touch(const u32x4* w1, const u32x4* w2, int tid) {
+    constexpr int LINES = C * C / 16;
+    const unsigned* p1 = reinterpret_cast<const unsigned*>(w1);
+    const unsigned* p2 = reinterpret_cast<const unsigned*>(w2);
+    unsigned v = 0;
+#pragma unroll
+    for (int l0 = 0; l0 < LINES; l0 += NTHR) {
+        const int l = l0 + tid;
+        if (l < LINES) v ^= p1[l * 32] ^ p2[l * 32];
+    }
+    return v;
+}
+
+template <int C, int XS, int RT>
+__global__ __launch_bounds__(B1D_STAGE_WAVES(RT) * 64) void vv_block1d_stage_kernel(const VVStageArgs a) {
+    constexpr int NW = B1D_STAGE_WAVES(RT);
+    using S = B1dShape<C, NW>;
+    using L = B1dLds<C, XS, RT>;
+    extern __shared__ __attribute__((aligned(16))) unsigned char smem[];
+    float* prm = reinterpret_cast<float*>(smem + L::END);
+    const int tid = threadIdx.x, lane = tid & 63;
+    const int wave = __builtin_amdgcn_readfirstlane(tid >> 6);
+    const int nb = a.nb;
+    u32x4 w1r[S::M1][S::KT1], w2r[S::M2][S::KT2];
+    b1d_load_w1<C, NW>(w1r, a.b[0].w1, wave, lane);
+    b1d_load_w2<C, NW>(w2r, a.b[0].w2, wave, lane);
+#pragma unroll
+    for (int k = 0; k < B1D_STAGE_MAX; ++k)
+        if (k < nb) b1d_stage_params<C, NW * 64>(prm + k * S::PRM, a.b[k], tid);
+    const int tb = (int)blockIdx.x * B1D_TT - (RT - 1) * B1D_TT;
+    const bool hist = blockIdx.x == gridDim.x - 1;
+#pragma unroll
+    for (int k = 0; k < B1D_STAGE_MAX; ++k) {
+        if (k >= nb) break;
+        const bool last = k == nb - 1;
+        __syncthreads();
+        if (k > 0) {
+            b1d_load_w1<C, NW>(w1r, a.b[k].w1, wave, lane);
+            b1d_load_w2<C, NW>(w2r, a.b[k].w2, wave, lane);
+        }
+        unsigned warm = 0;
+        if (!last) warm = b1d_touch<C, NW * 64>(a.b[k + 1 < B1D_STAGE_MAX ? k + 1 : k].w1, a.b[k + 1 < B1D_STAGE_MAX ? k + 1 : k].w2, tid);
+        const float* q = prm + k * S::PRM;
+        B1dPrm<C, NW> p;
+        b1d_load_prm<C, NW>(p, q, q + C, q + 2 * C, q + 3 * C, q + 4 * C, q + 11 * C, q + 12 * C, q + 16 * C, tid, wave, lane);
+        const int jv = (RT - 1) * B1D_TT - B1D_HALO * (nb - 1 - k);
+        if (last) {
+            if (k == 0) b1d_body<C, XS, RT, NW, true, true>(smem, p, w1r, w2r, a.xin, a.xout, a.b[k].nst, tb, RT - 1, 0, a.T, a.eps, hist);
+            else b1d_body<C, XS, RT, NW, false, true>(smem, p, w1r, w2r, a.xin, a.xout, a.b[k].nst, tb, RT - 1, jv - B1D_HALO, a.T, a.eps, hist);
         } else {
-#pragma unroll
-            for (int q = 0; q < CL; ++q) {
-                const int c = lane + q * 64;
-                if (c < C) { nrm[rr * C + c] = 0.f; if (rr >= HALO) xs[(rr - HALO) * C + c] = 0.f; }
-            }
-        }
-    }
-    __syncthreads();
-    for (int e = tid; e < TT * C; e += 256) {
-        const int r = e / C;
-        float acc = dwb_r;
-#pragma unroll
-        for (int j = 0; j < 7; ++j) acc += dw_r[j] * nrm[(r + j) * C + cc];
-        xs[e] += gam_r * acc;
-    }
-    __syncthreads();
-    for (int r = wave; r < TT; r += 4) {
-        float s = 0.f;
-        float xr[CL];
-#pragma unroll
-        for (int q = 0; q < CL; ++q) { const int c = lane + q * 64; xr[q] = (c < C) ? xs[r * C + c] : 0.f; s += xr[q] * xr[q]; }
-        const float rr = rsqrtf(vv_wave_sum(s) / (float)C + a.eps);
-#pragma unroll
-        for (int q = 0; q < CL; ++q) {
-            const int c = lane + q * 64;
-            if (c < C) {
-                const float n = xr[q] * rr * fnw_r[q];
-                const int off = vv_packed_index(c >> 5, r, c) * 2;
-                split_store<XS>(f1, (size_t)KT1 * 1024, off, n);
-            }
-        }
-    }
-    __syncthreads();
-#pragma unroll
-    for (int i1 = 0; i1 < M1; ++i1) {
-        const int nt = wave + 4 * i1;
-        if (nt >= NT1) break;
-        f32x4 acc = {0.f, 0.f, 0.f, 0.f};
-#pragma unroll
-        for (int kt = 0; kt < KT1; ++kt) {
-            const bf16x8 wf = __builtin_bit_cast(bf16x8, w1r[i1][kt]);
-#pragma unroll
-            for (int p = 0; p < XS; ++p) {
-                const bf16x8 xb = __builtin_bit_cast(bf16x8, *reinterpret_cast<const u32x4*>(f1 + ((size_t)(p * KT1 + kt) * 64 + lane) * 16));
-                acc = __builtin_amdgcn_mfma_f32_16x16x32_bf16(wf, xb, acc, 0, 0, 0);
-            }
-        }
-        const int n0 = nt * 16 + fq * 4;
-        float u[4];
-        const float bb[4] = {b1_r[i1].x, b1_r[i1].y, b1_r[i1].z, b1_r[i1].w};
-#pragma unroll
-        for (int r = 0; r < 4; ++r) u[r] = vv_gelu_erf(acc[r] + bb[r]);
-        const int off = vv_packed_index(n0 >> 5, frow, n0) * 2;
-#pragma unroll
-        for (int r = 0; r < 4; ++r) split_store<XS>(f2, (size_t)KT2 * 1024, off + r * 2, u[r]);
-    }
-    __syncthreads();
-#pragma unroll
-    for (int i2 = 0; i2 < M2; ++i2) {
-        const int nt = wave + 4 * i2;
-        if (nt >= NT2) break;
-        f32x4 acc = {0.f, 0.f, 0.f, 0.f};
-#pragma unroll
-        for (int kt = 0; kt < KT2; ++kt) {
-            const bf16x8 wf = __builtin_bit_cast(bf16x8, w2r[i2][kt]);
-#pragma unroll
-            for (int p = 0; p < XS; ++p) {
-                const bf16x8 ub = __builtin_bit_cast(bf16x8, *reinterpret_cast<const u32x4*>(f2 + ((size_t)(p * KT2 + kt) * 64 + lane) * 16));
-                acc = __builtin_amdgcn_mfma_f32_16x16x32_bf16(wf, ub, acc, 0, 0, 0);
-            }
-        }
-        const int c0 = nt * 16 + fq * 4;
-        const int t = t0 + frow;
-        if (t < a.T) {
-            float4 o;
-            o.x = xs[frow * C + c0 + 0] + fg_r[i2].x * (acc[0] + b2_r[i2].x);
-            o.y = xs[frow * C + c0 + 1] + fg_r[i2].y * (acc[1] + b2_r[i2].y);
-            o.z = xs[frow * C + c0 + 2] + fg_r[i2].z * (acc[2] + b2_r[i2].z);
-            o.w = xs[frow * C + c0 + 3] + fg_r[i2].w * (acc[3] + b2_r[i2].w);
-            *reinterpret_cast<float4*>(xout + (int64_t)t * C + c0) = o;
-        }
+            if (k == 0) b1d_body<C, XS, RT, NW, true, false>(smem, p, w1r, w2r, a.xin, a.xout, a.b[k].nst, tb, jv >> 4, 0, a.T, a.eps, hist);
+            else b1d_body<C, XS, RT, NW, false, false>(smem, p, w1r, w2r, a.xin, a.xout, a.b[k].nst, tb, jv >> 4, jv - B1D_HALO, a.T, a.eps, hist);
+        }
+        asm volatile("" ::"v"(warm));
     }
 }
 
 template <int C, int XS>
 static void go(const VVBlock& a, hipStream_t s) {
-    constexpr int TT = 16, HALO = 6, F = 4 * C;
-    const size_t smem = (size_t)((TT + HALO) * C + TT * C + TT) * 4 + (size_t)XS * (C / 32) * 1024 + (size_t)XS * (F / 32) * 1024;
+    constexpr int TT = B1D_TT;
+    const size_t smem = B1dLds<C, XS, 1>::END;
     static const hipError_t lds = vv_raise_lds_limit(160 * 1024, &vv_block1d_kernel<C, XS>);
     (void)lds;
     hipLaunchKernelGGL((vv_block1d_kernel<C, XS>), dim3((a.T + TT - 1) / TT, a.sl.n > 0 ? a.sl.n : 1), dim3(256), smem, s, a);
 }
 
-}
-
-extern "C" int vv_block1d_supported(int C) { return C == 32 || C == 64 || C == 128; }
+template <int C, int XS, int RT>
+static void go_stage(const VVStageArgs& a, hipStream_t s) {
+    constexpr int TT = B1D_TT;
+    constexpr size_t smem = B1dLds<C, XS, RT>::END + (size_t)B1D_STAGE_MAX * B1dShape<C>::PRM * 4;
+    static_assert(smem <= 160 * 1024, "the stage kernel's rows, fragments and parameters must fit the LDS");
+    static const hipError_t lds = vv_raise_lds_limit(160 * 1024, &vv_block1d_stage_kernel<C, XS, RT>);
+    (void)lds;
+    hipLaunchKernelGGL((vv_block1d_stage_kernel<C, XS, RT>), dim3((a.T + TT - 1) / TT), dim3(B1D_STAGE_WAVES(RT) * 64), smem, s, a);
+}
+
+}
+
+extern "C" int vv_block1d_supported(int C) { return vv_plan_block1d_c(C); }
 extern "C" int vv_block1d_slots_launch(int C, int xs, const float* xin, float* xout, float* nst, const float* norm_w,
                                        const float* ffn_norm_w, const float* gamma, const float* ffn_gamma,
                                        const float* dw_w, const float* dw_b, const float* b1, const float* b2,
@@ -251,3 +409,21 @@
 #undef VV_B
     return vv_launch_rc(0);
 }
+
+extern "C" int vv_block1d_stage_launch(int C, int xs, const float* xin, float* xout, const VVBlock1dW* blocks, int nb, int T, float eps,
+                                       hipStream_t s) {
+    if (!vv_block1d_supported(C) || xs < 1 || xs > 2 || nb < 1 || nb > B1D_STAGE_MAX || T < 1 || !blocks || !xin || !xout || xin == xout) return -1;
+    VVStageArgs a;
+    a.xin = xin; a.xout = xout; a.T = T; a.nb = nb; a.eps = eps;
+    for (int k = 0; k < B1D_STAGE_MAX; ++k) a.b[k] = blocks[k < nb ? k : nb - 1];
+#define VV_S(C_)                                                     \
+    do {                                                             \
+        if (nb == 1) { if (xs == 1) go_stage<C_, 1, 1>(a, s); else go_stage<C_, 2, 1>(a, s); }      \
+        else { if (xs == 1) go_stage<C_, 1, 2>(a, s); else go_stage<C_, 2, 2>(a, s); }              \
+    } while (0)
+    if (C == 32) VV_S(32);
+    else if (C == 64) VV_S(64);
+    else VV_S(128);
+#undef VV_S
+    return vv_launch_rc(0);
+}
diff --git a/vibevoice_amd/csrc/codec_plan.h b/vibevoice_amd/csrc/codec_plan.h
--- /dev/null
+++ b/vibevoice_amd/csrc/codec_plan.h
@@ -0,0 +1,55 @@
+#pragma once
+
+inline bool vv_plan_block1d_c(int C) { return C == 32 || C == 64 || C == 128; }
+inline bool vv_plan_normdw_sliced(int T, int C) { return T >= 1 && T <= 8 && (C == 1024 || C == 2048); }
+inline bool vv_plan_normdw_rows(int T, int C) { return T >= 1 && (C == 256 || C == 512 || C == 1024); }
+
+constexpr int VV_BLOCK1D_STAGE_MAX = 3;
+constexpr int VV_BLOCK1D_MIN_ROWS = 8;
+
+enum {
+    VV_STAGE_NONE,
+    VV_STAGE_BLOCK1D,
+    VV_STAGE_BLOCK1D_STAGE,
+    VV_STAGE_ROW_PROLOGUE,
+    VV_STAGE_SLICED,
+    VV_STAGE_ROWS,
+    VV_STAGE_NORMDW1,
+    VV_STAGE_SPLIT
+};
+
+inline bool vv_codec_stage_fused(int C, int rows_per_frame, int n_blocks) {
+    return vv_plan_block1d_c(C) && rows_per_frame >= VV_BLOCK1D_MIN_ROWS && n_blocks > 0;
+}
+inline bool vv_codec_stage_pingpong(int C, int rows_per_frame, int n_blocks) {
+    return !vv_codec_stage_fused(C, rows_per_frame, n_blocks) && n_blocks > 0 &&
+           (vv_plan_normdw_sliced(rows_per_frame, C) || vv_plan_normdw_rows(rows_per_frame, C));
+}
+
+inline int vv_codec_stage_route(int C, int rows_per_frame, int frames, int n_set, int xs, int n_blocks) {
+    if (n_blocks <= 0) return VV_STAGE_NONE;
+    const int T = rows_per_frame * frames;
+    const bool batched = n_set > 0;
+    if (vv_codec_stage_fused(C, rows_per_frame, n_blocks)) {
+        const bool stage = !batched && frames == 1 && xs >= 1 && xs <= 2 && n_blocks > 1 && n_blocks <= VV_BLOCK1D_STAGE_MAX && (n_blocks & 1);
+        return stage ? VV_STAGE_BLOCK1D_STAGE : VV_STAGE_BLOCK1D;
+    }
+    const bool pp = vv_codec_stage_pingpong(C, rows_per_frame, n_blocks);
+    const bool sliced = pp && vv_plan_normdw_sliced(T, C);
+    if (sliced && T == 1 && !batched) return VV_STAGE_ROW_PROLOGUE;
+    if (sliced) return VV_STAGE_SLICED;
+    if (pp && vv_plan_normdw_rows(T, C)) return VV_STAGE_ROWS;
+    if (!pp && (long long)T * C <= 8192 && (C & 3) == 0) return VV_STAGE_NORMDW1;
+    return VV_STAGE_SPLIT;
+}
+
+inline int vv_codec_stage_launches(int route, int n_blocks) {
+    switch (route) {
+        case VV_STAGE_NONE: return 0;
+        case VV_STAGE_BLOCK1D: return n_blocks;
+        case VV_STAGE_BLOCK1D_STAGE: return 1;
+        case VV_STAGE_ROW_PROLOGUE: return 2 * n_blocks;
+        case VV_STAGE_SPLIT: return 4 * n_blocks;
+        default: return 3 * n_blocks;
+    }
+}
diff --git a/vibevoice_amd/csrc/engine_codec.hip b/vibevoice_amd/csrc/engine_codec.hip
--- a/vibevoice_amd/csrc/engine_codec.hip
+++ b/vibevoice_amd/csrc/engine_codec.hip
@@ -96,8 +96,8 @@
     }
     for (int i = 0; i < ns; ++i) {
         const int hist = (i == ns - 1) ? 6 : (decoder ? 1 : ratios[i]);
-        const bool fused = vv_block1d_supported(C[i]) && Tpf[i] >= 8 && !sw[i].blocks.empty();
-        const bool pp = !fused && !sw[i].blocks.empty() && (vv_normdw_sliced_ok(Tpf[i], C[i]) || vv_normdw_rows_ok(Tpf[i], C[i]));
+        const bool fused = vv_codec_stage_fused(C[i], Tpf[i], (int)sw[i].blocks.size());
+        const bool pp = vv_codec_stage_pingpong(C[i], Tpf[i], (int)sw[i].blocks.size());
         const int64_t xstride = (int64_t)pad64((size_t)(hist + (size_t)Tpf[i] * Fmax) * C[i]);
         float* xs_all = (float*)dalloc(ctx, (size_t)n_slots * xstride * 4);
         float* xs2_all = (fused || pp) ? (float*)dalloc(ctx, (size_t)n_slots * xstride * 4) : nullptr;
@@ -247,7 +247,18 @@
             }
         }
         float* xo = (s.fused || s.pp) ? s.xs2 + (size_t)s.hist * s.C : x;
-        if (s.fused) {
+        const int route = vv_codec_stage_route(s.C, s.Tpf, F, ss.n, ctx->c.xsplit, (int)s.blocks.size());
+        if (route == VV_STAGE_BLOCK1D_STAGE) {
+            VVBlock1dW bw[VV_BLOCK1D_STAGE_MAX];
+            for (size_t j = 0; j < s.blocks.size(); ++j) {
+                const Block& b = s.blocks[j];
+                bw[j] = {b.nst, b.norm_w, b.ffn_norm_w, b.gamma, b.ffn_gamma, b.dw_w, b.dw_b, b.b1, b.b2, (const u32x4*)b.w1, (const u32x4*)b.w2};
+            }
+            ctx->launches++;
+            VVCHK(vv_block1d_stage_launch(s.C, ctx->c.xsplit, x, xo, bw, (int)s.blocks.size(), T, eps, st));
+            continue;
+        }
+        if (route == VV_STAGE_BLOCK1D) {
             for (auto& b : s.blocks) {
                 ctx->launches++;
                 VVCHK(vv_block1d_slots_launch(s.C, ctx->c.xsplit, x, xo, b.nst, b.norm_w, b.ffn_norm_w, b.gamma, b.ffn_gamma, b.dw_w, b.dw_b,
@@ -257,8 +268,7 @@
             continue;
         }
         for (auto& b : s.blocks) {
-            const bool sliced = s.pp && vv_normdw_sliced_ok(T, s.C);
-            if (sliced && T == 1 && !batched) {
+            if (route == VV_STAGE_ROW_PROLOGUE) {
                 const VVGemm g1 = ffn1(s, b, xo, T, x);
                 if (vv_gemv_ok(&g1)) {
                     VVTRY(ffn(s, b, g1, xo, T));
@@ -266,15 +276,15 @@
                     continue;
                 }
             }
-            if (sliced) {
+            if (route == VV_STAGE_ROW_PROLOGUE || route == VV_STAGE_SLICED) {
                 ctx->launches += 1;
                 VVCHK(vv_normdw_sliced_slots_launch(x, xo, b.nb, b.norm_w, b.dw_w, b.dw_b, b.gamma, T, s.C, eps, ss.ids, ss.n, stride(s.sl_stride),
                                                     stride(b.nb_stride), st));
-            } else if (s.pp && vv_normdw_rows_ok(T, s.C)) {
+            } else if (route == VV_STAGE_ROWS) {
                 ctx->launches += 1;
                 VVCHK(vv_normdw_rows_slots_launch(x, xo, b.nb, b.norm_w, b.dw_w, b.dw_b, b.gamma, T, s.C, eps, ss.ids, ss.n, stride(s.sl_stride),
                                                   stride(b.nb_stride), st));
-            } else if (!s.pp && (size_t)T * s.C <= 8192 && (s.C & 3) == 0) {
+            } else if (route == VV_STAGE_NORMDW1) {
                 ctx->launches += 1;
                 VVCHK(vv_normdw_launch(x, b.nb, b.norm_w, b.dw_w, b.dw_b, b.gamma, T, s.C, eps, st));
             } else {
diff --git a/vibevoice_amd/csrc/engine_prof.hip b/vibevoice_amd/csrc/engine_prof.hip
--- a/vibevoice_amd/csrc/engine_prof.hip
+++ b/vibevoice_amd/csrc/engine_prof.hip
@@ -124,6 +124,24 @@
     if (r == VV_RC_NO_FORM) return VV_GEMV_REFUSED;
     if (r == 0 && form_out) for (int j = 0; j < 5; ++j) form_out[j] = form[j];
     return r;
+}
+extern "C" int vv_block1d_case(void* stream, int stage, int C, int xsplit, int nb, const float* xin, float* xout, float* nst, const float* prm,
+                               const void* const* w1, const void* const* w2, int T, float eps) {
+    if (!vv_block1d_supported(C) || xsplit < 1 || xsplit > 3 || nb < 1 || nb > VV_BLOCK1D_STAGE_MAX || T < 1 || !xin || !xout || !nst || !prm ||
+        !w1 || !w2 || xin == xout || (!stage && nb != 1))
+        return VV_GEMV_REFUSED;
+    VVBlock1dW b[VV_BLOCK1D_STAGE_MAX];
+    for (int k = 0; k < nb; ++k) {
+        const float* q = prm + (size_t)k * 17 * C;
+        b[k] = {nst + (size_t)k * 12 * C, q, q + C, q + 2 * C, q + 3 * C, q + 4 * C, q + 11 * C, q + 12 * C, q + 16 * C,
+                (const u32x4*)w1[k], (const u32x4*)w2[k]};
+    }
+    if (stage) {
+        const int r = vv_block1d_stage_launch(C, xsplit, xin, xout, b, nb, T, eps, (hipStream_t)stream);
+        return r == -1 ? VV_GEMV_REFUSED : r;
+    }
+    return vv_block1d_slots_launch(C, xsplit, xin, xout, b[0].nst, b[0].norm_w, b[0].ffn_norm_w, b[0].gamma, b[0].ffn_gamma, b[0].dw_w, b[0].dw_b,
+                                   b[0].b1, b[0].b2, b[0].w1, b[0].w2, T, eps, nullptr, 0, 0, 0, (hipStream_t)stream);
 }
 extern "C" int vv_gemm3_raw(vv_ctx* ctx, void* stream, const void* w, const void* w2, const float* x_dev, int T, int N, int K, int epi,
                             const float* nw_dev, float eps, const float* bias_dev, float* y_dev, void* xp_scratch, void* yp_scratch) {
diff --git a/vibevoice_amd/csrc/misc.hip b/vibevoice_amd/csrc/misc.hip
--- a/vibevoice_amd/csrc/misc.hip
+++ b/vibevoice_amd/csrc/misc.hip
@@ -496,7 +496,7 @@
     hipLaunchKernelGGL(vv_normdw_kernel, dim3(1), dim3(1024), 0, s, x, nb, nw, w, b, gamma, T, C, eps);
     return okk();
 }
-int vv_normdw_sliced_ok(int T, int C) { return T >= 1 && T <= 8 && (C == 1024 || C == 2048); }
+int vv_normdw_sliced_ok(int T, int C) { return vv_plan_normdw_sliced(T, C); }
 int vv_normdw_sliced_slots_launch(const float* xin, float* xout, float* nb, const float* nw, const float* w, const float* b,
                                   const float* gamma, int T, int C, float eps, const int* ids, int n, int64_t sx, int64_t snb,
                                   hipStream_t s) {
@@ -518,7 +518,7 @@
     hipLaunchKernelGGL(vv_affine_slots_kernel, dim3((L + 255) / 256, n), dim3(256), 0, s, x, y, mul, add, L, sl, stride);
     return okk();
 }
-int vv_normdw_rows_ok(int T, int C) { return T >= 1 && (C == 256 || C == 512 || C == 1024); }
+int vv_normdw_rows_ok(int T, int C) { return vv_plan_normdw_rows(T, C); }
 int vv_normdw_rows_slots_launch(const float* xin, float* xout, float* nb, const float* nw, const float* w, const float* b,
                                 const float* gamma, int T, int C, float eps, const int* ids, int n, int64_t sx, int64_t snb,
                                 hipStream_t s) {
diff --git a/vibevoice_amd/csrc/vv_launch.h b/vibevoice_amd/csrc/vv_launch.h
--- a/vibevoice_amd/csrc/vv_launch.h
+++ b/vibevoice_amd/csrc/vv_launch.h
@@ -1,6 +1,13 @@
 #pragma once
 #include "vv_common.h"
 #include "gemv_plan.h"
+#include "codec_plan.h"
+
+struct VVBlock1dW {
+    float* nst;
+    const float *norm_w, *ffn_norm_w, *gamma, *ffn_gamma, *dw_w , *dw_b, *b1, *b2;
+    const u32x4 *w1, *w2;
+};
 
 struct VVSolverStep {
     const float* eps;
@@ -44,6 +51,7 @@
 int vv_block1d_slots_launch(int C, int xs, const float* xin, float* xout, float* nst, const float* norm_w, const float* ffn_norm_w,
                             const float* gamma, const float* ffn_gamma, const float* dw_w, const float* dw_b, const float* b1, const float* b2,
                             const void* w1, const void* w2, int T, float eps, const int* ids, int n, int64_t sx, int64_t snst, hipStream_t s);
+int vv_block1d_stage_launch(int C, int xs, const float* xin, float* xout, const VVBlock1dW* blocks, int nb, int T, float eps, hipStream_t s);
 int vv_affine_slots_launch(const float* x, float* y, float mul, float add, int L, const int* ids, int n, int64_t stride, hipStream_t s);
 int vv_normdw_launch(float* x, float* nb, const float* nw, const float* w, const float* b, const float* gamma, int T, int C, float eps,
                      hipStream_t s);
diff --git a/vibevoice_amd/engine.py b/vibevoice_amd/engine.py
--- a/vibevoice_amd/engine.py
+++ b/vibevoice_amd/engine.py
@@ -809,6 +809,27 @@
             raise EngineError(f"vv_gemv_case failed ({rc})")
         return tuple(form)
 
+    def block1d_case(self, stage, C_, xs, xin, xout, nst, prm, w1, w2, T, eps):
+        nb = len(w1)
+        if len(w2) != nb or not 1 <= nb <= 3 or C_ not in (32, 64, 128) or T < 1:
+            raise ValueError("block1d_case: nb in 1..3, C in {32, 64, 128}, T >= 1")
+        for name, t, numel in (("xin", xin, T * C_), ("xout", xout, T * C_), ("nst", nst, nb * 12 * C_), ("prm", prm, nb * 17 * C_)):
+            if t.device != self.device or t.dtype != torch.float32 or not t.is_contiguous() or t.data_ptr() % 16 or t.numel() < numel:
+                raise ValueError(f"block1d_case: {name} must be a contiguous, 16-byte aligned fp32 tensor of >= {numel} elements on {self.device}")
+        for name, ws, (N, K) in (("w1", w1, (4 * C_, C_)), ("w2", w2, (C_, 4 * C_))):
+            for w in ws:
+                if w.device != self.device or w.dtype != torch.uint8 or w.numel() != int(self.lib.vv_packed_bytes(N, K)):
+                    raise ValueError(f"block1d_case: {name} entries must be pack_matrix outputs of a [{N}][{K}] matrix")
+        a1 = (C.c_void_p * nb)(*[w.data_ptr() for w in w1])
+        a2 = (C.c_void_p * nb)(*[w.data_ptr() for w in w2])
+        rc = self.lib.vv_block1d_case(self._s, 1 if stage else 0, C_, xs, nb, xin.data_ptr(), xout.data_ptr(), nst.data_ptr(), prm.data_ptr(),
+                                      a1, a2, T, float(eps))
+        if rc == _lib.GEMV_REFUSED:
+            return False
+        if rc != 0:
+            raise EngineError(f"vv_block1d_case failed ({rc})")
+        return True
+
 
 class TempoCapacityError(EngineError):
     """A Tempo.push row that brings more input, or emits more output, than one launch takes per row; nothing ran, no state changed:
```

Result: no change. 16.55, median of 6 (+0.3%).
